# cavelandiah/BBMap

Measured on AMD Instinct MI355X. Metric: aligned_reads_per_sec, higher is better.
Workload: dtype int32

## Files before the change

bbmap_amd/_lib.py:

```python
import ctypes as C
import os

HERE = os.path.dirname(os.path.abspath(__file__))
SO_PATH = os.path.join(HERE, "libbbmap_amd.so")

EXPORTS = [
    "bbmap_last_error", "bbmap_abi_version",
    "bbmsa_create", "bbmsa_destroy", "bbmsa_align_batch_device", "bbmsa_align_batch",
    "bbmsa_fill_packed", "bbmsa_fill_submit", "bbmsa_fill_collect", "bbmsa_legacy_stats", "bbmsa_last_kernel_ms", "bbmsa_last_kernel_ms3", "bbmsa_last_counts", "bbmsa_align_gapped_batch_device", "bbmsa_align_gapped_batch", "bbmsa_align_batch_device_indirect",
    "bbmsa_align_gapped_batch_device_indirect", "bbmsa_last_route", "bbmsa_last_unlimited", "bbmsa_geometry", "bbmsa_debug_sorted_lists",
    "bbband_create", "bbband_destroy", "bbband_align_batch_device", "bbband_align_batch",
    "bbband_align_quadruple_batch", "bbband_align_quadruple_progressive_batch", "bbband_align_double_batch",
    "bbidx_create", "bbidx_destroy", "bbidx_find_batch_device", "bbidx_find_batch", "bbidx_find_batch_device_rc", "bbidx_last_stats", "bbidx_last_launch", "bbidx_set_kernel", "bbidx_set_max_read_len", "bbidx_build", "bbidx_get_params", "bbidx_export_block",
    "bbmap_default_config", "bbmap_create", "bbmap_destroy", "bbmap_map_batch_device", "bbmap_map_batch", "bbmap_get_output", "bbmap_get_overflow_output", "bbmap_last_stats", "bbmap_pack_sites_device",
    "bbmap_copy_to_host", "bbidx_get_chrom_table",
    "bbpipe_revcomp_device", "bbpipe_quick_rescue_device",
    "bbidx_build_profile", "bbkeys_default_config", "bbkeys_make", "bbkeys_make_batch", "bbmap_default_config_profile",
    "bbmap_get_final", "bbmap_set_average_pair_dist", "bbmap_final_batch_device", "bbmap_untrim_batch_device",
    "bbidx_set_scaffolds", "bbmap_get_scaffold_records",
    "bbmap_get_sam_records", "bbmap_get_sam",
    "bbkeys_device_workspace_bytes", "bbkeys_make_batch_device",
    "bbpipe_run_stats_device", "bbmap_add_run_stats", "bbmap_get_run_stats", "bbmap_reset_run_stats", "bbmap_set_adaptive", "bbmap_set_truth",
    "bbmap_get_adaptive_state",
    "bbpipe_coverage_layout", "bbpipe_coverage_workspace_bytes", "bbpipe_coverage_add_device", "bbpipe_coverage_finalize_device",
    "bbmap_cov_enable", "bbmap_add_coverage", "bbmap_cov_finalize", "bbmap_get_coverage", "bbmap_reset_coverage",
    "bbpipe_read_hist_bytes", "bbpipe_read_hist_view", "bbpipe_read_hist_add_device",
    "bbmap_hist_enable", "bbmap_add_read_hist", "bbmap_get_read_hist_view", "bbmap_get_read_hist", "bbmap_reset_read_hist",
    "bbpipe_refsplit_state_bytes", "bbpipe_refsplit_add_device", "bbpipe_refsplit_lists_workspace_bytes", "bbpipe_refsplit_lists_device",
    "bbmap_split_enable", "bbmap_add_split", "bbmap_get_split_records", "bbmap_get_split_lists_device", "bbmap_get_split_lists",
    "bbmap_get_split_stats", "bbmap_reset_split",
]
TRIM_EXPORTS = ["bbtrim_default_config", "bbtrim_batch", "bbtrim_batch_device"]


class bbmsa_job(C.Structure):
    _fields_ = [("read_off", C.c_int64), ("ref_off", C.c_int64),
                ("read_len", C.c_int32), ("ref_len", C.c_int32),
                ("refStartLoc", C.c_int32), ("refEndLoc", C.c_int32),
                ("minScore", C.c_int32), ("flags", C.c_int32)]


class bbmsa_result(C.Structure):
    _fields_ = [("result", C.c_int32 * 5), ("status", C.c_int32), ("iterations", C.c_int64),
                ("score", C.c_int32 * 8), ("score_len", C.c_int32), ("match_len", C.c_int32),
                ("fill_kind", C.c_int32), ("columns", C.c_int32)]


class bbmsa_config(C.Structure):
    _fields_ = [("device", C.c_int32), ("maxRows", C.c_int32), ("maxColumns", C.c_int32),
                ("bandwidth", C.c_int32), ("bandwidthRatio", C.c_float), ("reserved", C.c_int32 * 3)]


class bbband_job(C.Structure):
    _fields_ = [("query_off", C.c_int64), ("ref_off", C.c_int64), ("query_len", C.c_int32), ("ref_len", C.c_int32),
                ("qstart", C.c_int32), ("rstart", C.c_int32), ("maxEdits", C.c_int32), ("flags", C.c_int32)]


class bbband_result(C.Structure):
    _fields_ = [("edits", C.c_int32), ("lastQueryLoc", C.c_int32), ("lastRefLoc", C.c_int32), ("lastRow", C.c_int32),
                ("lastEdits", C.c_int32), ("lastOffset", C.c_int32), ("status", C.c_int32), ("reserved", C.c_int32)]


class bbband_config(C.Structure):
# ... 10 lines not shown
    pass


def load():
    global _lib
    if _lib is not None:
        return _lib
    so_path = os.environ.get("BBMAP_AMD_SO") or SO_PATH
    if not os.path.exists(so_path):
        raise BBMapAmdError(
            "libbbmap_amd.so is missing (%s). Build it with `python -m bbmap_amd.build`; "
            "there is no CPU fallback." % so_path)
    L = C.CDLL(so_path)
    L.bbmap_last_error.restype = C.c_char_p
    L.bbmap_abi_version.restype = C.c_int
    L.bbmsa_create.argtypes = [C.POINTER(bbmsa_config), C.POINTER(C.c_void_p)]
    L.bbmsa_create.restype = C.c_int
    L.bbmsa_destroy.argtypes = [C.c_void_p]
    L.bbmsa_destroy.restype = None
    L.bbmsa_align_batch_device.argtypes = [C.c_void_p, C.c_void_p, C.c_int64, C.c_void_p, C.c_void_p,
                                           C.c_void_p, C.c_void_p, C.c_void_p, C.c_int32]
    L.bbmsa_align_batch_device.restype = C.c_int
    L.bbmsa_align_batch.argtypes = [C.c_void_p, C.c_int64, C.c_void_p, C.c_void_p, C.c_int64,
                                    C.c_void_p, C.c_int64, C.c_void_p, C.c_void_p, C.c_int32]
    L.bbmsa_align_batch.restype = C.c_int
    L.bbmsa_align_gapped_batch_device.argtypes = [C.c_void_p, C.c_void_p, C.c_int64, C.c_void_p, C.c_void_p, C.c_void_p,
                                                  C.c_void_p, C.c_void_p, C.c_void_p, C.c_int32]
    L.bbmsa_align_gapped_batch_device.restype = C.c_int
    L.bbmsa_align_batch_device_indirect.argtypes = [C.c_void_p, C.c_void_p, C.c_void_p, C.c_int64, C.c_void_p, C.c_void_p,
                                                    C.c_void_p, C.c_void_p, C.c_void_p, C.c_int32]
    L.bbmsa_align_batch_device_indirect.restype = C.c_int
    L.bbmsa_align_gapped_batch_device_indirect.argtypes = [C.c_void_p, C.c_void_p, C.c_void_p, C.c_int64, C.c_void_p, C.c_void_p,
                                                           C.c_void_p, C.c_void_p, C.c_void_p, C.c_void_p, C.c_int32]
    L.bbmsa_align_gapped_batch_device_indirect.restype = C.c_int
    L.bbmsa_align_gapped_batch.argtypes = [C.c_void_p, C.c_int64, C.c_void_p, C.c_void_p, C.c_void_p, C.c_int64,
                                           C.c_void_p, C.c_int64, C.c_void_p, C.c_void_p, C.c_int32]
    L.bbmsa_align_gapped_batch.restype = C.c_int
    L.bbmsa_fill_packed.argtypes = [C.c_void_p, C.c_void_p, C.c_int32, C.c_void_p, C.c_int32, C.c_int32, C.c_int32, C.c_int32,
                                    C.c_int32, C.c_void_p, C.POINTER(C.c_int64), C.c_void_p]
    L.bbmsa_fill_packed.restype = C.c_int
    L.bbmsa_fill_submit.argtypes = [C.c_void_p, C.c_void_p, C.c_int32, C.c_void_p, C.c_int32, C.c_int32, C.c_int32, C.c_int32,
                                    C.c_int32, C.c_void_p, C.POINTER(C.c_int64), C.c_void_p]
    L.bbmsa_fill_submit.restype = C.c_int
    L.bbmsa_fill_collect.argtypes = [C.c_void_p, C.c_void_p, C.c_void_p, C.c_void_p, C.c_void_p]
    L.bbmsa_fill_collect.restype = C.c_int
    L.bbmsa_legacy_stats.argtypes = [C.c_void_p, C.POINTER(C.c_int64)]
    L.bbmsa_legacy_stats.restype = C.c_int
    L.bbmsa_last_kernel_ms3.argtypes = [C.c_void_p, C.POINTER(C.c_float)]
    L.bbmsa_last_kernel_ms3.restype = C.c_int
    L.bbmsa_last_counts.argtypes = [C.c_void_p, C.POINTER(C.c_int64)]
    L.bbmsa_last_counts.restype = C.c_int
    L.bbmsa_debug_sorted_lists.argtypes = [C.c_void_p, C.c_int64, C.c_void_p, C.POINTER(C.c_int64)]
    L.bbmsa_debug_sorted_lists.restype = C.c_int
    L.bbmsa_last_route.argtypes = [C.c_void_p, C.POINTER(C.c_int64)]
    L.bbmsa_last_route.restype = C.c_int
    L.bbmsa_last_unlimited.argtypes = [C.c_void_p, C.POINTER(C.c_int64)]
    L.bbmsa_last_unlimited.restype = C.c_int
    L.bbmsa_geometry.argtypes = [C.c_void_p, C.POINTER(C.c_int32)]
    L.bbmsa_geometry.restype = C.c_int
    L.bbmsa_last_kernel_ms.argtypes = [C.c_void_p, C.POINTER(C.c_float), C.POINTER(C.c_float)]
    L.bbmsa_last_kernel_ms.restype = C.c_int
    L.bbband_create.argtypes = [C.POINTER(bbband_config), C.POINTER(C.c_void_p)]
    L.bbband_create.restype = C.c_int
    L.bbband_destroy.argtypes = [C.c_void_p]
    L.bbband_destroy.restype = None
    L.bbband_align_batch_device.argtypes = [C.c_void_p, C.c_void_p, C.c_int64, C.c_void_p, C.c_void_p, C.c_void_p]
    L.bbband_align_batch_device.restype = C.c_int
    L.bbband_align_batch.argtypes = [C.c_void_p, C.c_int64, C.c_void_p, C.c_void_p, C.c_int64, C.c_void_p]
    L.bbband_align_batch.restype = C.c_int
    L.bbpipe_revcomp_device.argtypes = [C.c_void_p, C.c_int64, C.c_void_p, C.c_void_p, C.c_void_p]
    L.bbpipe_revcomp_device.restype = C.c_int
    L.bbpipe_quick_rescue_device.argtypes = [C.c_void_p, C.c_int64, C.c_void_p, C.c_void_p, C.c_void_p, C.c_void_p, C.c_void_p,
                                             C.c_void_p, C.c_void_p, C.c_int32, C.c_int32, C.c_int32, C.c_int32]
    L.bbpipe_quick_rescue_device.restype = C.c_int
    _lib = L
    return L


def check(rc, what):
    if rc != 0:
        raise BBMapAmdError("%s failed (%d): %s" % (what, rc, load().bbmap_last_error().decode()))
```

bbmap_amd/csrc/mapper_ctx.h:

```cpp
#pragma once
#include <hip/hip_runtime.h>

#include <cstdio>
#include <thread>
#include <vector>

#include "bbmap_amd.h"
#include "host_common.h"
#include "index_ctx.h"
#include "mapper_dev.h"
#include "msa_ctx.h"

enum { HIO_READS, HIO_BASES, HIO_SCORES, HIO_KEYINFO, HIO_COUNTS, HIO_OFFSETS, HIO_PACKED, BUF_PACK_TMP, BUF_SAM_TMP, BUF_SAM_TEXT, BUF_COUNT };

enum { ACC_STATS, ACC_COV, ACC_HIST, ACC_SPLIT, ACC_COUNT };
struct Accum { bool counted = false; hipStream_t stream = nullptr; };

struct bbmap_ctx {
    bbmap_config cfg;
    bbidx_ctx *index;
    hipStream_t hostStream = nullptr;
    bbidx_launch probeLs;
    bbmsa_ctx *msa, *msaGapped;
    bbmapper::Settings S;
    std::vector<void *> allocs;
    bbidx_site *d_psites; int *d_pnsites;
    bbmap_msite *d_ms; int *d_mcount, *d_near;
    bbmapper::SlowState *d_slow;
    int *d_active[2];
    unsigned *d_counters;
    bbmsa_job *d_jobs; bbmap_jobinfo *d_jinfo; bbmsa_result *d_results; uint8_t *d_match;
    bbmsa_job *d_gjobs; bbmsa_gaps *d_ggaps; bbmap_jobinfo *d_ginfo; bbmsa_result *d_gresults; uint8_t *d_gmatch;
    bbresc_job *d_rjobs; bbmapper::RescInfo *d_rinfo; bbresc_result *d_rres; bbmapper::PairResc *d_pres; bbmap_msite *d_rsite;
    const uint8_t *const *d_chromArr; const int *d_chromArrLen; const uint8_t *refsBase;
    int *d_chromMin;
    long long *d_chromOff;
    long long jobCap, gjobCap, rescCap;
    bbmapper::FinalRead *d_fin; bbmap_final *d_final; uint8_t *d_pool; long long poolUnits, poolUsed, finalFills;
    int matchStride, gmatchStride, maxRows, plainColumns;
    unsigned *h_counters;
    hipEvent_t ev[bbmapper::EV_COUNT];
    bbmap_stats stats;
    long long nJobs, nGapped;
    bool ran;
    bbmap_ctx *tier;
    bool ownsMsa;
    long long narrowMinJobs;
    bool sortWide;
    bool sortPlain;
    int *d_tierUnits; bbidx_read *d_tierReads; int *d_tierReadIds;
    long long tierReads;
    hipStream_t tierStream;
    hipStream_t dpStream; hipEvent_t evFork, evJoin;
    std::thread tierThread;
    bool tierStarted;
    int tierRc; char tierErr[320];
    long long overAfterBegin;
    struct BatchArgs { int64_t n_reads; const bbidx_read *reads; uint8_t *bases; int64_t minus_delta; const int8_t *baseScores; const int32_t *keyinfo; } batch;
    DevBuf buf[BUF_COUNT];
    bbmap_scafrec *d_scafRec = nullptr;
    int *d_scafTier = nullptr;
    bbmap_samrec *d_samRec = nullptr;
    int *d_samCounts = nullptr;
    long long *d_samOffsets = nullptr;
    float *d_mapqMax = nullptr;
    long long samTextBytes = 0;
    unsigned long long *d_runStats = nullptr, *d_insertHist = nullptr;
    int adaptive = 0;
    long long numMatedSeen = 0;
    const bbmap_truth *truthNext = nullptr;
    struct CovState *cov = nullptr;
    unsigned long long *d_readHist = nullptr;
    int rhFlags = 0;
    uint8_t *d_pool2 = nullptr; long long pool2Units = 0;
    int *d_untrimCounts = nullptr;
    long long *d_untrimOffsets = nullptr;
    DevBuf untrimTmp;
    bool untrimmed = false;
    struct SplitState *split = nullptr;
    Accum accum[ACC_COUNT];
    void new_batch() { for (Accum &a : accum) a.counted = false; untrimmed = false; }
};

struct SplitState {
    bbmap_split_config cfg = {};
    int nscaf = 0;
    long long gen = 0, added = -1, total = 0;
    DevBuf sets, keys, state, recs, ws, setoff, units;
    SplitState() = default;
    SplitState(const SplitState &) = delete;
    ~SplitState() { for (DevBuf *b : {&sets, &keys, &state, &recs, &ws, &setoff, &units}) b->release(); }
};

struct CovState {
    int flags = 0, nscaf = 0, binsize = -1;
    long long slots = 0, nbins = 0, gen = 0;
    DevBuf covoff, len, diff[2], depth[2], recs, hist[2], totals, ws, refgc, binoff, bins[2];
    std::vector<int> hostLen;
    CovState() = default;
    CovState(const CovState &) = delete;
    ~CovState() {
// ... 15 lines not shown
```

bbmap_amd/csrc/mapper_host.hip:

```cpp
#include <hip/hip_runtime.h>

#include <algorithm>
#include <cstdlib>
#include <cstring>
#include <new>
#include <thread>
#include <vector>

#include "mapper_ctx.h"

using namespace bbmapper;

extern "C" int bbmap_default_config_profile(int32_t profile, bbmap_config *c) {
    if (!c || (profile != BBIDX_PROFILE_BBMAP && profile != BBIDX_PROFILE_PACBIO)) return bbfail(BBMAP_E_ARG, "bbmap_default_config: bad argument");
    memset(c, 0, sizeof *c);
    c->paired = 0; c->max_reads = 0; c->max_sites = 32;
    c->extraPadding = 10; c->maxPairDist = 32000; c->averagePairDist = 100; c->maxRescueDist = 1200; c->maxRescueMismatches = 32;
    c->maxTrimSitesToRetain = 800; c->trimList = 1; c->doRescue = 1; c->clearzone3 = 800; c->fastCols = 0; c->jobsPerRead = 0;
    c->finalStage = profile == BBIDX_PROFILE_BBMAP ? 1 : 0;
    if (profile == BBIDX_PROFILE_PACBIO) {
        c->max_read_len = 6016; c->minRatio = 0.46f; c->slowAlignPadding = 8; c->slowRescuePadding = 16; c->tipSearchDist = 15;
        c->alignColumns = 7600; c->msaMaxColumns = 7600;
    } else {
        c->max_read_len = 150; c->minRatio = 0.56f; c->slowAlignPadding = 4; c->slowRescuePadding = 8; c->tipSearchDist = 100;
// ... 62 lines not shown
    S.clearzone1e = 2 * S.ptsMatch2 - S.ptsMatch - S.ptsSub + 1;
    S.msaMaxColumns = cfg->msaMaxColumns;
    if (pacbio) { S.ptsSubR = -157; S.ptsIns = -205; S.ptsIns2 = -42; S.ptsIns3 = -23; S.ptsIns4 = -8; S.ptsDel = -292; S.ptsDel2 = -37; S.ptsDel3 = -17; S.ptsDel4 = -2; }
    else { S.ptsSubR = -147; S.ptsIns = -395; S.ptsIns2 = -39; S.ptsIns3 = -23; S.ptsIns4 = -8; S.ptsDel = -472; S.ptsDel2 = -33; S.ptsDel3 = -9; S.ptsDel4 = -1; }
    S.ptsDel5 = -1; S.ptsGap = -2;
    if (pacbio && (cfg->finalStage < 0 || cfg->finalStage > 2)) return bail(bbfail(BBMAP_E_ARG, "bbmap_create: finalStage must be 0, 1 or 2"));
    S.finalStage = cfg->finalStage ? 1 : 0;
    S.finalPolicy = (pacbio && cfg->finalStage == 1) ? 1 : 0;
    {
        const float rP = S.finalPolicy ? 1.5f : 1.6f, r1 = S.finalPolicy ? 2.2f : 2.0f, r1b = S.finalPolicy ? 2.8f : 2.6f, r1c = S.finalPolicy ? 4.8f : 4.6f;
        const float m2 = (float)S.ptsMatch2;
        S.czP = (int)(rP * m2); S.cz1 = (int)(r1 * m2); S.cz1b = (int)(r1b * m2); S.cz1c = (int)(r1c * m2);
        S.czLimit1e = 40;
    }
    index->dev.p.quitAfterTwoPerfects = cfg->paired ? 0 : 1;
    S.expLimit = (cfg->alignColumns * 17) / 20 - (2 * (cfg->slowAlignPadding + 10));
    const int maxRows = ((cfg->max_read_len + 31) / 32) * 32;
    c->maxRows = maxRows;
    bbmsa_config mc; memset(&mc, 0, sizeof mc);
    mc.device = cfg->device; mc.maxRows = maxRows;
    bbmsa_config gc;
    if (pacbio) {
        mc.maxRows = cfg->max_read_len + 4 > 6100 ? 6100 : cfg->max_read_len + 4;
        c->maxRows = mc.maxRows;
        mc.maxColumns = cfg->msaMaxColumns;
        mc.reserved[2] = BBMSA_SCHEME_9PACBIO;
        gc = mc;
        c->plainColumns = mc.maxColumns;
        if (parent) { c->msa = parent->msa; c->msaGapped = parent->msaGapped; c->ownsMsa = false; }
        else {
            c->ownsMsa = true;
            if ((rc = bbmsa_create(&mc, &c->msa)) != BBMAP_OK) return bail(rc);
            c->msaGapped = c->msa;
        }
    } else {
        mc.maxColumns = cfg->fastCols > 0 ? cfg->fastCols : 256;
        if (mc.maxColumns > cfg->msaMaxColumns) mc.maxColumns = cfg->msaMaxColumns;
        c->plainColumns = mc.maxColumns;
        gc = mc;
        gc.maxColumns = cfg->msaMaxColumns;
        gc.reserved[0] = 32; gc.reserved[1] = 640 < gc.maxColumns ? 640 : gc.maxColumns;
        if (const char *e = getenv("BBMAP_G2_LANES")) { if (*e) gc.reserved[0] = atoi(e); }
        if (const char *e = getenv("BBMAP_G2_COLS")) { if (*e) gc.reserved[1] = atoi(e) < gc.maxColumns ? atoi(e) : gc.maxColumns; }
        (void)parent;
        c->ownsMsa = true;
        if ((rc = bbmsa_create(&mc, &c->msa)) != BBMAP_OK) return bail(rc);
        if ((rc = bbmsa_create(&gc, &c->msaGapped)) != BBMAP_OK) return bail(rc);
    }
    const long long n = cfg->max_reads;
    const int cap = cfg->max_sites;
    c->narrowMinJobs = getenv("BBMAP_NARROW_MIN_JOBS") ? atoll(getenv("BBMAP_NARROW_MIN_JOBS")) : 32768;
    c->sortWide = !(getenv("BBMAP_SORT_WIDE") && atoi(getenv("BBMAP_SORT_WIDE")) == 0);
    c->sortPlain = !(getenv("BBMAP_SORT_PLAIN") && atoi(getenv("BBMAP_SORT_PLAIN")) == 0);
    if (!pacbio) {
        const bool wideUnl = !(getenv("BBMAP_WIDE_UNLIMITED") && atoi(getenv("BBMAP_WIDE_UNLIMITED")) == 0);
        bbmsa_set_wide_unlimited(c->msa, wideUnl);
        if (c->msaGapped != c->msa) bbmsa_set_wide_unlimited(c->msaGapped, wideUnl);
    }
    if (!pacbio) {
        const long long lat = getenv("BBMAP_LATENCY_JOBS") ? atoll(getenv("BBMAP_LATENCY_JOBS")) : 4096;
        if ((rc = bbmsa_set_latency_jobs(c->msa, lat)) != BBMAP_OK) return bail(rc);
        if (c->msaGapped != c->msa && (rc = bbmsa_set_latency_jobs(c->msaGapped, lat)) != BBMAP_OK) return bail(rc);
    }
    const int jpr = cfg->jobsPerRead > 0 ? cfg->jobsPerRead : 3;
    c->jobCap = n * jpr + 1024;
    c->gjobCap = parent ? n * 16 + 4096 : (n * jpr) / 24 + 4096;
    if (cfg->jobsPerRead < 0) c->jobCap = c->gjobCap = -(long long)cfg->jobsPerRead;
    c->rescCap = parent ? n * 64 + 1024 : n * 2 + 1024;
    c->matchStride = ((maxRows + c->plainColumns + 15) / 16) * 16;
    c->gmatchStride = ((maxRows + gc.maxColumns + 2 + 128 * 8 + 15) / 16) * 16;
#define DA(ptr, count) if ((rc = dalloc(c, &(ptr), (size_t)(count))) != BBMAP_OK) return bail(rc)
    DA(c->d_psites, n * cap); DA(c->d_pnsites, n);
    DA(c->d_ms, n * cap); DA(c->d_mcount, n); DA(c->d_near, n);
    DA(c->d_slow, n);
    DA(c->d_active[0], n); DA(c->d_active[1], n);
    DA(c->d_counters, CNT_WORDS);
    DA(c->d_jobs, c->jobCap); DA(c->d_jinfo, c->jobCap); DA(c->d_results, c->jobCap); DA(c->d_match, c->jobCap * c->matchStride);
    DA(c->d_gjobs, c->gjobCap); DA(c->d_ggaps, c->gjobCap); DA(c->d_ginfo, c->gjobCap); DA(c->d_gresults, c->gjobCap); DA(c->d_gmatch, c->gjobCap * c->gmatchStride);
    DA(c->d_rjobs, c->rescCap); DA(c->d_rinfo, c->rescCap); DA(c->d_rres, c->rescCap); DA(c->d_rsite, c->rescCap);
    DA(c->d_pres, n / 2 + 1);
    if (S.finalStage) {
        c->poolUnits = (n * (long long)(3 * (cfg->max_read_len + 16)) + 65536) / 4;
        if (const char *e = getenv("BBMAP_FINAL_POOL_UNITS")) { if (*e && atoll(e) >= 64) c->poolUnits = atoll(e); }
        DA(c->d_fin, n); DA(c->d_final, n); DA(c->d_pool, c->poolUnits * 4);
    }
    const int nch = index->dev.nchroms;
    DA(c->d_chromMin, nch + 1); DA(c->d_chromOff, nch + 1);
#undef DA
    c->d_chromArr = index->dev.chromArr; c->d_chromArrLen = index->dev.chromArrLen;
    {
        std::vector<const uint8_t *> hc((size_t)nch + 1);
        if (hipMemcpy(hc.data(), index->dev.chromArr, sizeof(void *) * hc.size(), hipMemcpyDeviceToHost) != hipSuccess) return bail(bbfail(BBMAP_E_HIP, "bbmap_create: reading the chromosome table failed"));
        c->refsBase = hc[1];
        std::vector<long long> off((size_t)nch + 1, 0);
        for (int i = 1; i <= nch; i++) off[(size_t)i] = (long long)(hc[(size_t)i] - hc[1]);
        if (hipMemcpy(c->d_chromOff, off.data(), 8 * off.size(), hipMemcpyHostToDevice) != hipSuccess) return bail(bbfail(BBMAP_E_HIP, "bbmap_create: upload failed"));
        if (hipMemset(c->d_chromMin, 0, 4 * ((size_t)nch + 1)) != hipSuccess) return bail(bbfail(BBMAP_E_HIP, "bbmap_create: memset failed"));
    }
    if (hipHostMalloc((void **)&c->h_counters, CNT_WORDS * 4) != hipSuccess) return bail(bbfail(BBMAP_E_NOMEM, "bbmap_create: pinned allocation failed"));
    for (hipEvent_t &e : c->ev) if (hipEventCreate(&e) != hipSuccess) return bail(bbfail(BBMAP_E_HIP, "bbmap_create: hipEventCreate failed"));
    if (!getenv("BBMAP_SERIAL_DP") && !pacbio) {
        if (hipStreamCreateWithFlags(&c->dpStream, hipStreamNonBlocking) != hipSuccess || hipEventCreateWithFlags(&c->evFork, hipEventDisableTiming) != hipSuccess ||
            hipEventCreateWithFlags(&c->evJoin, hipEventDisableTiming) != hipSuccess) return bail(bbfail(BBMAP_E_HIP, "bbmap_create: stream / event creation failed"));
    }
    *out = c;
    return BBMAP_OK;
// ... 28 lines not shown
    BBHIP(hipMemcpyAsync(c->h_counters, c->d_counters, CNT_WORDS * 4, hipMemcpyDeviceToHost, stream));
    BBHIP(hipStreamSynchronize(stream));
    return BBMAP_OK;
}

template <class T> static int regrow(bbmap_ctx *c, hipStream_t stream, T **p, size_t oldCount, size_t newCount, std::vector<void *> &dead) {
    void *d = nullptr;
    if (hipMalloc(&d, (newCount ? newCount : 1) * sizeof(T)) != hipSuccess) return bbfail(BBMAP_E_NOMEM, "bbmap_map_batch_device: growing a fill log failed (device memory)");
    if (oldCount) BBHIP(hipMemcpyAsync(d, *p, oldCount * sizeof(T), hipMemcpyDeviceToDevice, stream));
    for (void *&q : c->allocs) if (q == (void *)*p) q = d;
    dead.push_back((void *)*p);
    *p = (T *)d;
    return BBMAP_OK;
}
struct DeadArrays {
    hipStream_t stream; std::vector<void *> v;
    explicit DeadArrays(hipStream_t s) : stream(s) {}
    ~DeadArrays() { if (!v.empty()) { (void)hipStreamSynchronize(stream); for (void *q : v) (void)hipFree(q); } }
};
static int grow_logs(bbmap_ctx *c, hipStream_t stream, Dev &D, long long needJobs, long long needGapped, long long usedJobs, long long usedGapped) {
    DeadArrays guard(stream);
    std::vector<void *> &dead = guard.v;
    if (needJobs > c->jobCap) {
        long long nc = c->jobCap * 2; if (nc < needJobs) nc = needJobs + needJobs / 4 + 1024;
        BBTRY(regrow(c, stream, &c->d_jobs, (size_t)usedJobs, (size_t)nc, dead));
        BBTRY(regrow(c, stream, &c->d_jinfo, (size_t)usedJobs, (size_t)nc, dead));
        BBTRY(regrow(c, stream, &c->d_results, (size_t)usedJobs, (size_t)nc, dead));
        BBTRY(regrow(c, stream, &c->d_match, (size_t)usedJobs * c->matchStride, (size_t)nc * c->matchStride, dead));
        c->jobCap = nc;
    }
    if (needGapped > c->gjobCap) {
        long long nc = c->gjobCap * 2; if (nc < needGapped) nc = needGapped + needGapped / 4 + 1024;
        BBTRY(regrow(c, stream, &c->d_gjobs, (size_t)usedGapped, (size_t)nc, dead));
        BBTRY(regrow(c, stream, &c->d_ggaps, (size_t)usedGapped, (size_t)nc, dead));
        BBTRY(regrow(c, stream, &c->d_ginfo, (size_t)usedGapped, (size_t)nc, dead));
        BBTRY(regrow(c, stream, &c->d_gresults, (size_t)usedGapped, (size_t)nc, dead));
        BBTRY(regrow(c, stream, &c->d_gmatch, (size_t)usedGapped * c->gmatchStride, (size_t)nc * c->gmatchStride, dead));
        c->gjobCap = nc;
    }
    c->h_counters[CNT_STAGE_FILLS] = (unsigned)usedJobs; c->h_counters[CNT_STAGE_GAPPED] = (unsigned)usedGapped;
    BBHIP(hipMemcpyAsync(c->d_counters + CNT_FILLS, c->h_counters + CNT_STAGE_FILLS, 8, hipMemcpyHostToDevice, stream));
    BBHIP(hipStreamSynchronize(stream));
    D.jobs = c->d_jobs; D.jinfo = c->d_jinfo; D.results = c->d_results; D.match = c->d_match; D.jobCap = c->jobCap;
    D.gjobs = c->d_gjobs; D.ggaps = c->d_ggaps; D.ginfo = c->d_ginfo; D.gresults = c->d_gresults; D.gmatch = c->d_gmatch; D.gjobCap = c->gjobCap;
    c->stats.log_growths += 1.0f;
    return BBMAP_OK;
}

static int run_fills(bbmap_ctx *c, hipStream_t stream, const uint8_t *bases, long long jobBase, long long nNew, long long gBase, long long gNew,
                     bool finalStage = false) {
    bbmsa_use_narrow(c->msa, nNew >= c->narrowMinJobs);
    bbmsa_sort_by_width(c->msa, c->sortPlain && nNew >= c->narrowMinJobs);
    bbmsa_sort_with_band(c->msa, c->sortPlain);
    if (c->msaGapped != c->msa) { bbmsa_use_narrow(c->msaGapped, false); bbmsa_sort_by_width(c->msaGapped, c->sortWide); }
    hipStream_t gs = (c->dpStream && nNew > 0) ? c->dpStream : stream;
    if (gNew > 0) {
        if (gs != stream) { BBHIP(hipEventRecord(c->evFork, stream)); BBHIP(hipStreamWaitEvent(gs, c->evFork, 0)); }
        BBTRY(bbmsa_align_gapped_batch_device(c->msaGapped, gs, gNew, c->d_gjobs + gBase, c->d_ggaps + gBase, bases, c->refsBase,
                                             c->d_gresults + gBase, c->d_gmatch + gBase * c->gmatchStride, c->gmatchStride));
        if (gs != stream) { BBHIP(hipEventRecord(c->evJoin, gs)); if (nNew > 0) BBTRY(bbmsa_wait_first_pass(c->msaGapped, stream)); }
    }
    if (nNew > 0)
        BBTRY(bbmsa_align_batch_device(c->msa, stream, nNew, c->d_jobs + jobBase, bases, c->refsBase, c->d_results + jobBase,
                                      c->d_match + jobBase * c->matchStride, c->matchStride));
    const int r1 = nNew > 0 ? bbmsa_last_route_flags(c->msa) : 0;
    const int r2 = gNew > 0 ? bbmsa_last_route_flags(c->msaGapped) : 0;
    c->stats.dp_narrow_launches += (r1 & 1) + (r2 & 1);
    c->stats.dp_sorted_launches += ((r1 >> 1) & 1) + ((r2 >> 1) & 1);
    if (gNew > 0 && gs != stream) BBHIP(hipStreamWaitEvent(stream, c->evJoin, 0));
    return BBMAP_OK;
}

static void add_dp_ms(bbmap_ctx *c, bool plain, bool gapped) {
    float k3[3];
    if (plain && bbmsa_last_kernel_ms3(c->msa, k3) == BBMAP_OK) { c->stats.ms_dp_narrow += k3[0]; c->stats.ms_dp_wave += k3[1]; c->stats.ms_dp_generic += k3[2];
                                                                 if (k3[1] > c->stats.ms_dp_wave_max) c->stats.ms_dp_wave_max = k3[1]; }
    if (gapped && c->msaGapped != c->msa && bbmsa_last_kernel_ms3(c->msaGapped, k3) == BBMAP_OK) c->stats.ms_dp_gapped += k3[0] + k3[1] + k3[2];
    static const bool show = getenv("BBMAP_DP_COUNTS") != nullptr;
    if (show) {
        int64_t n4[4], u4[4];
        if (plain && bbmsa_last_counts(c->msa, n4) == BBMAP_OK && bbmsa_last_unlimited(c->msa, u4) == BBMAP_OK)
            fprintf(stderr, "dp counts plain : narrow finished %lld, narrow handed on %lld, wavefront list %lld, to the wide/generic pass %lld, "
                    "unlimited in their own build %lld, in the general build %lld, wavefront steps unlimited %lld of %lld\n",
                    (long long)n4[0], (long long)n4[1], (long long)n4[2], (long long)n4[3], (long long)u4[0], (long long)u4[1], (long long)u4[2], (long long)u4[3]);
        if (gapped && bbmsa_last_counts(c->msaGapped, n4) == BBMAP_OK && bbmsa_last_unlimited(c->msaGapped, u4) == BBMAP_OK)
            fprintf(stderr, "dp counts second: narrow finished %lld, narrow handed on %lld, wavefront list %lld, to the wide/generic pass %lld, "
                    "unlimited in their own build %lld, in the general build %lld, wavefront steps unlimited %lld of %lld\n",
                    (long long)n4[0], (long long)n4[1], (long long)n4[2], (long long)n4[3], (long long)u4[0], (long long)u4[1], (long long)u4[2], (long long)u4[3]);
    }
}

static void tier_start_async(bbmap_ctx *c, long long found);

struct Rounds {
    bool finalStage;
    long long jobBase, gBase;
    long long nActive;
    int cur = 0;
    bool first = true, ranPlain = false, ranGapped = false;
};
template <class K> static int round_begin(bbmap_ctx *c, hipStream_t stream, Dev &D, Rounds &R, K kernel) {
    BBHIP(hipMemsetAsync(c->d_counters + CNT_NEXT_ACTIVE, 0, 4, stream));
    if (R.finalStage) {
        BBHIP(hipMemsetAsync(c->d_counters + CNT_POOL_AT_FAILURE, 0xff, 4, stream));
        BBHIP(hipMemsetAsync(c->d_counters + CNT_POOL_FAILED, 0, 4, stream));
    }
    D.activeIn = R.first ? nullptr : c->d_active[R.cur]; D.nActiveIn = (int)R.nActive; D.activeOut = c->d_active[1 - R.cur];
    BBTRY(launch<128>(kernel, R.nActive, stream, D));
    return read_counters(c, stream);
}
static int round_end(bbmap_ctx *c, hipStream_t stream, Dev &D, Rounds &R, const uint8_t *bases) {
    add_dp_ms(c, R.ranPlain, R.ranGapped);
    const long long asked = c->h_counters[CNT_FILLS], gasked = c->h_counters[CNT_GAPPED_FILLS];
    const long long total = asked < c->jobCap ? asked : c->jobCap, gtotal = gasked < c->gjobCap ? gasked : c->gjobCap;
    BBTRY(run_fills(c, stream, bases, R.jobBase, total - R.jobBase, R.gBase, gtotal - R.gBase, R.finalStage));
    R.ranPlain = total > R.jobBase; R.ranGapped = gtotal > R.gBase;
    R.jobBase = total; R.gBase = gtotal;
    if (asked > c->jobCap || gasked > c->gjobCap) BBTRY(grow_logs(c, stream, D, asked, gasked, total, gtotal));
    R.nActive = c->h_counters[CNT_NEXT_ACTIVE];
    R.cur = 1 - R.cur; R.first = false;
    return BBMAP_OK;
}

static int grow_pool(bbmap_ctx *c, hipStream_t stream, Dev &D, long long used, long long units, bool setCounter) {
    if (units > 0x7ffffff0LL) return bbfail(BBMAP_E_NOMEM, "bbmap_map_batch_device: the final stage's match strings exceed 8 GB; map smaller batches");
    DeadArrays guard(stream);
    BBTRY(regrow(c, stream, &c->d_pool, (size_t)used * 4, (size_t)units * 4, guard.v));
    if (setCounter) {
        c->h_counters[CNT_STAGE_POOL] = (unsigned)used;
        BBHIP(hipMemcpyAsync(c->d_counters + CNT_POOL_UNITS, c->h_counters + CNT_STAGE_POOL, 4, hipMemcpyHostToDevice, stream));
    }
    BBHIP(hipStreamSynchronize(stream));
    c->poolUnits = units; D.pool = c->d_pool; D.poolUnits = units;
    return BBMAP_OK;
}

static int run_final_stage(bbmap_ctx *c, hipStream_t stream, Dev &D, int64_t n_reads, const uint8_t *bases, long long jobBase, long long gBase,
                           long long &finalRounds, long long &finalLocal) {
// ... 141 lines not shown
    c->finalFills = 0; c->poolUsed = 0;
    long long finalRounds = 0, finalLocal = 0;
    if (c->S.finalStage) BBTRY(run_final_stage(c, stream, D, n_reads, bases, jobBase, gBase, finalRounds, finalLocal));
    BBTRY(finish_stats(c, stream, true, jobBase + gBase, finalRounds, finalLocal));
    c->ran = true;
    return BBMAP_OK;
}

static int tier_pass(bbmap_ctx *c, hipStream_t s, long long found) {
    bbmap_ctx *t = c->tier;
    const bbmap_ctx::BatchArgs &B = c->batch;
    const int paired = c->cfg.paired;
    c->tierReads = 0; t->ran = false;
    std::vector<int> ids((size_t)found);
    BBHIP(hipMemcpyAsync(ids.data(), c->d_tierUnits, 4 * (size_t)found, hipMemcpyDeviceToHost, s));
    BBHIP(hipStreamSynchronize(s));
    std::sort(ids.begin(), ids.end());
    const long long room = paired ? t->cfg.max_reads / 2 : t->cfg.max_reads;
    const long long take = found < room ? found : room;
    BBHIP(hipMemcpyAsync(c->d_tierUnits, ids.data(), 4 * (size_t)take, hipMemcpyHostToDevice, s));
    BBTRY(launch<128>(gather_reads_kernel, take, s, B.reads, c->d_tierUnits, (int)take, paired, c->d_tierReads, c->d_tierReadIds));
    BBHIP(hipStreamSynchronize(s));
    const long long tn = paired ? 2 * take : take;
    BBTRY(map_records(t, s, tn, c->d_tierReads, B.bases, B.minus_delta, B.baseScores, B.keyinfo, false));
    c->tierReads = tn;
    return BBMAP_OK;
}

static void tier_start_async(bbmap_ctx *c, long long found) {
    c->tierStarted = true; c->tierRc = BBMAP_OK; c->tierErr[0] = 0;
    c->tierThread = std::thread([c, found]() {
        int rc = hipSetDevice(c->cfg.device) == hipSuccess ? BBMAP_OK : BBMAP_E_HIP;
        if (rc == BBMAP_OK) rc = tier_pass(c, c->tierStream, found);
        if (rc != BBMAP_OK) { snprintf(c->tierErr, sizeof c->tierErr, "overflow tier: %s", bbmap_last_error()); }
        c->tierRc = rc;
    });
}

static int tier_finish(bbmap_ctx *c, hipStream_t stream) {
    bbmap_ctx *t = c->tier;
    const long long tn = c->tierReads;
    if (tn == 0) return BBMAP_OK;
    BBHIP(hipMemsetAsync(c->d_counters + CNT_TIER_RESOLVED, 0, 4, stream));
    BBTRY(launch<128>(mark_tier_kernel, tn, stream, c->d_mcount, t->d_mcount, c->d_tierReadIds, (int)tn, c->d_counters + CNT_TIER_RESOLVED));
    BBTRY(read_counters(c, stream));
    bbmap_stats &st = c->stats; const bbmap_stats &ts = t->stats;
    st.reads_reprobed = tn;
    st.reads_overflowed -= (long long)c->h_counters[CNT_TIER_RESOLVED];
    st.reads_without_site += ts.reads_without_site;
    st.fills += ts.fills; st.gapped_fills += ts.gapped_fills; st.refills += ts.refills; st.rescue_scans += ts.rescue_scans;
    st.rescue_fills += ts.rescue_fills; st.fills_dropped += ts.fills_dropped;
    st.final_fills += ts.final_fills; st.final_local += ts.final_local;
    st.dp_narrow_launches += ts.dp_narrow_launches; st.dp_sorted_launches += ts.dp_sorted_launches;
    st.sites_cross_scaffold += ts.sites_cross_scaffold;
    if (getenv("BBMAP_TIER_DEBUG"))
        fprintf(stderr, "[bbmap tier] reads %lld: probe %.2f begin %.2f score %.2f slow %.2f (rounds %lld) finish %.2f rescue %.2f total %.2f\n",
                tn, ts.ms_probe, ts.ms_begin, ts.ms_score, ts.ms_slow, (long long)ts.rounds, ts.ms_finish, ts.ms_rescue, ts.ms_total);
    return BBMAP_OK;
}

static int rescue_skip_rule(bbmap_ctx *c, bool *skip) {
    *skip = false;
    if (!c->d_runStats) return BBMAP_OK;
    bbmap_runstats rs;
    BBHIP(hipStreamSynchronize(c->accum[ACC_STATS].stream));
    BBHIP(hipMemcpy(&rs, c->d_runStats, sizeof rs, hipMemcpyDeviceToHost));
    *skip = rs.mappedRetained2 > 1000 && rs.numMated * 20LL < rs.mappedRetained2;
    return BBMAP_OK;
}

static int adapt_after_batch(bbmap_ctx *c, hipStream_t stream) {
    if (!(c->adaptive & BBMAP_ADAPT_INSERT_LENGTH)) return BBMAP_OK;
    bbmap_runstats rs;
    BBHIP(hipMemcpyAsync(&rs, c->d_runStats, sizeof rs, hipMemcpyDeviceToHost, stream));
    BBHIP(hipStreamSynchronize(stream));
    const bool heldPaired = rs.numMated > c->numMatedSeen;
    c->numMatedSeen = rs.numMated;
    if (rs.numMated > 1000 && heldPaired) {
        volatile float sum = (float)rs.innerLengthSum, cnt = (float)rs.numMated;
        const float q = sum * 1.0f / cnt;
        const int v = (int)q;
        if (v >= 0) BBTRY(bbmap_set_average_pair_dist(c, v));
    }
    return BBMAP_OK;
}

extern "C" int bbmap_get_adaptive_state(bbmap_ctx *c, int32_t *averagePairDist, int32_t *rescueSkipped) {
    if (!c) return bbfail(BBMAP_E_ARG, "bbmap_get_adaptive_state: null context");
    if (averagePairDist) *averagePairDist = c->cfg.averagePairDist;
    if (rescueSkipped) {
        bool skip = false;
        if (c->adaptive & BBMAP_ADAPT_RESCUE_SKIP) { BBHIP(hipSetDevice(c->cfg.device)); BBTRY(rescue_skip_rule(c, &skip)); }
        *rescueSkipped = skip ? 1 : 0;
    }
    return BBMAP_OK;
}

static int map_batch_device(bbmap_ctx *c, hipStream_t stream, int64_t n_reads, const bbidx_read *reads, uint8_t *bases,
                            int64_t minus_delta, const int8_t *baseScores, const int32_t *keyinfo) {
    c->batch = {n_reads, reads, bases, minus_delta, baseScores, keyinfo};
    c->tierStarted = false; c->tierReads = 0;
    if (c->tier) c->tier->ran = false;
    const int rc = map_records(c, stream, n_reads, reads, bases, minus_delta, baseScores, keyinfo, true);
    hipEvent_t e0 = c->ev[EV_TIER_BEGIN], e1 = c->ev[EV_TIER_END];
    if (c->tierStarted) {
        c->tierThread.join();
// ... 72 lines not shown
```

bbmap_amd/csrc/msa_common.h:

```cpp
#pragma once
#include <hip/hip_runtime.h>
#include <stdint.h>
#include "bbmap_amd.h"

namespace bbmsa {

constexpr int kScoreOffset = 11;
constexpr int kTimeMask = 0x7FF;
constexpr int kScoreMask = (int)0xFFFFF800;
constexpr int kMaxTime = 2047;

#define BBMSA_PT(x) ((x) * 2048)
constexpr int P_MATCH = BBMSA_PT(70), P_MATCH2 = BBMSA_PT(100);
constexpr int P_SUB = BBMSA_PT(-127), P_SUBR = BBMSA_PT(-147), P_SUB2 = BBMSA_PT(-51), P_SUB3 = BBMSA_PT(-25);
constexpr int P_INS = BBMSA_PT(-395), P_INS2 = BBMSA_PT(-39), P_INS3 = BBMSA_PT(-23), P_INS4 = BBMSA_PT(-8);
constexpr int P_DEL = BBMSA_PT(-472), P_DEL2 = BBMSA_PT(-33), P_DEL3 = BBMSA_PT(-9), P_DEL4 = BBMSA_PT(-1),
              P_DEL5 = BBMSA_PT(-1);
constexpr int P_DEL_REF_N = BBMSA_PT(-10), P_GAP = BBMSA_PT(-2);
constexpr int kBadOff = (-(((1 << 20) - 1) - 2000) - 1) * 2048;
constexpr int kMinOffScore = (-(((1 << 20) - 1) - 2000)) * 2048;
constexpr int kNegInf = -(1 << 30);
constexpr int kGapLen = 128;

constexpr int kTableLen = 3072;
// ... 49 lines not shown
    static constexpr int BADOFF = (-(((1 << 22) - 1) - 2000) - 1) * 512;
#undef BBMSA_PB
    __host__ __device__ static inline int del_off(int len) {
        if (len <= 0) return 0;
        int s = DEL;
        if (len > 80) { s += ((len - 80 + 3) / 4) * DEL5; len = 80; }
        if (len > 20) { s += (len - 20) * DEL4; len = 20; }
        if (len > 5) { s += (len - 5) * DEL3; len = 5; }
        if (len > 1) s += (len - 1) * DEL2;
        return s;
    }
    __host__ __device__ static inline int ins_cum_off(int len) {
        if (len <= 0) return 0;
        int s = INS;
        if (len > 20) { s += (len - 20) * INS4; len = 20; }
        if (len > 5) { s += (len - 5) * INS3; len = 5; }
        if (len > 1) s += (len - 1) * INS2;
        return s;
    }
    __host__ __device__ static inline int col0(int row) {
        if (row <= 0) return 0;
        int s = INS;
        if (row >= 20) { s += (row - 19) * INS4; row = 19; }
        if (row >= 5) { s += (row - 4) * INS3; row = 4; }
        if (row >= 2) s += (row - 1) * INS2;
        return s;
    }
};

__host__ __device__ inline int fill_halfband(int rows, int columns, int bandwidth, float bandwidthRatio) {
    if (bandwidth < 1 && bandwidthRatio <= 0.0f) return 0;
    const int bwA = bandwidth < 1 ? 9999999 : bandwidth;
    const int bwB = bandwidthRatio <= 0.0f ? 9999999 : 8 + (int)((float)rows * bandwidthRatio);
    return max(min(bwA, bwB), columns - rows + 8) / 2;
}
__host__ __device__ inline bool fill_is_limited(int flags, int minScore, int rows, int columns, int halfband) {
    const int mode = flags & BBMSA_MODE_MASK;
    if (mode == BBMSA_FILL_UNLIMITED_RAW) return false;
    if (mode == BBMSA_FILL_LIMITED_RAW) return true;
    return !(minScore < 1 || (columns + rows < 90) ||
             ((halfband < 1 || halfband * 3 > columns) && (columns > rows + min(170, rows + 20))));
}

__host__ __device__ inline bool band_is_candidate(int flags, int minScore, int rows, int columns, int maxRows, int maxColumns, int bandRows, int maxSlack) {
    const int mode = flags & BBMSA_MODE_MASK;
    if (!(rows >= 16 && columns >= rows && rows <= maxRows && rows <= bandRows && columns <= maxColumns && mode != BBMSA_FILL_UNLIMITED_RAW)) return false;
    int tmin = minScore;
    if (mode == BBMSA_FILL_LIMITED) {
        if (tmin < 1 || (columns + rows < 90) || (columns > rows + min(170, rows + 20))) return false;
        tmin -= 120;
    }
    return (70 + 100 * (rows - 1)) - tmin <= maxSlack;
}

__device__ inline long long job_count(long long njobs, const unsigned int *njobs_dev) {
    if (!njobs_dev) return njobs;
    const long long n = (long long)__hip_atomic_load(njobs_dev, __ATOMIC_RELAXED, __HIP_MEMORY_SCOPE_AGENT);
    return n < njobs ? n : njobs;
}

constexpr int kCounterWords = 32, kCounterBytes = kCounterWords * 4;
enum CounterSlot {
    CNT_FAST_QUEUE = 0,
    CNT_SLOW_COUNT = 1,
    CNT_GENERIC_QUEUE = 2,
    CNT_BAND_QUEUE = 3,
    CNT_LIST_COUNT = 4,
    CNT_BAND_DONE = 5,
    CNT_BAND_HANDED = 6,
    CNT_WIDE_SLOW_COUNT = 7,
    CNT_WIDE_QUEUE = 8,
    CNT_UNL_RAN_UNL = 9,
    CNT_UNL_RAN_GENERAL = 10,
    CNT_UNL_LIST_COUNT = 11,
    CNT_UNL_QUEUE = 12,
    CNT_UNL_STEPS = 13,
    CNT_ALL_STEPS = 14,
    CNT_CAND_COUNT = 15,
    CNT_SORTED_COUNT = 16,
    CNT_WAVE_STEPS = 17,
};
constexpr int CNT_BAND_STATS = 5, CNT_UNL_STATS = 9;
enum BandStat { BAND_STAT_DONE = 0, BAND_STAT_HANDED = 1 };
enum UnlStat { UNL_STAT_RAN_UNL = 0, UNL_STAT_RAN_GENERAL = 1, UNL_STAT_STEPS = 4, UNL_STAT_ALL_STEPS = 5, UNL_STAT_WAVE_STEPS = 8 };
static_assert(CNT_BAND_DONE == CNT_BAND_STATS + BAND_STAT_DONE && CNT_BAND_HANDED == CNT_BAND_STATS + BAND_STAT_HANDED, "band kernel's counters");
static_assert(CNT_UNL_RAN_UNL == CNT_UNL_STATS + UNL_STAT_RAN_UNL && CNT_UNL_RAN_GENERAL == CNT_UNL_STATS + UNL_STAT_RAN_GENERAL &&
              CNT_UNL_STEPS == CNT_UNL_STATS + UNL_STAT_STEPS && CNT_ALL_STEPS == CNT_UNL_STATS + UNL_STAT_ALL_STEPS &&
              CNT_WAVE_STEPS == CNT_UNL_STATS + UNL_STAT_WAVE_STEPS, "wavefront kernel's counters");
constexpr bool counter_slots_distinct() {
    constexpr int all[] = {CNT_FAST_QUEUE, CNT_SLOW_COUNT, CNT_GENERIC_QUEUE, CNT_BAND_QUEUE, CNT_LIST_COUNT, CNT_BAND_DONE, CNT_BAND_HANDED,
                           CNT_WIDE_SLOW_COUNT, CNT_WIDE_QUEUE, CNT_UNL_RAN_UNL, CNT_UNL_RAN_GENERAL, CNT_UNL_LIST_COUNT, CNT_UNL_QUEUE,
                           CNT_UNL_STEPS, CNT_ALL_STEPS, CNT_CAND_COUNT, CNT_SORTED_COUNT, CNT_WAVE_STEPS};
    unsigned seen = 0;
    for (int s : all) { if (s < 0 || s >= kCounterWords || ((seen >> s) & 1u)) return false; seen |= 1u << s; }
    return true;
}
static_assert(counter_slots_distinct(), "two counter names share a word, or one lies outside d_counters");

struct FillParams {
    const bbmsa_job *jobs;
    const uint8_t *reads;
    const uint8_t *refs;
    bbmsa_result *results;
    uint8_t *match;
    long long njobs;
    const unsigned int *njobs_dev;
    unsigned int *queue;
    unsigned int *dirbuf;
    long long dir_slot_dwords;
    const int *list;
    const unsigned int *list_count;
    int priority;
    int *slow_list;
    unsigned int *slow_count;
    int match_stride;
    int lanesPerJob;
    int fastCols;
    int tmpBytes;
    int tableLen;
    int maxRows, maxColumns;
    int bandwidth;
    float bandwidthRatio;
    unsigned int *unl_stats;
    int *planes;
    const long long *plane_off;
    int *limits;
    const long long *limits_off;
};

struct NarrowParams {
    const bbmsa_job *jobs;
    const uint8_t *reads;
    const uint8_t *refs;
    bbmsa_result *results;
    uint8_t *match;
    long long njobs;
    const unsigned int *njobs_dev;
    unsigned int *queue;
    int *fast_list;
    unsigned int *fast_count;
    unsigned int *stats;
    int match_stride;
    int maxRows, maxColumns;
    int bandwidth;
    float bandwidthRatio;
    int maxSlack;
    unsigned int *dirbuf32;
    int tableLen;
    int bandRows;
    const int *list;
    const unsigned int *list_count;
};

struct GenericParams {
    const bbmsa_job *jobs;
    const uint8_t *reads;
    const uint8_t *refs;
    bbmsa_result *results;
    uint8_t *match;
    const int *list;
    const unsigned int *list_count;
    long long njobs;
    const unsigned int *njobs_dev;
    int *matrix;
    int *limits;
    unsigned int *queue;
    int match_stride;
    int maxRows, maxColumns;
    int bandwidth;
    float bandwidthRatio;
};

}
```

bbmap_amd/csrc/msa_ctx.h:

```cpp
#pragma once
#include <hip/hip_runtime.h>

#include "bbmap_amd.h"
#include "host_common.h"
#include "msa_route.h"

struct bbmsa_ctx {
    bbmsa_config cfg = {};
    int device = 0;
    int numCUs = 0;
    RouteSwitches sw;
    Route last;
    int G = 0, R = 0, fastCols = 0, tmpBytes = 0, blocks = 0, ldsBytes = 0, tableLen = 0, wideTableLen = 0;
    long long dirSlotDwords = 0;
    unsigned int *d_dir = nullptr;
    unsigned int *d_counters = nullptr;
    DevBuf slowList;
    int genThreads = 0;
    int *d_matrix = nullptr;
    int *d_limits = nullptr;
    int wideR = 0, wideCols = 0, wideTmpBytes = 0, wideBlocks = 0, wideLdsBytes = 0;
    long long wideDirSlotDwords = 0;
    unsigned int *d_wideDir = nullptr;
    DevBuf slowList2;
    int narrowBlocks = 0, narrowSlack = 0;
    bool unlimitedStats = false;
    unsigned int *d_widthHist = nullptr;
    int bandRows = 0, bandLds = 0;
    unsigned int *d_bandDir = nullptr;
    DevBuf fastList;
    DevBuf gref, gaux, gjobs;
    hipEvent_t ev[4] = {};
    bool timed = false;
    bool legacyOnly = false;
    struct bbmsa_legacy *legacy = nullptr;
    int stripBlocks = 0, stripLds = 0;
    long long stripDwords = 0, stripSlotDwords = 0;
    int *d_stripBoundary = nullptr;
    uint8_t *d_stripTmp = nullptr;
    int pipeK = 0, pipeSlots = 0;
    int *d_pipeBoundary = nullptr, *d_pipeSync = nullptr;
};

struct JobBatch {
    int64_t n_jobs; const uint32_t *n_jobs_dev; const bbmsa_job *jobs; const uint8_t *reads, *refs; bbmsa_result *results; uint8_t *match;
    int32_t match_stride;
};
template <class P> void set_batch(P &p, const bbmsa_ctx *c, const JobBatch &B) {
    p.jobs = B.jobs; p.reads = B.reads; p.refs = B.refs; p.results = B.results; p.match = B.match;
    p.njobs = B.n_jobs; p.njobs_dev = B.n_jobs_dev; p.match_stride = B.match_stride;
    p.maxRows = c->cfg.maxRows; p.maxColumns = c->cfg.maxColumns; p.bandwidth = c->cfg.bandwidth; p.bandwidthRatio = c->cfg.bandwidthRatio;
}

int bbmsa_width_sort(bbmsa_ctx *c, hipStream_t stream, const bbmsa_job *jobs, int64_t n_jobs, bool band);

int bbmsa_align_impl(bbmsa_ctx *c, void *stream_, int64_t n_jobs, const uint32_t *n_jobs_dev, const bbmsa_job *jobs,
                     const uint8_t *reads, const uint8_t *refs, bbmsa_result *results, uint8_t *match, int32_t match_stride);

void bbmsa_use_narrow(bbmsa_ctx *c, bool on);
int bbmsa_wait_first_pass(bbmsa_ctx *c, void *waiter);
void bbmsa_sort_by_width(bbmsa_ctx *c, bool on);
void bbmsa_sort_with_band(bbmsa_ctx *c, bool on);
void bbmsa_set_wide_unlimited(bbmsa_ctx *c, bool on);
int bbmsa_set_latency_jobs(bbmsa_ctx *c, int64_t n);
enum { BBMSA_ROUTE_NARROW = 1, BBMSA_ROUTE_SORTED = 2, BBMSA_ROUTE_LATENCY = 4 };
int bbmsa_last_route_flags(const bbmsa_ctx *c);

int bbmsa_legacy_create(bbmsa_ctx *c);
void bbmsa_legacy_destroy(bbmsa_ctx *c);
void bbmsa_legacy_rows_per_lane(bbmsa_ctx *c, int *last, int *mask);
```

bbmap_amd/csrc/msa_fill_band.hip:

```cpp
#include "msa_common.h"
#include "msa_cell.h"

namespace bbmsa {

namespace {

__device__ __forceinline__ int from_left(int x, int fill) { return __builtin_amdgcn_update_dpp(fill, x, 0x138, 0xf, 0xf, false); }
__device__ __forceinline__ int from_right(int x, int fill) { return __builtin_amdgcn_update_dpp(fill, x, 0x130, 0xf, 0xf, false); }

__device__ __forceinline__ unsigned ld_coherent(const unsigned *p) { return __hip_atomic_load(p, __ATOMIC_RELAXED, __HIP_MEMORY_SCOPE_AGENT); }
__device__ __forceinline__ unsigned ld_coherent(const uint8_t *p) { return __hip_atomic_load(p, __ATOMIC_RELAXED, __HIP_MEMORY_SCOPE_AGENT); }

struct BandSet {
    int M[4], D[4], I[4];
    int rows, columns;
    int c0off;
    int minScoreOff, vs;
    unsigned w;
    int gprev;
    int gmask, mprev;
    int gpass;
    int bail;
    int rdOff, rfOff;
    int slot;
};

}

#ifndef BBMSA_BAND_OCC
#define BBMSA_BAND_OCC 4
#endif

template <int Q>
__global__ __launch_bounds__(256, BBMSA_BAND_OCC) void msa_fill_band_kernel(const NarrowParams p) {
    constexpr int B = 4 * Q;
    constexpr int GROUPS = 64 / Q;
    constexpr int JOBS = 2 * GROUPS;
    static_assert(Q == 4 || Q == 8 || Q == 16, "a group is a power of two of lanes, its good bits fit 64");
    extern __shared__ int lds[];
    const int TL = p.tableLen;
    int *delC = lds, *insC = lds + TL, *delExt = lds + 2 * TL, *insExt = delExt + 128;
    int4 *mTab = reinterpret_cast<int4 *>(delExt + 192);
    LdsPen pen; pen.delC = delC; pen.insC = insC; pen.delExt = delExt; pen.insExt = insExt; pen.mTab = mTab;
    for (int i = threadIdx.x; i < TL; i += blockDim.x) { delC[i] = calc_del_off(i); insC[i] = calc_ins_cum_off(i); }
    for (int i = threadIdx.x; i < 128; i += blockDim.x) delExt[i] = SpelledPen<Scheme11ts>().del_ext(i);
    if (threadIdx.x < 32) insExt[threadIdx.x] = SpelledPen<Scheme11ts>().ins_ext(threadIdx.x);
    if (threadIdx.x < 32) {
        const int st = threadIdx.x & 7, mt = (threadIdx.x >> 3) & 1, pv = threadIdx.x >> 4;
        const MEntry e = SpelledPen<Scheme11ts>().m_entry(min(st, 5), 0, 0, pv != 0, mt != 0);
        int4 v; v.x = e.addA; v.y = e.bonus; v.z = e.t3sub; v.w = 0;
        mTab[threadIdx.x] = v;
    }
    __syncthreads();

    const int lane = threadIdx.x & 63, wave = threadIdx.x >> 6;
    const int q = lane & (Q - 1), grp = lane / Q, groupBase = grp * Q;
    const int RB = (p.bandRows + 4 + 3) & ~3, FB = (p.bandRows + B + 4 + 3) & ~3;
    uint8_t *jobLds = reinterpret_cast<uint8_t *>(lds + lds_table_ints(TL)) + (long long)wave * JOBS * (RB + FB);
    unsigned *dir = p.dirbuf32 + ((long long)blockIdx.x * 4 + wave) * (long long)(p.bandRows + 1) * 128;
    const long long NJ = p.list ? (long long)ld_coherent(p.list_count) : job_count(p.njobs, p.njobs_dev);
    unsigned nDone = 0, nLeft = 0;

    for (;;) {
        long long myJ = -1;
        if (lane < JOBS) {
            for (;;) {
                const long long e_ = (long long)atomicAdd(p.queue, 1u);
                if (e_ >= NJ || e_ >= p.njobs) break;
                const long long t_ = p.list ? (long long)p.list[e_] : e_;
                const bbmsa_job t = p.jobs[t_];
                int ta = t.refStartLoc, tb = t.refEndLoc;
                if (t.flags & BBMSA_CLAMP_WINDOW) {
                    ta = max(0, ta); tb = min(t.ref_len - 1, tb);
                    if (tb - ta >= p.maxColumns) tb = min(t.ref_len - 1, ta + p.maxColumns - 1);
                }
                if (band_is_candidate(t.flags, t.minScore, t.read_len, tb - ta + 1, p.maxRows, p.maxColumns, p.bandRows, p.maxSlack)) { myJ = t_; break; }
                const unsigned k = atomicAdd(p.fast_count, 1u);
                p.fast_list[k] = (int)t_;
            }
        }
        if (!__any(myJ >= 0)) break;

        BandSet S[2];
        long long jobJ[2]; bool jobOk[2];
#pragma unroll
        for (int s = 0; s < 2; s++) {
            const long long j = __shfl(myJ, grp * 2 + s, 64);
            jobJ[s] = j;
            bbmsa_job jb;
            jb.read_off = 0; jb.ref_off = 0; jb.read_len = 0; jb.ref_len = 0; jb.refStartLoc = 0; jb.refEndLoc = -1; jb.minScore = 0; jb.flags = 0;
            if (j >= 0) jb = p.jobs[j];
            int a = jb.refStartLoc, b = jb.refEndLoc;
            if (jb.flags & BBMSA_CLAMP_WINDOW) {
                a = max(0, a); b = min(jb.ref_len - 1, b);
                if (b - a >= p.maxColumns) b = min(jb.ref_len - 1, a + p.maxColumns - 1);
            }
            const int rows = jb.read_len, columns = b - a + 1;
            int minScore = jb.minScore;
            if ((jb.flags & BBMSA_MODE_MASK) == BBMSA_FILL_LIMITED) minScore -= 120;
            const int D0 = (columns - rows) / 2 - B / 2;
            const uint8_t *rd = p.reads + jb.read_off, *rf = p.refs + jb.ref_off + a;
            const int rdOff = (grp * 2 + s) * (RB + FB), rfOff = rdOff + RB;
            int cost = 0; bool allDef = true;
#pragma unroll 4
            for (int i = q; i < rows; i += Q) {
                const int cb = rd[i];
                jobLds[rdOff + i] = (uint8_t)cb;
                if (fully_defined(cb)) cost += (i + 1 < rows && fully_defined(rd[i + 1])) ? P_MATCH2 : P_MATCH;
            }
            if (j >= 0)
#pragma unroll 4
            for (int k = q; k < rows + B + 1; k += Q) {
                const int col = k + D0;
                int v = 0;
                if (col == 0) v = '!';
                else if (col >= 1 && col <= columns) { v = rf[col - 1]; allDef = allDef && fully_defined(v); }
                jobLds[rfOff + k] = (uint8_t)v;
            }
            for (int c = 1 + q; c <= columns; c += Q) if (c < 1 + D0 || c > D0 + B) allDef = allDef && fully_defined(rf[c - 1]);
            int nd = allDef ? 0 : 1;
            for (int d = 1; d < Q; d <<= 1) { cost += __shfl_xor(cost, d, 64); nd |= __shfl_xor(nd, d, 64); }
            bool ok = j >= 0 && nd == 0;

            const int minScoreOff = minScore * 2048;
            const int floorv = minScoreOff - ((rows - 1) * P_MATCH2 + P_MATCH);
            const int subfloor = floorv - 5 * P_MATCH2;
            if (ok) {
                const int cl1 = rd[0];
                const int c0cost = fully_defined(cl1) ? ((rows > 1 && fully_defined(rd[1])) ? P_MATCH2 : P_MATCH) : 0;
// ... 66 lines not shown
                    const int c0 = row + T.c0off;
                    const int insRow = insC[row], insPrev = insC[row - 1];
                    const int delForce = (row < 3 || row > rows - 3) ? INT_MAX : INT_MIN;
                    const unsigned g5 = (unsigned)T.gmask | (((unsigned)uG & 1u) << 4);
                    const bool rowOne = row == 1;
                    unsigned goods = 0, mbits = 0, word = 0;
                    int leftM = lM, leftD = lD;
#pragma unroll
                    for (int i = 0; i < 4; i++) {
                        const int c = c0 + i;
                        const int ref1 = (int)((T.w >> (8 * i)) & 255u);
                        const bool inRange = (c >= 1) & (c <= columns);
                        const bool started = (T.gprev != 0) | ((g5 & ((4u << i) - 1u)) != 0u);
                        const bool first = c == 1;
                        const int hs = c <= columns - 1 ? P_MATCH + (columns - 1 - c) * P_MATCH2 : 0;
                        CellIn ci;
                        ci.row = row; ci.c = c; ci.rows = rows; ci.insNeededBase = (columns - c) + 1;
                        ci.cl1 = cl1; ci.ref1 = ref1; ci.refN = false; ci.gap = false; ci.match = cl1 == ref1; ci.act = inRange & started;
                        ci.refPen = 0; ci.limitP = max(vlimP, max(T.minScoreOff - hs, floorv) + 2048); ci.floorP = floorP; ci.subfloor = subfloor;
                        ci.dgM = first ? insPrev : T.M[i]; ci.dgD = first ? insPrev : T.D[i]; ci.dgI = first ? insPrev : T.I[i];
                        ci.lM = first ? insRow : leftM; ci.lD = first ? insRow : leftD;
                        ci.upM = i < 3 ? T.M[i + 1] : uM; ci.upI = i < 3 ? T.I[i + 1] : uI;
                        ci.delForce = delForce;
                        ci.insForce = ((rowOne & (c > 1)) | ((row > rows - 2) & (c < columns - 1))) ? INT_MAX : INT_MIN;
                        ci.pm8 = ((T.mprev >> i) & 1) ? 8 : 0;
                        const CellOut co = cell_update<Scheme11ts, false>(pen, ci);
                        const bool good = co.goodM | co.goodD | co.goodI;
                        goods |= good ? (1u << i) : 0u;
                        mbits |= ci.match ? (1u << i) : 0u;
                        word |= co.nib << (4 * i);
                        T.M[i] = co.nM; T.D[i] = co.nD; T.I[i] = co.nI;
                        leftM = co.nM; leftD = co.nD;
                    }
                    if (q == 0 && (goods & 1u) && c0 >= 1) T.bail = 1;
                    if (q == Q - 1 && (goods & 8u) && c0 + 3 < columns) T.bail = 1;
                    T.gprev = gIn; T.gmask = (int)goods; T.mprev = (int)mbits; T.gpass = (gIn | (goods ? 1 : 0));
                    dir[((long long)row * 2 + T.slot) * 64 + lane] = word | (goods << 16);
                }
            }
        }
        asm volatile("s_waitcnt vmcnt(0)" ::: "memory");
        __builtin_amdgcn_wave_barrier();

#pragma unroll
        for (int s = 0; s < 2; s++) {
            const long long j = jobJ[s];
            const int set = (q & 1) ^ s;
            int lastM[4], lastD[4], lastI[4];
#pragma unroll
            for (int i = 0; i < 4; i++) { lastM[i] = set ? S[1].M[i] : S[0].M[i]; lastD[i] = set ? S[1].D[i] : S[0].D[i]; lastI[i] = set ? S[1].I[i] : S[0].I[i]; }
            int bail = set ? S[1].bail : S[0].bail;
            for (int d = 1; d < Q; d <<= 1) bail |= __shfl_xor(bail, d, 64);
            const bool live = jobOk[s];
            if (live && bail) { if (q == 0) { const unsigned k = atomicAdd(p.fast_count, 1u); p.fast_list[k] = (int)j; nLeft++; } }
            if (!(live && !bail)) continue;

            const bbmsa_job jb = p.jobs[j];
            int a = jb.refStartLoc, b = jb.refEndLoc;
            if (jb.flags & BBMSA_CLAMP_WINDOW) {
                a = max(0, a); b = min(jb.ref_len - 1, b);
                if (b - a >= p.maxColumns) b = min(jb.ref_len - 1, a + p.maxColumns - 1);
            }
            const int rows = jb.read_len, columns = b - a + 1, mode = jb.flags & BBMSA_MODE_MASK;
            const int minScoreOff = (mode == BBMSA_FILL_LIMITED ? jb.minScore - 120 : jb.minScore) * 2048;
            const int subfloor = minScoreOff - ((rows - 1) * P_MATCH2 + P_MATCH) - 5 * P_MATCH2;
            const int D0 = (columns - rows) / 2 - B / 2;
            const uint8_t *rdL = jobLds + (grp * 2 + s) * (RB + FB), *rfL = rdL + RB;
            const unsigned *jdir = dir + s * 64 + groupBase;

            const int per = (rows + Q - 1) / Q;
            const int rFirst = q * per + 1, rLast = min(rows, (q + 1) * per);
            int iters = 0, lastColStart = 1, lastHasGood = 0, lastEntered = 0;
            {
                unsigned long long pg = 0;
                if (rFirst > 1 && rFirst <= rLast) for (int l = 0; l < Q; l++) pg |= (unsigned long long)((ld_coherent(jdir + (long long)(rFirst - 1) * 128 + l) >> 16) & 15u) << (4 * l);
                for (int r = rFirst; r <= rLast; r++) {
                    unsigned long long g = 0;
                    for (int l = 0; l < Q; l++) g |= (unsigned long long)((ld_coherent(jdir + (long long)r * 128 + l) >> 16) & 15u) << (4 * l);
                    const bool entered = r == 1 || pg != 0;
                    const int colStart = r == 1 ? 1 : (r - 1) + D0 + __builtin_ctzll(pg | (1ull << 63));
                    const int colStop = r == 1 ? columns : (r - 1) + D0 + (63 - __builtin_clzll(pg | 1ull));
                    const int maxG = g ? r + D0 + (63 - __builtin_clzll(g)) : -2;
                    const int endc = min(columns, max(colStop, maxG) + 1);
                    if (entered) iters += endc - colStart + 1;
                    if (r == rows) { lastColStart = colStart; lastHasGood = g != 0; lastEntered = entered; }
                    pg = g;
                }
            }
            for (int d = 1; d < Q; d <<= 1) iters += __shfl_xor(iters, d, 64);
            {
                const int owner = groupBase + (rows - 1) / per;
                lastColStart = __shfl(lastColStart, owner, 64); lastHasGood = __shfl(lastHasGood, owner, 64); lastEntered = __shfl(lastEntered, owner, 64);
            }
            int bScore = INT_MIN, bKey = INT_MAX, bPacked = 0;
#pragma unroll
            for (int i = 0; i < 4; i++) {
                const int c = rows + D0 + 4 * q + i;
                if (c >= 1 && c <= columns) {
                    const int v[3] = {lastM[i], lastD[i], lastI[i]};
#pragma unroll
                    for (int st = 0; st < 3; st++) {
                        const int sc = v[st] & kScoreMask, key = st * 65536 + c;
                        if (sc > bScore || (sc == bScore && key < bKey)) { bScore = sc; bKey = key; bPacked = v[st]; }
                    }
                }
            }
            for (int d = 1; d < Q; d <<= 1) {
// ... 53 lines not shown
                }
                int colS = col;
                if (row > colS) colS -= row;
                const int bestRefStart = a + colS, bestRefStop = a + res1 - 1;
                int padLeft = 0, padRight = 0;
                if (bestRefStart < a) padLeft = max(0, a - bestRefStart);
                else if (bestRefStart == a && state == 2) padLeft = stateTime;
                const int bW = (jb.flags & BBMSA_INTERNAL_GAPPED) ? jb.ref_len : b;
                if (bestRefStop > bW) padRight = max(0, bestRefStop - bW);
                else if (bestRefStop == bW && res2 == 2) padRight = bPacked & kTimeMask;
                if (wantScore) {
                    sc[0] = bScore >> kScoreOffset; sc[1] = bestRefStart; sc[2] = bestRefStop; sc[3] = rows; sc[4] = res1; sc[5] = res2;
                    scoreLen = (padLeft > 0 || padRight > 0) ? 8 : 6;
                    if (scoreLen == 8) { sc[6] = padLeft; sc[7] = padRight; }
                }
                if (wantTrace) {
                    const int xs = (col != row) ? row : 0;
                    for (int i = q; i < xs; i += Q) if (n + i < p.match_stride) out[n + i] = 'X';
                    n += xs;
                    if (n > p.match_stride) matchLen = -1;
                    else {
                        asm volatile("s_waitcnt vmcnt(0)" ::: "memory");
                        __builtin_amdgcn_wave_barrier();
                        for (int i = q; i < n / 2; i += Q) {
                            const uint8_t lo = (uint8_t)ld_coherent(out + i), hi = (uint8_t)ld_coherent(out + n - 1 - i);
                            out[i] = hi; out[n - 1 - i] = lo;
                        }
                        matchLen = n;
                    }
                }
            }
            if (q == 0) {
                bbmsa_result r;
                r.result[0] = rows; r.result[1] = res1; r.result[2] = res2; r.result[3] = res3; r.result[4] = res4;
                r.status = (fillNull && mode == BBMSA_FILL_LIMITED) ? BBMSA_ST_NULL : BBMSA_ST_OK;
                r.iterations = iters;
#pragma unroll
                for (int i = 0; i < 8; i++) r.score[i] = sc[i];
                r.score_len = scoreLen; r.match_len = matchLen; r.fill_kind = 0; r.columns = columns;
                p.results[j] = r;
                nDone++;
            }
        }
        __builtin_amdgcn_fence(__ATOMIC_ACQ_REL, "wavefront");
        __builtin_amdgcn_wave_barrier();
    }
    if (p.stats) {
        for (int d = 32; d >= 1; d >>= 1) { nDone += __shfl_xor(nDone, d, 64); nLeft += __shfl_xor(nLeft, d, 64); }
        if (lane == 0) { if (nDone) atomicAdd(&p.stats[BAND_STAT_DONE], nDone); if (nLeft) atomicAdd(&p.stats[BAND_STAT_HANDED], nLeft); }
    }
}

template __global__ void msa_fill_band_kernel<8>(const NarrowParams);

const void *band_kernel() { return (const void *)msa_fill_band_kernel<8>; }
int band_lds_bytes(int tableLen, int bandRows) {
    constexpr int Q = 8, B = 4 * Q, JOBS = 2 * (64 / Q);
    const int RB = (bandRows + 4 + 3) & ~3, FB = (bandRows + B + 4 + 3) & ~3;
    return lds_table_ints(tableLen) * 4 + 4 * JOBS * (RB + FB);
}

}
```

bbmap_amd/csrc/msa_fill_fast.hip:

```cpp
#include "msa_common.h"
#include "msa_cell.h"

namespace bbmsa {

__device__ __forceinline__ int lane_up(int x, int fill) {
    return __builtin_amdgcn_update_dpp(fill, x, 0x138, 0xf, 0xf, false);
}

__device__ __forceinline__ int clamp_time(int t) { return t > kMaxTime ? kMaxTime - 3 : t; }

__device__ __forceinline__ int del_extend(int streak) {
    int c = (streak & 3) == 0 ? P_DEL5 : 0;
    c = streak < 80 ? P_DEL4 : c;
    c = streak < 20 ? P_DEL3 : c;
    c = streak < 5 ? P_DEL2 : c;
    c = streak == 0 ? P_DEL : c;
    return c;
}
__device__ __forceinline__ int ins_extend(int streak) {
    int c = P_INS4;
    c = streak < 20 ? P_INS3 : c;
    c = streak < 5 ? P_INS2 : c;
    c = streak == 0 ? P_INS : c;
    return c;
}
__device__ __forceinline__ int sub_extend(int streak) {
    int c = P_SUB3;
    c = streak < 5 ? P_SUB2 : c;
    c = streak == 0 ? P_SUB : c;
    return c;
}

__device__ __forceinline__ unsigned load_coherent(const unsigned *p) {
    return __hip_atomic_load(p, __ATOMIC_RELAXED, __HIP_MEMORY_SCOPE_AGENT);
}

#ifndef BBMSA_MIN_WAVES
#define BBMSA_MIN_WAVES(R) ((R) <= 5 ? 4 : ((R) <= 7 ? 2 : 1))
#endif

template <int R, bool BANDED, bool MAT = false, int UNL = 0>
__global__ __launch_bounds__(256, (UNL == 2 && BBMSA_MIN_WAVES(R) > 2) ? 2 : BBMSA_MIN_WAVES(R)) void msa_fill_fast_kernel(const FillParams p) {
    extern __shared__ int lds[];
    int *delC = lds;
    const int TL = p.tableLen;
    int *insC = lds + TL;
    int *delExt = lds + 2 * TL;
    int *insExt = delExt + 128;
    int4 *mTab = reinterpret_cast<int4 *>(delExt + 192);
    LdsPen pen; pen.delC = delC; pen.insC = insC; pen.delExt = delExt; pen.insExt = insExt; pen.mTab = mTab;
    for (int i = threadIdx.x; i < TL; i += blockDim.x) {
        delC[i] = calc_del_off(i);
        insC[i] = calc_ins_cum_off(i);
    }
    for (int i = threadIdx.x; i < 128; i += blockDim.x) delExt[i] = del_extend(i);
    if (threadIdx.x < 32) insExt[threadIdx.x] = ins_extend(threadIdx.x);
    if (threadIdx.x < 32) {
        const int st = threadIdx.x & 7, mt = (threadIdx.x >> 3) & 1, pv = threadIdx.x >> 4;
        int4 e;
        if (mt) { e.x = pv ? P_MATCH2 : P_MATCH; e.y = P_MATCH; e.z = P_MATCH2; }
        else { e.x = pv ? (st <= 1 ? P_SUBR : P_SUB) : sub_extend(min(st, 5)); e.y = P_SUB; e.z = P_SUB3; }
        e.w = 0;
        mTab[threadIdx.x] = e;
    }
    __syncthreads();

    if (p.priority == 3) __builtin_amdgcn_s_setprio(3);
    else if (p.priority == 2) __builtin_amdgcn_s_setprio(2);
    else if (p.priority == 1) __builtin_amdgcn_s_setprio(1);
    const int lane = threadIdx.x & 63;
    const int wave = threadIdx.x >> 6;
    const int G = p.lanesPerJob;
    const int gl = lane & (G - 1);
    const int sub = lane / G;
    const int jobsPerWave = 64 / G;
    const int groupBase = sub * G;

    const int perJobLds = lds_job_ints(p.fastCols, p.tmpBytes);
    int *myLds = lds + lds_table_ints(TL) + (wave * jobsPerWave + sub) * perJobLds;
    int *colHl = myLds;
    uint8_t *colRef = reinterpret_cast<uint8_t *>(myLds + (p.fastCols + 2));
    uint8_t *tmp = reinterpret_cast<uint8_t *>(myLds + (p.fastCols + 2) + ((p.fastCols + 2 + 3) >> 2));

    const long long slot = ((long long)blockIdx.x * (blockDim.x >> 6) + wave) * jobsPerWave + sub;
    unsigned *dir = p.dirbuf + slot * p.dir_slot_dwords;

    const long long total = p.list ? (long long)load_coherent(p.list_count) : job_count(p.njobs, p.njobs_dev);
    for (;;) {
        unsigned base = 0;
        if (lane == 0) base = atomicAdd(p.queue, (unsigned)jobsPerWave);
        base = __builtin_amdgcn_readfirstlane(base);
        if ((long long)base >= total) break;
        const long long q = (long long)base + sub;
        const bool valid = q < total;
        const long long j = (p.list && valid) ? (long long)p.list[q] : q;

        bbmsa_job jb;
        if (valid) jb = p.jobs[j];
        else { jb.read_off = 0; jb.ref_off = 0; jb.read_len = 0; jb.ref_len = 0; jb.refStartLoc = 0; jb.refEndLoc = -1; jb.minScore = 0; jb.flags = 0; }
        const int rows = jb.read_len;
        int a = jb.refStartLoc, b = jb.refEndLoc;
        const int mode = jb.flags & BBMSA_MODE_MASK;
        if (jb.flags & BBMSA_CLAMP_WINDOW) {
            a = max(0, a);
            b = min(jb.ref_len - 1, b);
            if (b - a >= p.maxColumns) b = min(jb.ref_len - 1, a + p.maxColumns - 1);
        }
        const int columns = b - a + 1;
        const bool shapeOK = valid && rows >= 1 && columns >= 1 && rows <= p.maxRows && columns <= p.maxColumns;

        const int halfband = fill_halfband(rows, columns, p.bandwidth, p.bandwidthRatio);
        const bool limited = fill_is_limited(jb.flags, jb.minScore, rows, columns, halfband);
        const int minScore = (limited && mode != BBMSA_FILL_LIMITED_RAW) ? jb.minScore - 120 : jb.minScore;
        const bool fits = rows <= G * R && columns <= p.fastCols && columns >= rows - 2;
        const bool needGeneric = shapeOK && (!fits || (UNL == 1 && limited));
        const bool run = shapeOK && !needGeneric;
        const bool banded = limited && halfband > 0;
        int bandViolation = 0;

        if (gl == 0 && valid) {
            if (!shapeOK) {
                bbmsa_result r;
                for (int i = 0; i < 5; i++) r.result[i] = 0;
                r.status = BBMSA_ST_BAD_SHAPE; r.iterations = 0;
                for (int i = 0; i < 8; i++) r.score[i] = 0;
                r.score_len = 0; r.match_len = 0; r.fill_kind = 0; r.columns = columns;
                p.results[j] = r;
            } else if (needGeneric) {
                const unsigned k = atomicAdd(p.slow_count, 1u);
                p.slow_list[k] = (int)j;
            }
        }

        const uint8_t *rd = p.reads + jb.read_off;
        const uint8_t *rf = p.refs + jb.ref_off + a;
        int *planeM = nullptr; long long planeInts = 0; int planeW = 0;
        if (MAT && valid) { planeW = columns; planeInts = (long long)rows * planeW; planeM = p.planes + p.plane_off[j]; }

        const int maxGain = (rows - 1) * P_MATCH2 + P_MATCH;
        const int minScoreOff = minScore * 2048;
// ... 505 lines not shown
```

bbmap_amd/csrc/msa_host.hip:

```cpp
#include <hip/hip_runtime.h>

#include <cstdio>
#include <cstdlib>
#include <new>

#include "host_common.h"
#include "msa_common.h"
#include "msa_ctx.h"

namespace bbmsa {
struct StripParams {
    const bbmsa_job *jobs; const uint8_t *reads; const uint8_t *refs; bbmsa_result *results; uint8_t *match;
    long long njobs; const unsigned int *njobs_dev; unsigned int *queue; unsigned int *dirbuf;
    long long dir_slot_dwords, dir_strip_dwords; int *boundary; uint8_t *tmpbuf; int *slow_list; unsigned int *slow_count;
    int match_stride; int maxRows, maxColumns; int bandwidth; float bandwidthRatio;
    int pipeK, pipeSlots; int *pipeBoundary; int *pipeSync; int pipeSpinLimit;
};
int strip_rows_per_lane();
const void *strip_kernel_pacbio();
const void *strip_kernel_pacbio_pipelined();
int strip_pipe_sync_ints(int K);
const void *fast_kernel_for(int R, bool banded);
const void *fast_kernel_unl_for(int R);
const void *fast_kernel_both_for(int R);
template <class S> __global__ void msa_fill_generic_kernel(const GenericParams p);
const void *band_kernel();
int band_lds_bytes(int tableLen, int bandRows);
}

static int clamp_occupancy(int per, int most) { return per < 1 ? 1 : (per > most ? most : per); }

static int setup_wide_pass(bbmsa_ctx *c) {
    if (c->wideBlocks > 0) return BBMAP_OK;
    c->wideR = (c->cfg.maxRows + 63) / 64;
    c->wideCols = c->cfg.maxColumns;
    c->wideTmpBytes = ((64 * c->wideR + c->wideCols + 8) + 3) & ~3;
    const int perJob = bbmsa::lds_job_ints(c->wideCols, c->wideTmpBytes);
    c->wideLdsBytes = (bbmsa::lds_table_ints(c->wideTableLen) + perJob) * 4;
    const void *wfn = bbmsa::fast_kernel_for(c->wideR, c->sw.banded);
    if (wfn && c->wideLdsBytes <= 160 * 1024) {
        if (c->wideLdsBytes > 64 * 1024) BBHIP(hipFuncSetAttribute(wfn, hipFuncAttributeMaxDynamicSharedMemorySize, c->wideLdsBytes));
        const void *bfn = c->sw.banded ? nullptr : bbmsa::fast_kernel_both_for(c->wideR);
        if (bfn && c->wideLdsBytes > 64 * 1024) BBHIP(hipFuncSetAttribute(bfn, hipFuncAttributeMaxDynamicSharedMemorySize, c->wideLdsBytes));
        int per = 0;
        BBHIP(hipOccupancyMaxActiveBlocksPerMultiprocessor(&per, wfn, 64, c->wideLdsBytes));
        per = clamp_occupancy(per, 8);
        const long long slotDwords = (long long)(((c->wideCols + 64 - 1) >> 3) + 1) * c->wideR * 64;
        BBHIP(hipMalloc(&c->d_wideDir, (size_t)((long long)c->numCUs * per * slotDwords * 4)));
        c->wideDirSlotDwords = slotDwords;
        c->wideBlocks = c->numCUs * per;
        c->sw.widePresent = true;
    }
    return BBMAP_OK;
}

static int generic_threads(const bbmsa_config &cfg, int defaultMB, long long mostThreads, int *out) {
    const long long perThread = 3LL * (cfg.maxRows + 1) * (cfg.maxColumns + 2) * 4;
    long long threads = ((long long)env_int("BBMSA_GENERIC_SCRATCH_MB", defaultMB) << 20) / perThread;
    if (threads > mostThreads) threads = mostThreads;
    threads = (threads / 64) * 64;
    if (threads < 64) return bbfail(BBMAP_E_NOMEM, "bbmsa_create: BBMSA_GENERIC_SCRATCH_MB cannot hold one wavefront of scratch matrices for this maxRows x maxColumns");
    *out = (int)threads;
    return BBMAP_OK;
}
static int alloc_generic_scratch(bbmsa_ctx *c, int threads) {
    c->genThreads = threads;
    BBHIP(hipMalloc(&c->d_matrix, (size_t)threads * 3 * (size_t)(c->cfg.maxRows + 1) * (size_t)(c->cfg.maxColumns + 2) * 4));
    BBHIP(hipMalloc(&c->d_limits, (size_t)threads * (size_t)(c->cfg.maxRows + c->cfg.maxColumns + 4) * 4));
    return BBMAP_OK;
}

static int create_legacy_only(bbmsa_ctx *c) {
    BBTRY(alloc_generic_scratch(c, 1));
    return bbmsa_legacy_create(c);
}

static int create_pacbio(bbmsa_ctx *c) {
    const bbmsa_config *cfg = &c->cfg;
    int threads = 0;
    BBTRY(generic_threads(*cfg, 40960, 4096, &threads));
// ... 36 lines not shown
    if (G != 16 && G != 32 && G != 64) {
        G = env_int("BBMSA_LANES_PER_JOB", 0);
        if (G != 16 && G != 32 && G != 64) G = (cfg->maxRows <= 320) ? 32 : 64;
    }
    while (G < 64 && (cfg->maxRows + G - 1) / G > 10) G *= 2;
    c->G = G;
    c->R = (cfg->maxRows + G - 1) / G;
    int fastCols = cfg->reserved[1] > 0 ? cfg->reserved[1] : env_int("BBMSA_FAST_COLS", 0);
    if (fastCols <= 0) fastCols = cfg->maxColumns < 640 ? cfg->maxColumns : 640;
    if (fastCols > cfg->maxColumns) fastCols = cfg->maxColumns;
    c->fastCols = fastCols;
    c->tmpBytes = ((G * c->R + fastCols + 8) + 3) & ~3;
    const int jobsPerWave = 64 / G;
    const int perJobInts = bbmsa::lds_job_ints(fastCols, c->tmpBytes);
    {
        const int side = (cfg->maxColumns > cfg->maxRows ? cfg->maxColumns : cfg->maxRows) + 2;
        c->wideTableLen = (side < 2048 ? side : 2048) + cfg->maxRows + 8;
        const int sideF = (fastCols > cfg->maxRows ? fastCols : cfg->maxRows) + 2;
        c->tableLen = (sideF < 2048 ? sideF : 2048) + cfg->maxRows + 8;
    }
    if (c->tableLen > bbmsa::kTableLen) c->tableLen = bbmsa::kTableLen;
    if (c->wideTableLen > bbmsa::kTableLen) c->wideTableLen = bbmsa::kTableLen;
    c->tableLen = (c->tableLen + 3) & ~3; c->wideTableLen = (c->wideTableLen + 3) & ~3;
    c->ldsBytes = (bbmsa::lds_table_ints(c->tableLen) + 4 * jobsPerWave * perJobInts) * 4;
    if (c->ldsBytes > 160 * 1024) return bbfail(BBMAP_E_ARG, "bbmsa_create: fast-path LDS budget exceeded; lower reserved[1] (fastCols)");

    c->sw.banded = !(cfg->bandwidth < 1 && cfg->bandwidthRatio <= 0.0f);
    const void *kfn = bbmsa::fast_kernel_for(c->R, c->sw.banded);
    if (!kfn) return bbfail(BBMAP_E_ARG, "bbmsa_create: no kernel for this rows-per-lane");
    if (c->ldsBytes > 64 * 1024) {
        BBHIP(hipFuncSetAttribute(kfn, hipFuncAttributeMaxDynamicSharedMemorySize, c->ldsBytes));
        BBHIP(hipFuncSetAttribute(bbmsa::fast_kernel_unl_for(c->R), hipFuncAttributeMaxDynamicSharedMemorySize, c->ldsBytes));
    }
    int blocksPerCU = 0;
    BBHIP(hipOccupancyMaxActiveBlocksPerMultiprocessor(&blocksPerCU, kfn, 256, c->ldsBytes));
    if (blocksPerCU < 1) blocksPerCU = 1;
    const int capBlocks = env_int("BBMSA_BLOCKS_PER_CU", 0);
    if (capBlocks > 0 && capBlocks < blocksPerCU) blocksPerCU = capBlocks;
    c->blocks = c->numCUs * blocksPerCU;

    const int maxSteps = fastCols + G - 1;
    c->dirSlotDwords = (long long)((maxSteps >> 3) + 1) * c->R * G;
    const long long slots = (long long)c->blocks * 4 * jobsPerWave;
    BBHIP(hipMalloc(&c->d_dir, (size_t)(slots * c->dirSlotDwords * 4)));

    int threads = 0;
    BBTRY(generic_threads(*cfg, 2048, 16384, &threads));
    BBTRY(alloc_generic_scratch(c, threads));
    if (cfg->maxColumns > fastCols) BBTRY(setup_wide_pass(c));
    c->narrowSlack = env_int("BBMSA_NARROW_SLACK", 2000);
    if (!c->sw.banded && env_int("BBMSA_NARROW", 1) != 0) {
        int perCU = 0;
        c->bandRows = cfg->maxRows < 256 ? cfg->maxRows : 256;
        c->bandLds = bbmsa::band_lds_bytes(c->tableLen, c->bandRows);
        if (c->bandLds > 64 * 1024) BBHIP(hipFuncSetAttribute(bbmsa::band_kernel(), hipFuncAttributeMaxDynamicSharedMemorySize, c->bandLds));
        BBHIP(hipOccupancyMaxActiveBlocksPerMultiprocessor(&perCU, bbmsa::band_kernel(), 256, c->bandLds));
        c->narrowBlocks = c->numCUs * clamp_occupancy(perCU, 4);
        c->sw.bandPresent = true;
        BBHIP(hipMalloc(&c->d_bandDir, (size_t)c->narrowBlocks * 4 * (size_t)(c->bandRows + 1) * 128 * 4));
    }
    c->sw.sortByWidth = env_int("BBMSA_SORT_BY_WIDTH", 0) != 0;
    c->sw.sortWithBand = env_int("BBMSA_SORT_WITH_BAND", 0) != 0;
    c->sw.wideUnlimited = env_int("BBMSA_WIDE_UNLIMITED", 0) != 0;
    c->sw.unlimitedLoop = env_int("BBMSA_UNLIMITED_LOOP", 1) != 0;
    c->unlimitedStats = env_int("BBMSA_UNLIMITED_STATS", 0) != 0 || getenv("BBMAP_DP_COUNTS") != nullptr;
    { const int lat = env_int("BBMSA_LATENCY_JOBS", 0); if (lat > 0) BBTRY(bbmsa_set_latency_jobs(c, lat)); }
    return BBMAP_OK;
}

extern "C" int bbmsa_create(const bbmsa_config *cfg, bbmsa_ctx **out) {
    if (!cfg || !out) return bbfail(BBMAP_E_ARG, "bbmsa_create: null argument");
    *out = nullptr;
    const int scheme = cfg->reserved[2] & 0xFF;
    const bool legacyOnly = (cfg->reserved[2] & BBMSA_LEGACY_ONLY) != 0;
    if (scheme != BBMSA_SCHEME_11TS && scheme != BBMSA_SCHEME_9PACBIO) return bbfail(BBMAP_E_ARG, "bbmsa_create: unknown scoring scheme");
    if (scheme == BBMSA_SCHEME_11TS && (cfg->maxRows < 1 || cfg->maxRows > 640 || cfg->maxColumns < 1 || cfg->maxColumns > 4096))
        return bbfail(BBMAP_E_ARG, "bbmsa_create: maxRows must be 1..640 and maxColumns 1..4096");
    if (scheme == BBMSA_SCHEME_9PACBIO && (cfg->maxRows < 1 || cfg->maxRows > 6100 || cfg->maxColumns < 1 || cfg->maxColumns > 8192))
        return bbfail(BBMAP_E_ARG, "bbmsa_create: the PacBio scheme takes maxRows 1..6100 and maxColumns 1..8192");
    hipDeviceProp_t prop;
    BBTRY(bb_use_gfx950("bbmsa_create", cfg->device, &prop));

    bbmsa_ctx *c = new (std::nothrow) bbmsa_ctx();
    if (!c) return bbfail(BBMAP_E_NOMEM, "bbmsa_create: out of host memory");
    c->cfg = *cfg;
    c->device = cfg->device;
    c->numCUs = prop.multiProcessorCount;
    c->sw.scheme = scheme;
    c->legacyOnly = legacyOnly;
    struct Guard { bbmsa_ctx *c; ~Guard() { if (c) bbmsa_destroy(c); } } guard{c};
    BBTRY(legacyOnly ? create_legacy_only(c) : scheme != BBMSA_SCHEME_11TS ? create_pacbio(c) : create_11ts(c));
    BBHIP(hipMalloc(&c->d_counters, bbmsa::kCounterBytes));
    BBHIP(hipMemset(c->d_counters, 0, bbmsa::kCounterBytes));
    for (int i = 0; i < 4; i++) BBHIP(hipEventCreate(&c->ev[i]));
    guard.c = nullptr;
    *out = c;
    return BBMAP_OK;
}

extern "C" void bbmsa_destroy(bbmsa_ctx *c) {
    if (!c) return;
    (void)hipSetDevice(c->device);
    bbmsa_legacy_destroy(c);
    if (c->d_dir) (void)hipFree(c->d_dir);
    if (c->d_counters) (void)hipFree(c->d_counters);
    if (c->d_widthHist) (void)hipFree(c->d_widthHist);
    for (DevBuf *b : {&c->slowList, &c->slowList2, &c->fastList, &c->gref, &c->gaux, &c->gjobs}) b->release();
    if (c->d_matrix) (void)hipFree(c->d_matrix);
    if (c->d_limits) (void)hipFree(c->d_limits);
    if (c->d_wideDir) (void)hipFree(c->d_wideDir);
    if (c->d_bandDir) (void)hipFree(c->d_bandDir);
    if (c->d_stripBoundary) (void)hipFree(c->d_stripBoundary);
// ... 3 lines not shown
    for (int i = 0; i < 4; i++) if (c->ev[i]) (void)hipEventDestroy(c->ev[i]);
    delete c;
}

extern "C" int bbmsa_align_batch_device(bbmsa_ctx *c, void *stream_, int64_t n_jobs,
                                        const bbmsa_job *jobs, const uint8_t *reads, const uint8_t *refs,
                                        bbmsa_result *results, uint8_t *match, int32_t match_stride) {
    return bbmsa_align_impl(c, stream_, n_jobs, nullptr, jobs, reads, refs, results, match, match_stride);
}

extern "C" int bbmsa_align_batch_device_indirect(bbmsa_ctx *c, void *stream_, const uint32_t *n_jobs_dev, int64_t max_jobs,
                                                 const bbmsa_job *jobs, const uint8_t *reads, const uint8_t *refs,
                                                 bbmsa_result *results, uint8_t *match, int32_t match_stride) {
    if (!n_jobs_dev) return bbfail(BBMAP_E_ARG, "bbmsa_align_batch_device_indirect: null counter");
    return bbmsa_align_impl(c, stream_, max_jobs, n_jobs_dev, jobs, reads, refs, results, match, match_stride);
}

namespace {
using namespace bbmsa;

template <class S> int launch_generic(bbmsa_ctx *c, const JobBatch &B, hipStream_t stream, const int *list, const unsigned int *count) {
    bbmsa::GenericParams gp;
    set_batch(gp, c, B);
    gp.list = list; gp.list_count = count;
    gp.matrix = c->d_matrix; gp.limits = c->d_limits; gp.queue = c->d_counters + CNT_GENERIC_QUEUE;
    hipLaunchKernelGGL(bbmsa::msa_fill_generic_kernel<S>, dim3(c->genThreads / 64), dim3(64), 0, stream, gp);
    BBHIP(hipGetLastError());
    BBHIP(hipEventRecord(c->ev[2], stream));
    c->timed = true;
    return BBMAP_OK;
}

int launch_strip(bbmsa_ctx *c, const JobBatch &B, const Route &r, hipStream_t stream) {
    bbmsa::StripParams sp;
    set_batch(sp, c, B);
    sp.queue = c->d_counters + CNT_FAST_QUEUE; sp.dirbuf = c->d_dir; sp.dir_slot_dwords = c->stripSlotDwords; sp.dir_strip_dwords = c->stripDwords;
    sp.boundary = c->d_stripBoundary; sp.tmpbuf = c->d_stripTmp; sp.slow_list = c->slowList.as<int>(); sp.slow_count = c->d_counters + CNT_SLOW_COUNT;
    sp.pipeK = 0; sp.pipeSlots = 0; sp.pipeBoundary = nullptr; sp.pipeSync = nullptr;
    sp.pipeSpinLimit = env_int("BBMSA_PIPE_SPIN_LIMIT", 1 << 21);
    if (sp.pipeSpinLimit < 1) sp.pipeSpinLimit = 1;
    void *sargs[] = {&sp};
    if (r.pipelined) {
        const long long slots = r.jobs < c->pipeSlots ? r.jobs : c->pipeSlots;
        sp.pipeK = c->pipeK; sp.pipeSlots = (int)slots; sp.pipeBoundary = c->d_pipeBoundary; sp.pipeSync = c->d_pipeSync;
        BBHIP(hipMemsetAsync(c->d_pipeSync, 0, (size_t)(slots * bbmsa::strip_pipe_sync_ints(c->pipeK) * 4), stream));
        BBHIP(hipLaunchKernel(bbmsa::strip_kernel_pacbio_pipelined(), dim3((unsigned)(slots * c->pipeK)), dim3(64), sargs, (size_t)c->stripLds, stream));
        return BBMAP_OK;
    }
    const long long sblocks = r.jobs < c->stripBlocks ? r.jobs : c->stripBlocks;
    BBHIP(hipLaunchKernel(bbmsa::strip_kernel_pacbio(), dim3((unsigned)sblocks), dim3(64), sargs, (size_t)c->stripLds, stream));
    return BBMAP_OK;
}

int launch_band(bbmsa_ctx *c, const JobBatch &B, const Route &r, hipStream_t stream) {
    int *const fastList = c->fastList.as<int>();
    bbmsa::NarrowParams np;
    set_batch(np, c, B);
    np.queue = c->d_counters + CNT_BAND_QUEUE; np.fast_list = fastList; np.fast_count = c->d_counters + CNT_LIST_COUNT;
    np.stats = c->d_counters + CNT_BAND_STATS; np.maxSlack = c->narrowSlack;
    np.dirbuf32 = c->d_bandDir; np.tableLen = c->tableLen; np.bandRows = c->bandRows;
    np.list = r.sorted ? fastList + 2 * r.jobs : nullptr; np.list_count = r.sorted ? c->d_counters + CNT_CAND_COUNT : nullptr;
    long long nb = (r.jobs + 63) / 64;
    if (nb > c->narrowBlocks) nb = c->narrowBlocks;
    void *nargs[] = {&np};
    BBHIP(hipLaunchKernel(bbmsa::band_kernel(), dim3((unsigned)nb), dim3(256), nargs, (size_t)c->bandLds, stream));
    return BBMAP_OK;
}

bbmsa::FillParams first_pass_params(const bbmsa_ctx *c, const JobBatch &B, const Route &r) {
    bbmsa::FillParams fp = {};
    set_batch(fp, c, B);
    fp.queue = c->d_counters + CNT_FAST_QUEUE; fp.dirbuf = c->d_dir; fp.dir_slot_dwords = c->dirSlotDwords;
    fp.list = (r.band || r.sorted) ? c->fastList.as<int>() : nullptr; fp.list_count = c->d_counters + CNT_LIST_COUNT; fp.priority = 0;
    fp.slow_list = c->slowList.as<int>(); fp.slow_count = c->d_counters + CNT_SLOW_COUNT;
    fp.lanesPerJob = c->G; fp.fastCols = c->fastCols; fp.tmpBytes = c->tmpBytes; fp.tableLen = c->tableLen;
    fp.unl_stats = c->unlimitedStats ? c->d_counters + CNT_UNL_STATS : nullptr;
    return fp;
}

int launch_unlimited(bbmsa_ctx *c, const bbmsa::FillParams &fp, const Route &r, long long blocks, hipStream_t stream) {
    bbmsa::FillParams up = fp;
    up.queue = c->d_counters + CNT_UNL_QUEUE; up.list = c->fastList.as<int>() + r.jobs; up.list_count = c->d_counters + CNT_UNL_LIST_COUNT;
    void *uargs[] = {&up};
    BBHIP(hipLaunchKernel(bbmsa::fast_kernel_unl_for(c->R), dim3((unsigned)blocks), dim3(256), uargs, (size_t)c->ldsBytes, stream));
    return BBMAP_OK;
}

int launch_wide(bbmsa_ctx *c, const bbmsa::FillParams &fp, const Route &r, hipStream_t stream) {
    bbmsa::FillParams wp = fp;
    wp.queue = c->d_counters + CNT_WIDE_QUEUE; wp.dirbuf = c->d_wideDir; wp.dir_slot_dwords = c->wideDirSlotDwords;
    wp.list = r.latency ? nullptr : fp.slow_list; wp.list_count = r.latency ? nullptr : fp.slow_count;
    wp.slow_list = c->slowList2.as<int>(); wp.slow_count = c->d_counters + CNT_WIDE_SLOW_COUNT;
    wp.lanesPerJob = 64; wp.fastCols = c->wideCols; wp.tmpBytes = c->wideTmpBytes; wp.tableLen = c->wideTableLen;
    static const int widePrio = env_int("BBMSA_WIDE_PRIORITY", 2);
    wp.priority = widePrio;
    void *wargs[] = {&wp};
    const long long wblocks = r.latency && r.jobs < c->wideBlocks ? r.jobs : c->wideBlocks;
    const void *bothFn = r.wideBoth ? bbmsa::fast_kernel_both_for(c->wideR) : nullptr;
    BBHIP(hipLaunchKernel(bothFn ? bothFn : bbmsa::fast_kernel_for(c->wideR, c->sw.banded), dim3((unsigned)wblocks), dim3(64), wargs, (size_t)c->wideLdsBytes, stream));
    return BBMAP_OK;
}
}

int bbmsa_align_impl(bbmsa_ctx *c, void *stream_, int64_t n_jobs, const uint32_t *n_jobs_dev,
                     const bbmsa_job *jobs, const uint8_t *reads, const uint8_t *refs,
                     bbmsa_result *results, uint8_t *match, int32_t match_stride) {
    if (!c) return bbfail(BBMAP_E_ARG, "bbmsa_align_batch_device: null context");
    if (n_jobs < 0 || n_jobs > 0x7fffffffLL) return bbfail(BBMAP_E_ARG, "bbmsa_align_batch_device: n_jobs out of range");
    if (n_jobs == 0) return BBMAP_OK;
    if (!jobs || !reads || !refs || !results) return bbfail(BBMAP_E_ARG, "bbmsa_align_batch_device: null buffer");
    if (match && match_stride < 1) return bbfail(BBMAP_E_ARG, "bbmsa_align_batch_device: match_stride must be positive");
    hipStream_t stream = (hipStream_t)stream_;
    BBHIP(hipSetDevice(c->device));
    if (c->legacyOnly) return bbfail(BBMAP_E_ARG, "bbmsa_align_batch_device: this context was created for bbmsa_fill_packed only (BBMSA_LEGACY_ONLY)");
    const JobBatch B = {n_jobs, n_jobs_dev, jobs, reads, refs, results, match, match_stride};
    const Route r = plan_route(c->sw, n_jobs, n_jobs_dev != nullptr);
    const size_t listBytes = (size_t)n_jobs * 4;
    BBHIP(c->slowList.grow(listBytes, 0, &stream));
    if (r.wide) BBHIP(c->slowList2.grow(listBytes, 0, &stream));
    if (c->sw.bandPresent || r.sorted) BBHIP(c->fastList.grow(r.sorted ? 3 * listBytes : listBytes, 0, &stream));
    BBHIP(hipMemsetAsync(c->d_counters, 0, bbmsa::kCounterBytes, stream));
    c->last = r;
    BBHIP(hipEventRecord(c->ev[0], stream));
    if (c->sw.scheme != BBMSA_SCHEME_11TS) {
        BBHIP(hipEventRecord(c->ev[3], stream));
        BBTRY(launch_strip(c, B, r, stream));
        BBHIP(hipEventRecord(c->ev[1], stream));
        return launch_generic<bbmsa::Scheme9PacBio>(c, B, stream, c->slowList.as<int>(), c->d_counters + CNT_SLOW_COUNT);
    }
    if (r.sorted) BBTRY(bbmsa_width_sort(c, stream, jobs, n_jobs, r.band));
    if (r.band) BBTRY(launch_band(c, B, r, stream));
    BBHIP(hipEventRecord(c->ev[3], stream));
    bbmsa::FillParams fp = first_pass_params(c, B, r);
    const int jobsPerBlock = 4 * (64 / c->G);
    long long blocks = (n_jobs + jobsPerBlock - 1) / jobsPerBlock;
    if (blocks > c->blocks) blocks = c->blocks;
    if (r.unlList) BBTRY(launch_unlimited(c, fp, r, blocks, stream));
    void *args[] = {&fp};
    if (!r.latency)
        BBHIP(hipLaunchKernel(bbmsa::fast_kernel_for(c->R, c->sw.banded), dim3((unsigned)blocks), dim3(256), args, (size_t)c->ldsBytes, stream));
    if (r.wide) BBTRY(launch_wide(c, fp, r, stream));
    BBHIP(hipEventRecord(c->ev[1], stream));
    return launch_generic<bbmsa::Scheme11ts>(c, B, stream, r.wide ? c->slowList2.as<int>() : fp.slow_list,
                                             c->d_counters + (r.wide ? CNT_WIDE_SLOW_COUNT : CNT_SLOW_COUNT));
}

void bbmsa_use_narrow(bbmsa_ctx *c, bool on) { if (c) c->sw.bandOff = !on; }
void bbmsa_sort_by_width(bbmsa_ctx *c, bool on) { if (c) c->sw.sortByWidth = on; }
void bbmsa_sort_with_band(bbmsa_ctx *c, bool on) { if (c) c->sw.sortWithBand = on; }
void bbmsa_set_wide_unlimited(bbmsa_ctx *c, bool on) { if (c) c->sw.wideUnlimited = on; }
int bbmsa_set_latency_jobs(bbmsa_ctx *c, int64_t n) {
    if (!c || c->sw.scheme != BBMSA_SCHEME_11TS || c->legacyOnly) return BBMAP_OK;
    BBHIP(hipSetDevice(c->device));
    if (n > 0) BBTRY(setup_wide_pass(c));
    if (n > 0 && !c->slowList2.p) BBHIP(c->slowList2.grow(c->slowList.cap));
    c->sw.latencyJobs = c->sw.widePresent ? n : 0;
    return BBMAP_OK;
}
int bbmsa_wait_first_pass(bbmsa_ctx *c, void *waiter) {
    if (!c || !c->timed) return BBMAP_OK;
    BBHIP(hipStreamWaitEvent((hipStream_t)waiter, c->ev[3], 0));
    return BBMAP_OK;
}

extern "C" int bbmsa_last_kernel_ms(bbmsa_ctx *c, float *ms_fast, float *ms_slow) {
    if (!c || !c->timed) return bbfail(BBMAP_E_ARG, "bbmsa_last_kernel_ms: nothing launched yet");
    BBHIP(hipSetDevice(c->device));
    BBHIP(hipEventSynchronize(c->ev[2]));
    float a = 0, b = 0;
    BBHIP(hipEventElapsedTime(&a, c->ev[0], c->ev[1]));
    BBHIP(hipEventElapsedTime(&b, c->ev[1], c->ev[2]));
    if (ms_fast) *ms_fast = a;
    if (ms_slow) *ms_slow = b;
    return BBMAP_OK;
}

extern "C" int bbmsa_last_kernel_ms3(bbmsa_ctx *c, float *ms3) {
    if (!c || !c->timed || !ms3) return bbfail(BBMAP_E_ARG, "bbmsa_last_kernel_ms3: nothing launched yet");
    BBHIP(hipSetDevice(c->device));
    BBHIP(hipEventSynchronize(c->ev[2]));
    BBHIP(hipEventElapsedTime(&ms3[0], c->ev[0], c->ev[3]));
    BBHIP(hipEventElapsedTime(&ms3[1], c->ev[3], c->ev[1]));
    BBHIP(hipEventElapsedTime(&ms3[2], c->ev[1], c->ev[2]));
    return BBMAP_OK;
}

static int read_counters(bbmsa_ctx *c, unsigned (&h)[bbmsa::kCounterWords]) {
    BBHIP(hipSetDevice(c->device));
    BBHIP(hipEventSynchronize(c->ev[2]));
    BBHIP(hipMemcpy(h, c->d_counters, sizeof h, hipMemcpyDeviceToHost));
    return BBMAP_OK;
}

extern "C" int bbmsa_last_counts(bbmsa_ctx *c, int64_t *counts4) {
    if (!c || !c->timed || !counts4) return bbfail(BBMAP_E_ARG, "bbmsa_last_counts: nothing launched yet");
    unsigned h[bbmsa::kCounterWords];
    BBTRY(read_counters(c, h));
    const Route &r = c->last;
    counts4[0] = h[CNT_BAND_DONE]; counts4[1] = h[CNT_BAND_HANDED];
    counts4[2] = r.band ? (r.sorted ? h[CNT_SORTED_COUNT] + h[CNT_UNL_LIST_COUNT] : h[CNT_LIST_COUNT]) : 0;
    counts4[3] = r.wide ? h[CNT_WIDE_SLOW_COUNT] : h[CNT_SLOW_COUNT];
    if (getenv("BBMAP_DP_COUNTS")) {
        if (r.wide) fprintf(stderr, "   (first pass handed %u jobs to the wide pass)\n", h[CNT_SLOW_COUNT]);
        if (r.sorted) fprintf(stderr, "   (sorted: %u general, %u unlimited, %u band candidates)\n", h[CNT_SORTED_COUNT], h[CNT_UNL_LIST_COUNT], h[CNT_CAND_COUNT]);
        fprintf(stderr, "   (the wavefronts ran %u steps)\n", h[CNT_WAVE_STEPS]);
    }
    return BBMAP_OK;
}

extern "C" int bbmsa_debug_sorted_lists(bbmsa_ctx *c, int64_t n_jobs, int32_t *lists3, int64_t *lens3) {
    if (!c || !c->timed || !lists3 || !lens3) return bbfail(BBMAP_E_ARG, "bbmsa_debug_sorted_lists: nothing launched yet");
    if (!c->last.sorted || n_jobs != c->last.jobs) return bbfail(BBMAP_E_ARG, "bbmsa_debug_sorted_lists: the last launch was not a sorted launch of n_jobs jobs");
    unsigned h[bbmsa::kCounterWords];
    BBTRY(read_counters(c, h));
    const unsigned len[3] = {h[CNT_SORTED_COUNT], h[CNT_UNL_LIST_COUNT], h[CNT_CAND_COUNT]};
    for (int k = 0; k < 3; k++) {
        if ((int64_t)len[k] > n_jobs) return bbfail(BBMAP_E_HIP, "bbmsa_debug_sorted_lists: a list is longer than the launch");
        lens3[k] = len[k];
        if (len[k]) BBHIP(hipMemcpy(lists3 + (size_t)k * (size_t)n_jobs, c->fastList.as<int>() + (size_t)k * (size_t)n_jobs, (size_t)len[k] * 4, hipMemcpyDeviceToHost));
    }
    return BBMAP_OK;
}

extern "C" int bbmsa_last_unlimited(bbmsa_ctx *c, int64_t *counts4) {
    if (!c || !c->timed || !counts4) return bbfail(BBMAP_E_ARG, "bbmsa_last_unlimited: nothing launched yet");
    const bool wave = c->sw.scheme == BBMSA_SCHEME_11TS && !c->legacyOnly;
    if (wave && !c->unlimitedStats) return bbfail(BBMAP_E_ARG, "bbmsa_last_unlimited: the context does not count (create it with BBMSA_UNLIMITED_STATS=1 in the environment)");
    unsigned h[bbmsa::kCounterWords];
    BBTRY(read_counters(c, h));
    counts4[0] = wave ? h[CNT_UNL_RAN_UNL] : 0; counts4[1] = wave ? h[CNT_UNL_RAN_GENERAL] : 0;
    counts4[2] = wave ? h[CNT_UNL_STEPS] : 0; counts4[3] = wave ? h[CNT_ALL_STEPS] : 0;
    return BBMAP_OK;
}

int bbmsa_last_route_flags(const bbmsa_ctx *c) {
    if (!c || !c->timed) return 0;
    return (c->last.band ? BBMSA_ROUTE_NARROW : 0) | (c->last.sorted ? BBMSA_ROUTE_SORTED : 0) | (c->last.latency ? BBMSA_ROUTE_LATENCY : 0);
}

extern "C" int bbmsa_last_route(bbmsa_ctx *c, int64_t *route8) {
    if (!c || !c->timed || !route8) return bbfail(BBMAP_E_ARG, "bbmsa_last_route: nothing launched yet");
    unsigned h[bbmsa::kCounterWords];
    BBTRY(read_counters(c, h));
    const Route &r = c->last;
    route8[0] = r.band; route8[1] = r.sorted; route8[2] = r.latency; route8[3] = r.wide; route8[4] = r.indirect;
    route8[5] = h[CNT_SLOW_COUNT]; route8[6] = r.wide ? h[CNT_WIDE_SLOW_COUNT] : 0; route8[7] = r.band ? h[CNT_BAND_DONE] : 0;
    return BBMAP_OK;
}

extern "C" int bbmsa_geometry(bbmsa_ctx *c, int32_t *geo4) {
    if (!c || !geo4) return bbfail(BBMAP_E_ARG, "bbmsa_geometry: null argument");
    geo4[0] = geo4[1] = geo4[2] = geo4[3] = 0;
    if (c->legacy) {
        int last = 0, mask = 0;
        bbmsa_legacy_rows_per_lane(c, &last, &mask);
        geo4[0] = 64; geo4[1] = last; geo4[2] = c->cfg.maxColumns; geo4[3] = mask;
    } else if (c->sw.scheme == BBMSA_SCHEME_11TS) {
        geo4[0] = c->G; geo4[1] = c->R; geo4[2] = c->fastCols; geo4[3] = c->wideBlocks > 0 ? c->wideR : 0;
    }
    return BBMAP_OK;
}

extern "C" int bbmsa_align_batch(bbmsa_ctx *c, int64_t n_jobs, const bbmsa_job *jobs,
                                 const uint8_t *reads, int64_t reads_bytes,
                                 const uint8_t *refs, int64_t refs_bytes,
                                 bbmsa_result *results, uint8_t *match, int32_t match_stride) {
    if (!c) return bbfail(BBMAP_E_ARG, "bbmsa_align_batch: null context");
    if (n_jobs == 0) return BBMAP_OK;
    if (n_jobs < 0 || !jobs || !reads || !refs || !results || reads_bytes < 0 || refs_bytes < 0)
        return bbfail(BBMAP_E_ARG, "bbmsa_align_batch: bad argument");
    BBHIP(hipSetDevice(c->device));
    for (int64_t i = 0; i < n_jobs; i++) {
        const bbmsa_job &j = jobs[i];
        if (j.read_len < 0 || j.read_off < 0 || j.read_off + j.read_len > reads_bytes)
            return bbfail(BBMAP_E_ARG, "bbmsa_align_batch: a read lies outside the reads buffer");
        if (j.ref_len < 0 || j.ref_off < 0 || j.ref_off + j.ref_len > refs_bytes)
            return bbfail(BBMAP_E_ARG, "bbmsa_align_batch: a reference array lies outside the refs buffer");
        if (!(j.flags & BBMSA_CLAMP_WINDOW) && (j.refStartLoc < 0 || j.refEndLoc >= j.ref_len))
            return bbfail(BBMAP_E_ARG, "bbmsa_align_batch: window outside its reference array (set BBMSA_CLAMP_WINDOW to clamp)");
    }
    DevTmp<bbmsa_job> d_jobs; DevTmp<uint8_t> d_reads, d_refs, d_match; DevTmp<bbmsa_result> d_res;
    BBTRY(d_jobs.upload(jobs, (size_t)n_jobs));
    BBTRY(d_reads.upload(reads, (size_t)reads_bytes));
    BBTRY(d_refs.upload(refs, (size_t)refs_bytes));
    BBTRY(d_res.alloc((size_t)n_jobs));
    if (match) BBTRY(d_match.alloc((size_t)n_jobs * (size_t)match_stride));
    BBHIP(hipMemset(d_res, 0xff, (size_t)n_jobs * sizeof(bbmsa_result)));
    BBTRY(bbmsa_align_batch_device(c, nullptr, n_jobs, d_jobs, d_reads, d_refs, d_res, d_match, match_stride));
    BBHIP(hipStreamSynchronize(nullptr));
    BBHIP(hipMemcpy(results, d_res, (size_t)n_jobs * sizeof(bbmsa_result), hipMemcpyDeviceToHost));
// ... 4 lines not shown
```

bbmap_amd/csrc/msa_route.h:

```cpp
#pragma once
#include "bbmap_amd.h"

struct RouteSwitches {
    int scheme = 0;
    bool banded = false;
    bool bandPresent = false;
    bool bandOff = false;
    bool sortByWidth = false;
    bool sortWithBand = false;
    bool unlimitedLoop = true;
    bool wideUnlimited = false;
    bool widePresent = false;
    long long latencyJobs = 0;
    int pipeJobsMax = 0;
};

struct Route {
    bool band = false;
    bool sorted = false;
    bool latency = false;
    bool indirect = false;
    bool wide = false;
    bool unlList = false;
    bool wideBoth = false;
    bool pipelined = false;
    long long jobs = 0;
};

inline Route plan_route(const RouteSwitches &s, long long n_jobs, bool indirect) {
    Route r;
    r.indirect = indirect; r.jobs = n_jobs;
    if (s.scheme != BBMSA_SCHEME_11TS) {
        r.pipelined = !indirect && s.pipeJobsMax > 0 && n_jobs <= s.pipeJobsMax;
        return r;
    }
    r.band = s.bandPresent && !s.bandOff;
    r.wide = s.widePresent;
    r.sorted = s.sortByWidth && !indirect && n_jobs >= 256 && n_jobs > s.latencyJobs && (!r.band || s.sortWithBand);
    r.latency = r.wide && !indirect && !r.band && n_jobs <= s.latencyJobs;
    r.unlList = r.sorted && s.unlimitedLoop;
    r.wideBoth = s.wideUnlimited && !s.banded;
    return r;
}
```

bbmap_amd/csrc/msa_sort.hip:

```cpp
#include <hip/hip_runtime.h>

#include "host_common.h"
#include "msa_common.h"
#include "msa_ctx.h"

namespace bbmsa {
constexpr int WIDTH_PER_CLASS = 512;
constexpr int WIDTH_CLASSES = 3;
constexpr int WIDTH_BUCKETS = WIDTH_CLASSES * WIDTH_PER_CLASS;
enum { CLASS_UNLIMITED = 0, CLASS_CANDIDATE = 1, CLASS_GENERAL = 2 };
constexpr int SORT_THREADS = 256, SORT_JOBS_PER_THREAD = 4;
struct SortKey { int maxRows, maxColumns, bandwidth; float bandwidthRatio; int byKind, band, bandRows, maxSlack; };
__device__ inline int job_width_bucket(const bbmsa_job &t, const SortKey k) {
    int a = t.refStartLoc, b = t.refEndLoc;
    if (t.flags & BBMSA_CLAMP_WINDOW) { a = max(0, a); b = min(t.ref_len - 1, b); if (b - a >= k.maxColumns) b = min(t.ref_len - 1, a + k.maxColumns - 1); }
    const int cols = max(0, b - a + 1);
    int cls = CLASS_GENERAL;
    if (k.band && band_is_candidate(t.flags, t.minScore, t.read_len, b - a + 1, k.maxRows, k.maxColumns, k.bandRows, k.maxSlack)) cls = CLASS_CANDIDATE;
    else if (k.byKind && !fill_is_limited(t.flags, t.minScore, t.read_len, b - a + 1, fill_halfband(t.read_len, b - a + 1, k.bandwidth, k.bandwidthRatio))) cls = CLASS_UNLIMITED;
    constexpr int W = WIDTH_PER_CLASS;
    return cls * W + W - 1 - min(W - 1, cols >> 3);
}
__global__ __launch_bounds__(SORT_THREADS) void width_hist_kernel(const bbmsa_job *jobs, long long n, SortKey key, unsigned *hist) {
    __shared__ unsigned s[WIDTH_BUCKETS];
    for (int i = threadIdx.x; i < WIDTH_BUCKETS; i += SORT_THREADS) s[i] = 0;
    __syncthreads();
    const long long base = (long long)blockIdx.x * (SORT_THREADS * SORT_JOBS_PER_THREAD) + threadIdx.x;
#pragma unroll
    for (int k = 0; k < SORT_JOBS_PER_THREAD; k++) {
        const long long i = base + (long long)k * SORT_THREADS;
        if (i < n) atomicAdd(&s[job_width_bucket(jobs[i], key)], 1u);
    }
    __syncthreads();
    for (int i = threadIdx.x; i < WIDTH_BUCKETS; i += SORT_THREADS) { const unsigned v = s[i]; if (v) atomicAdd(&hist[i], v); }
}
__global__ void width_scan_kernel(unsigned *hist, unsigned *listCount, unsigned *sortedCount, unsigned *unlCount, unsigned *candCount) {
    __shared__ unsigned s[WIDTH_PER_CLASS];
    const int t = threadIdx.x;
    for (int cls = 0; cls < WIDTH_CLASSES; cls++) {
        const unsigned own = hist[cls * WIDTH_PER_CLASS + t];
        s[t] = own;
        __syncthreads();
        for (int d = 1; d < WIDTH_PER_CLASS; d <<= 1) { const unsigned v = t >= d ? s[t - d] : 0u; __syncthreads(); s[t] += v; __syncthreads(); }
        hist[cls * WIDTH_PER_CLASS + t] = s[t] - own;
        if (t == WIDTH_PER_CLASS - 1) {
            if (cls == CLASS_UNLIMITED) *unlCount = s[t];
            else if (cls == CLASS_CANDIDATE) *candCount = s[t];
            else { *listCount = s[t]; *sortedCount = s[t]; }
        }
        __syncthreads();
    }
}
__global__ __launch_bounds__(SORT_THREADS) void width_scatter_kernel(const bbmsa_job *jobs, long long n, SortKey key, unsigned *cursor, int *list, int *unlList, int *candList) {
    __shared__ unsigned s[WIDTH_BUCKETS];
    for (int i = threadIdx.x; i < WIDTH_BUCKETS; i += SORT_THREADS) s[i] = 0;
    __syncthreads();
    const long long base = (long long)blockIdx.x * (SORT_THREADS * SORT_JOBS_PER_THREAD) + threadIdx.x;
    int bucket[SORT_JOBS_PER_THREAD]; unsigned rank[SORT_JOBS_PER_THREAD];
#pragma unroll
    for (int k = 0; k < SORT_JOBS_PER_THREAD; k++) {
        const long long i = base + (long long)k * SORT_THREADS;
        bucket[k] = -1; rank[k] = 0;
        if (i < n) { bucket[k] = job_width_bucket(jobs[i], key); rank[k] = atomicAdd(&s[bucket[k]], 1u); }
    }
    __syncthreads();
    for (int i = threadIdx.x; i < WIDTH_BUCKETS; i += SORT_THREADS) { const unsigned v = s[i]; if (v) s[i] = atomicAdd(&cursor[i], v); }
    __syncthreads();
#pragma unroll
    for (int k = 0; k < SORT_JOBS_PER_THREAD; k++) {
        if (bucket[k] < 0) continue;
        const long long i = base + (long long)k * SORT_THREADS;
        const unsigned pos = s[bucket[k]] + rank[k];
        if ((long long)pos >= n) continue;
        const int cls = bucket[k] / WIDTH_PER_CLASS;
        (cls == CLASS_UNLIMITED ? unlList : (cls == CLASS_CANDIDATE ? candList : list))[pos] = (int)i;
    }
}
}

int bbmsa_width_sort(bbmsa_ctx *c, hipStream_t stream, const bbmsa_job *jobs, int64_t n_jobs, bool band) {
    using namespace bbmsa;
    if (!c->d_widthHist) BBHIP(hipMalloc(&c->d_widthHist, WIDTH_BUCKETS * 4));
    BBHIP(hipMemsetAsync(c->d_widthHist, 0, WIDTH_BUCKETS * 4, stream));
    const int perBlock = SORT_THREADS * SORT_JOBS_PER_THREAD;
    const unsigned sb = (unsigned)((n_jobs + perBlock - 1) / perBlock);
    const SortKey key = {c->cfg.maxRows, c->cfg.maxColumns, c->cfg.bandwidth, c->cfg.bandwidthRatio, c->sw.unlimitedLoop ? 1 : 0,
                         band ? 1 : 0, c->bandRows, c->narrowSlack};
    int *const list = c->fastList.as<int>();
    unsigned *const cnt = c->d_counters;
    hipLaunchKernelGGL(width_hist_kernel, dim3(sb), dim3(SORT_THREADS), 0, stream, jobs, (long long)n_jobs, key, c->d_widthHist);
    hipLaunchKernelGGL(width_scan_kernel, dim3(1), dim3(WIDTH_PER_CLASS), 0, stream, c->d_widthHist, cnt + CNT_LIST_COUNT, cnt + CNT_SORTED_COUNT,
                       cnt + CNT_UNL_LIST_COUNT, cnt + CNT_CAND_COUNT);
    hipLaunchKernelGGL(width_scatter_kernel, dim3(sb), dim3(SORT_THREADS), 0, stream, jobs, (long long)n_jobs, key, c->d_widthHist,
                       list, list + n_jobs, list + 2 * n_jobs);
    BBHIP(hipGetLastError());
    return BBMAP_OK;
}
```

bbmap_amd/mapper.py:

```python
import ctypes as C

import numpy as np
import torch

from . import _lib
from . import msa as M
from .index import READ_DTYPE

MSITE_DTYPE = np.dtype([("chrom", "<i4"), ("strand", "<i4"), ("start", "<i4"), ("stop", "<i4"), ("hits", "<i4"),
                        ("quickScore", "<i4"), ("score", "<i4"), ("slowScore", "<i4"), ("pairedScore", "<i4"),
                        ("perfect", "<i4"), ("semiperfect", "<i4"), ("rescued", "<i4"), ("ngaps", "<i4"),
                        ("gaps", "<i4", (16,)), ("match_job", "<i4"), ("reserved", "<i4", (2,))])
JOBINFO_DTYPE = np.dtype([("read", "<i4"), ("seq", "<i4"), ("kind", "<i4"), ("site", "<i4")])
FINAL_DTYPE = np.dtype([("mapped", "<i4"), ("chrom", "<i4"), ("strand", "<i4"), ("start", "<i4"), ("stop", "<i4"), ("mapScore", "<i4"),
                        ("paired", "<i4"), ("ambiguous", "<i4"), ("perfect", "<i4"), ("rescued", "<i4"), ("match_len", "<i4"),
                        ("nsites", "<i4"), ("match_off", "<i8"), ("reserved", "<i4", (2,))])
SCAFREC_DTYPE = np.dtype([("scaffold", "<i4"), ("start", "<i4"), ("stop", "<i4"), ("pos", "<i4"), ("end", "<i4"), ("scaflen", "<i4"),
                          ("flags", "<i4"), ("reserved", "<i4")])
SCAF_MAPPED, SCAF_PAIRED, SCAF_INBOUNDS, SCAF_SAME_SCAFFOLD = 1, 2, 4, 8
SAMREC_DTYPE = np.dtype([("flag", "<i4"), ("mapq", "<i4"), ("rname", "<i4"), ("rnext", "<i4"), ("pos", "<i4"), ("pnext", "<i4"),
                         ("tlen", "<i4"), ("nm", "<i4"), ("am", "<i4"), ("tags", "<i4"), ("cigar_off", "<i8"), ("cigar_len", "<i4"),
                         ("md_len", "<i4"), ("md_off", "<i8")])
SAM_CIGAR13, SAM_MD = 1, 2
SAM_TAG_XT = 1
assert MSITE_DTYPE.itemsize == 128 and FINAL_DTYPE.itemsize == 64 and SCAFREC_DTYPE.itemsize == 32 and SAMREC_DTYPE.itemsize == 64
GAPPED_BIT = 1 << 30


class bbmap_config(C.Structure):
    _fields_ = [("device", C.c_int32), ("paired", C.c_int32), ("max_reads", C.c_int32), ("max_read_len", C.c_int32),
                ("max_sites", C.c_int32), ("minRatio", C.c_float)] + [(n, C.c_int32) for n in (
                    "slowAlignPadding", "slowRescuePadding", "extraPadding", "tipSearchDist", "maxPairDist", "averagePairDist",
                    "maxRescueDist", "maxRescueMismatches", "maxTrimSitesToRetain", "trimList", "doRescue", "alignColumns",
                    "clearzone3", "msaMaxColumns", "fastCols", "jobsPerRead", "finalStage")] + [("reserved", C.c_int32 * 4)]


class bbmap_output(C.Structure):
    _fields_ = [("sites", C.c_void_p), ("nsites", C.c_void_p), ("cap", C.c_int32), ("match_stride", C.c_int32),
                ("gmatch_stride", C.c_int32), ("reserved", C.c_int32), ("n_jobs", C.c_int64), ("n_gapped_jobs", C.c_int64),
                ("jobs", C.c_void_p), ("results", C.c_void_p), ("jobinfo", C.c_void_p), ("match", C.c_void_p),
                ("gjobs", C.c_void_p), ("gresults", C.c_void_p), ("gjobinfo", C.c_void_p), ("gmatch", C.c_void_p),
                ("ggaps", C.c_void_p), ("final", C.c_void_p), ("final_match", C.c_void_p), ("final_match_bytes", C.c_int64),
                ("n_final_fills", C.c_int64)]


class bbmap_stats(C.Structure):
    _fields_ = [(n, C.c_int64) for n in ("reads", "reads_overflowed", "reads_without_site", "fills", "gapped_fills", "refills",
                                         "rescue_scans", "rescue_fills", "rounds", "fills_dropped")] + \
               [(n, C.c_float) for n in ("ms_probe", "ms_begin", "ms_score", "ms_slow", "ms_finish", "ms_rescue", "ms_total",
                                         "ms_dp_narrow", "ms_dp_wave", "ms_dp_generic", "ms_dp_gapped", "ms_quick_rescue")] + \
               [("probe_stats", C.c_int64 * 5), ("reads_reprobed", C.c_int64), ("ms_overflow", C.c_float), ("log_growths", C.c_float),
                ("ms_dp_wave_max", C.c_float), ("ms_final", C.c_float), ("final_fills", C.c_int64), ("final_rounds", C.c_int64),
                ("final_local", C.c_int64), ("dp_narrow_launches", C.c_int64), ("dp_sorted_launches", C.c_int64),
                ("sites_cross_scaffold", C.c_int64)]


class bbmap_overflow_output(C.Structure):
    _fields_ = [("n_reads", C.c_int64), ("read_ids", C.c_void_p), ("out", bbmap_output)]


NSITES_OVERFLOW, NSITES_MATE_OVERFLOW, NSITES_IN_TIER = -1, -2, -3


def _bind(L):
    L.bbmap_default_config.argtypes = [C.POINTER(bbmap_config)]
    L.bbmap_default_config_profile.argtypes = [C.c_int32, C.POINTER(bbmap_config)]
    L.bbmap_default_config_profile.restype = C.c_int
    L.bbmap_create.argtypes = [C.c_void_p, C.POINTER(bbmap_config), C.POINTER(C.c_void_p)]
    L.bbmap_destroy.argtypes = [C.c_void_p]
    L.bbmap_destroy.restype = None
    L.bbmap_map_batch_device.argtypes = [C.c_void_p, C.c_void_p, C.c_int64, C.c_void_p, C.c_void_p, C.c_int64, C.c_void_p, C.c_void_p]
    L.bbmap_get_output.argtypes = [C.c_void_p, C.POINTER(bbmap_output)]
    L.bbmap_last_stats.argtypes = [C.c_void_p, C.POINTER(bbmap_stats)]
    L.bbmap_get_overflow_output.argtypes = [C.c_void_p, C.POINTER(bbmap_overflow_output)]
    L.bbmap_pack_sites_device.argtypes = [C.c_void_p, C.c_void_p, C.c_int64, C.c_void_p, C.c_void_p, C.c_void_p, C.c_int64]
    L.bbmap_pack_sites_device.restype = C.c_int
    L.bbmap_map_batch.argtypes = [C.c_void_p, C.c_int64, C.c_void_p, C.c_void_p, C.c_int64, C.c_void_p, C.c_void_p, C.c_int64, C.c_void_p,
                                  C.c_void_p, C.c_void_p, C.c_int64, C.POINTER(C.c_int64)]
    L.bbmap_map_batch.restype = C.c_int
    L.bbmap_get_final.argtypes = [C.c_void_p, C.c_int64, C.c_void_p, C.c_void_p, C.c_int64, C.POINTER(C.c_int64)]
    L.bbmap_get_final.restype = C.c_int
    L.bbmap_set_average_pair_dist.argtypes = [C.c_void_p, C.c_int32]
    L.bbmap_set_average_pair_dist.restype = C.c_int
    L.bbmap_get_scaffold_records.argtypes = [C.c_void_p, C.c_void_p, C.POINTER(C.c_void_p)]
    L.bbmap_get_scaffold_records.restype = C.c_int
    L.bbmap_get_sam_records.argtypes = [C.c_void_p, C.c_void_p, C.c_int32, C.POINTER(C.c_void_p), C.POINTER(C.c_void_p), C.POINTER(C.c_int64)]
    L.bbmap_get_sam_records.restype = C.c_int
    L.bbmap_get_sam.argtypes = [C.c_void_p, C.c_int64, C.c_int32, C.c_void_p, C.c_void_p, C.c_int64, C.POINTER(C.c_int64)]
    L.bbmap_get_sam.restype = C.c_int
    L.bbmap_add_run_stats.argtypes = [C.c_void_p, C.c_void_p, C.c_void_p]
    L.bbmap_get_run_stats.argtypes = [C.c_void_p, C.c_void_p, C.c_void_p]
    L.bbmap_reset_run_stats.argtypes = [C.c_void_p]
    L.bbmap_set_adaptive.argtypes = [C.c_void_p, C.c_int32]
    L.bbmap_set_truth.argtypes = [C.c_void_p, C.c_void_p]
    L.bbmap_get_adaptive_state.argtypes = [C.c_void_p, C.POINTER(C.c_int32), C.POINTER(C.c_int32)]
    for f in ("bbmap_add_run_stats", "bbmap_get_run_stats", "bbmap_reset_run_stats", "bbmap_set_adaptive", "bbmap_set_truth",
              "bbmap_get_adaptive_state"):
        getattr(L, f).restype = C.c_int
    for f in ("bbmap_default_config", "bbmap_create", "bbmap_map_batch_device", "bbmap_get_output", "bbmap_last_stats",
              "bbmap_get_overflow_output"):
        getattr(L, f).restype = C.c_int


def _copy(ptr, nbytes, dev=None):
    out = np.empty(max(nbytes, 0), np.uint8)
    if nbytes > 0:
        L = _lib.load()
# ... 445 lines not shown
```

bbmap_amd/msa.py:

```python
import ctypes as C

import numpy as np

from . import _lib
from ._lib import bbmsa_config, bbmsa_job, bbmsa_result

FILL_LIMITED_RAW = 0
FILL_UNLIMITED_RAW = 1
FILL_LIMITED = 2
CLAMP_WINDOW = 1 << 3
DO_SCORE = 1 << 4
DO_TRACEBACK = 1 << 5
NO_ITERATIONS = 1 << 6
FILL_AND_SCORE_LIMITED = FILL_LIMITED | CLAMP_WINDOW | DO_SCORE

ST_OK, ST_NULL, ST_BAD_SHAPE = 0, 1, 2

JOB_DTYPE = np.dtype([("read_off", "<i8"), ("ref_off", "<i8"), ("read_len", "<i4"), ("ref_len", "<i4"),
                      ("refStartLoc", "<i4"), ("refEndLoc", "<i4"), ("minScore", "<i4"), ("flags", "<i4")])
RESULT_DTYPE = np.dtype([("result", "<i4", (5,)), ("status", "<i4"), ("iterations", "<i8"),
                         ("score", "<i4", (8,)), ("score_len", "<i4"), ("match_len", "<i4"),
                         ("fill_kind", "<i4"), ("columns", "<i4")])
GAPS_DTYPE = np.dtype([("ngaps", "<i4"), ("gaps", "<i4", (16,))])
assert JOB_DTYPE.itemsize == C.sizeof(bbmsa_job) and RESULT_DTYPE.itemsize == C.sizeof(bbmsa_result)
# ... 85 lines not shown
    def align_batch_device(self, n_jobs, jobs_ptr, reads_ptr, refs_ptr, results_ptr, match_ptr=0,
                           match_stride=0, stream=0):
        rc = self.L.bbmsa_align_batch_device(self.h, C.c_void_p(stream), n_jobs, C.c_void_p(jobs_ptr),
                                             C.c_void_p(reads_ptr), C.c_void_p(refs_ptr),
                                             C.c_void_p(results_ptr),
                                             C.c_void_p(match_ptr) if match_ptr else None, match_stride)
        _lib.check(rc, "bbmsa_align_batch_device")

    def align_batch_device_indirect(self, n_jobs_ptr, max_jobs, jobs_ptr, reads_ptr, refs_ptr, results_ptr, match_ptr=0,
                                    match_stride=0, stream=0):
        rc = self.L.bbmsa_align_batch_device_indirect(self.h, C.c_void_p(stream), C.c_void_p(n_jobs_ptr), max_jobs,
                                                      C.c_void_p(jobs_ptr), C.c_void_p(reads_ptr), C.c_void_p(refs_ptr),
                                                      C.c_void_p(results_ptr),
                                                      C.c_void_p(match_ptr) if match_ptr else None, match_stride)
        _lib.check(rc, "bbmsa_align_batch_device_indirect")

    def align_gapped_batch_device(self, n_jobs, jobs_ptr, gaps_ptr, reads_ptr, refs_ptr, results_ptr, match_ptr=0,
                                  match_stride=0, stream=0):
        rc = self.L.bbmsa_align_gapped_batch_device(self.h, C.c_void_p(stream), n_jobs, C.c_void_p(jobs_ptr), C.c_void_p(gaps_ptr),
                                                    C.c_void_p(reads_ptr), C.c_void_p(refs_ptr), C.c_void_p(results_ptr),
                                                    C.c_void_p(match_ptr) if match_ptr else None, match_stride)
        _lib.check(rc, "bbmsa_align_gapped_batch_device")

    def align_gapped_batch_device_indirect(self, n_jobs_ptr, max_jobs, jobs_ptr, gaps_ptr, reads_ptr, refs_ptr, results_ptr,
                                           match_ptr=0, match_stride=0, stream=0):
        rc = self.L.bbmsa_align_gapped_batch_device_indirect(self.h, C.c_void_p(stream), C.c_void_p(n_jobs_ptr), max_jobs,
                                                             C.c_void_p(jobs_ptr), C.c_void_p(gaps_ptr), C.c_void_p(reads_ptr),
                                                             C.c_void_p(refs_ptr), C.c_void_p(results_ptr),
                                                             C.c_void_p(match_ptr) if match_ptr else None, match_stride)
        _lib.check(rc, "bbmsa_align_gapped_batch_device_indirect")

    def last_route(self):
        r = (C.c_int64 * 8)()
        _lib.check(self.L.bbmsa_last_route(self.h, r), "bbmsa_last_route")
        return {"narrow": bool(r[0]), "sorted": bool(r[1]), "latency": bool(r[2]), "wide_pass": bool(r[3]), "indirect": bool(r[4]),
                "first_handed_on": r[5], "wide_handed_on": r[6], "narrow_finished": r[7]}

    def last_unlimited(self):
        c = (C.c_int64 * 4)()
        _lib.check(self.L.bbmsa_last_unlimited(self.h, c), "bbmsa_last_unlimited")
        return {"stripped": c[0], "general": c[1], "unlimited_steps": c[2], "steps": c[3]}

    def geometry(self):
        g = (C.c_int32 * 4)()
        _lib.check(self.L.bbmsa_geometry(self.h, g), "bbmsa_geometry")
        if self.legacy:
            return {"lanes": g[0], "rows_per_lane": g[1], "columns": g[2], "launched": {r for r in range(1, 32) if g[3] >> r & 1}}
        return {"lanes": g[0], "rows_per_lane": g[1], "fast_cols": g[2], "wide_rows_per_lane": g[3]}

    def last_counts(self):
        c = (C.c_int64 * 4)()
        _lib.check(self.L.bbmsa_last_counts(self.h, c), "bbmsa_last_counts")
        return {"narrow": c[0], "narrow_left": c[1], "wave": c[2], "generic": c[3]}

    def debug_sorted_lists(self, n_jobs):
        lists = np.full((3, n_jobs), -1, np.int32)
        lens = (C.c_int64 * 3)()
        _lib.check(self.L.bbmsa_debug_sorted_lists(self.h, n_jobs, lists.ctypes.data, lens), "bbmsa_debug_sorted_lists")
        return {"general": lists[0, :lens[0]].copy(), "unlimited": lists[1, :lens[1]].copy(), "candidates": lists[2, :lens[2]].copy()}

    def last_kernel_ms3(self):
        m = (C.c_float * 3)()
        _lib.check(self.L.bbmsa_last_kernel_ms3(self.h, m), "bbmsa_last_kernel_ms3")
        return m[0], m[1], m[2]

    def last_kernel_ms(self):
        a, b = C.c_float(), C.c_float()
        _lib.check(self.L.bbmsa_last_kernel_ms(self.h, C.byref(a), C.byref(b)), "bbmsa_last_kernel_ms")
        return a.value, b.value


def pack_problems(problems, flags):
    reads, refs, jobs = bytearray(), bytearray(), []
    ref_cache = {}
    for k, (read, ref, a, b, ms) in enumerate(problems):
        ro = len(reads)
        reads += bytes(read)
        key = id(ref)
        if key not in ref_cache:
            ref_cache[key] = len(refs)
            refs += bytes(ref)
        fo = ref_cache[key]
        fl = flags[k] if isinstance(flags, (list, tuple, np.ndarray)) else flags
        jobs.append((ro, fo, len(read), len(ref), a, b, ms, fl))
    jobs = np.array(jobs, dtype=JOB_DTYPE) if jobs else np.zeros(0, JOB_DTYPE)
    return jobs, np.frombuffer(bytes(reads) or b"\0", np.uint8), np.frombuffer(bytes(refs) or b"\0", np.uint8)


class MultiStateAligner11ts:

    def __init__(self, maxRows=601, maxColumns=3000, bandwidth=0, bandwidthRatio=0.0, device=0, **kw):
        self.ctx = MSAContext(maxRows, maxColumns, bandwidth, bandwidthRatio, device, **kw)
        self.maxRows, self.maxColumns = maxRows, maxColumns
        self.iterationsLimited = 0
        self.iterationsUnlimited = 0

    def _run(self, problems, flags, want_match=False):
        problems = list(problems)
        jobs, reads, refs = pack_problems(problems, flags)
        stride = 0
        if want_match and problems:
            stride = max(len(p[0]) + (p[3] - p[2] + 1) + 8 +
                         127 * bytes(p[1][max(0, p[2]):max(0, p[3] + 1)]).count(b"-") for p in problems)
            stride = (stride + 15) & ~15
        res, match = self.ctx.align_batch(jobs, reads, refs, stride)
        for r in res:
# ... 57 lines not shown
```

include/bbmap_amd.h:

```cpp
#ifndef BBMAP_AMD_H
#define BBMAP_AMD_H

#include <stdint.h>

#ifdef __cplusplus
extern "C" {
#endif

#define BBMAP_AMD_ABI_VERSION 6

enum {
    BBMAP_OK = 0,
    BBMAP_E_NODEVICE = -1,
    BBMAP_E_ARG = -2,
    BBMAP_E_NOMEM = -3,
    BBMAP_E_HIP = -4,
    BBMAP_E_SHAPE = -5
};

const char *bbmap_last_error(void);
int bbmap_abi_version(void);


enum {
// ... 48 lines not shown
    float   bandwidthRatio;
    int32_t reserved[3];
} bbmsa_config;

#define BBMSA_SCHEME_11TS 0
#define BBMSA_SCHEME_9PACBIO 1
#define BBMSA_LEGACY_ONLY 0x100

int bbmsa_create(const bbmsa_config *cfg, bbmsa_ctx **out);
void bbmsa_destroy(bbmsa_ctx *ctx);

int bbmsa_align_batch_device(bbmsa_ctx *ctx, void *stream, int64_t n_jobs,
                             const bbmsa_job *jobs, const uint8_t *reads, const uint8_t *refs,
                             bbmsa_result *results, uint8_t *match, int32_t match_stride);

int bbmsa_align_batch_device_indirect(bbmsa_ctx *ctx, void *stream, const uint32_t *n_jobs_dev, int64_t max_jobs,
                                      const bbmsa_job *jobs, const uint8_t *reads, const uint8_t *refs,
                                      bbmsa_result *results, uint8_t *match, int32_t match_stride);

int bbmsa_align_batch(bbmsa_ctx *ctx, int64_t n_jobs, const bbmsa_job *jobs,
                      const uint8_t *reads, int64_t reads_bytes,
                      const uint8_t *refs, int64_t refs_bytes,
                      bbmsa_result *results, uint8_t *match, int32_t match_stride);

typedef struct bbmsa_ticket {
    int32_t batch, slot;
    int64_t gen;
    int32_t rows, columns;
} bbmsa_ticket;
int bbmsa_fill_submit(bbmsa_ctx *ctx, const uint8_t *read, int32_t read_len, const uint8_t *ref, int32_t ref_len,
                      int32_t refStartLoc, int32_t refEndLoc, int32_t minScore, int32_t mode,
                      int32_t *result5, int64_t *iterations, bbmsa_ticket *ticket);
int bbmsa_fill_collect(bbmsa_ctx *ctx, bbmsa_ticket *ticket, int32_t *packed, int32_t *vertLimit, int32_t *horizLimit);
int bbmsa_fill_packed(bbmsa_ctx *ctx, const uint8_t *read, int32_t read_len, const uint8_t *ref, int32_t ref_len,
                      int32_t refStartLoc, int32_t refEndLoc, int32_t minScore, int32_t mode,
                      int32_t *result5, int64_t *iterations, int32_t *packed);
int bbmsa_legacy_stats(bbmsa_ctx *ctx, int64_t *stats6);

#define BBMSA_MAX_GAPS 16
typedef struct bbmsa_gaps { int32_t ngaps; int32_t gaps[BBMSA_MAX_GAPS]; } bbmsa_gaps;
int bbmsa_align_gapped_batch_device(bbmsa_ctx *ctx, void *stream, int64_t n_jobs, const bbmsa_job *jobs,
                                    const bbmsa_gaps *gaps, const uint8_t *reads, const uint8_t *refs,
                                    bbmsa_result *results, uint8_t *match, int32_t match_stride);
int bbmsa_align_gapped_batch_device_indirect(bbmsa_ctx *ctx, void *stream, const uint32_t *n_jobs_dev, int64_t max_jobs,
                                             const bbmsa_job *jobs, const bbmsa_gaps *gaps, const uint8_t *reads,
                                             const uint8_t *refs, bbmsa_result *results, uint8_t *match, int32_t match_stride);
int bbmsa_align_gapped_batch(bbmsa_ctx *ctx, int64_t n_jobs, const bbmsa_job *jobs, const bbmsa_gaps *gaps,
                             const uint8_t *reads, int64_t reads_bytes, const uint8_t *refs, int64_t refs_bytes,
                             bbmsa_result *results, uint8_t *match, int32_t match_stride);

int bbmsa_last_kernel_ms(bbmsa_ctx *ctx, float *ms_fast, float *ms_slow);
int bbmsa_last_kernel_ms3(bbmsa_ctx *ctx, float *ms3);
int bbmsa_last_counts(bbmsa_ctx *ctx, int64_t *counts4);
int bbmsa_debug_sorted_lists(bbmsa_ctx *ctx, int64_t n_jobs, int32_t *lists3, int64_t *lens3);
int bbmsa_last_route(bbmsa_ctx *ctx, int64_t *route8);
int bbmsa_last_unlimited(bbmsa_ctx *ctx, int64_t *counts4);
int bbmsa_geometry(bbmsa_ctx *ctx, int32_t *geo4);

enum {
    BBBAND_FORWARD = 0, BBBAND_FORWARD_RC = 1, BBBAND_REVERSE = 2, BBBAND_REVERSE_RC = 3,
    BBBAND_DIR_MASK = 3,
    BBBAND_EXACT = 1 << 2
};
enum {
    BBBAND_SEMANTICS_JNI_C = 0,
    BBBAND_SEMANTICS_JAVA = 1
};

typedef struct bbband_job {
    int64_t query_off;
    int64_t ref_off;
    int32_t query_len;
    int32_t ref_len;
    int32_t qstart;
    int32_t rstart;
    int32_t maxEdits;
    int32_t flags;
} bbband_job;

typedef struct bbband_result {
    int32_t edits;
    int32_t lastQueryLoc;
    int32_t lastRefLoc;
    int32_t lastRow;
    int32_t lastEdits;
    int32_t lastOffset;
    int32_t status;
    int32_t reserved;
} bbband_result;

typedef struct bbband_ctx bbband_ctx;
typedef struct bbband_config {
    int32_t device;
    int32_t width;
    int32_t semantics;
    int32_t reserved;
} bbband_config;

int bbband_create(const bbband_config *cfg, bbband_ctx **out);
void bbband_destroy(bbband_ctx *ctx);
int bbband_align_batch_device(bbband_ctx *ctx, void *stream, int64_t n_jobs, const bbband_job *jobs,
                              const uint8_t *seqs, bbband_result *results);
int bbband_align_batch(bbband_ctx *ctx, int64_t n_jobs, const bbband_job *jobs,
                       const uint8_t *seqs, int64_t seq_bytes, bbband_result *results);

typedef struct bbband_pair { int64_t query_off, ref_off; int32_t query_len, ref_len; } bbband_pair;
// ... 176 lines not shown
    int32_t trimList;
    int32_t doRescue;
    int32_t alignColumns;
    int32_t clearzone3;
    int32_t msaMaxColumns;
    int32_t fastCols;
    int32_t jobsPerRead;
    int32_t finalStage;
    int32_t reserved[4];
} bbmap_config;

typedef struct bbmap_final {
    int32_t mapped;
    int32_t chrom, strand, start, stop;
    int32_t mapScore;
    int32_t paired, ambiguous, perfect, rescued;
    int32_t match_len;
    int32_t nsites;
    int64_t match_off;
    int32_t reserved[2];
} bbmap_final;

typedef struct bbmap_output {
    const bbmap_msite *sites;
    const int32_t *nsites;
    int32_t cap;
    int32_t match_stride, gmatch_stride;
    int32_t reserved;
    int64_t n_jobs, n_gapped_jobs;
    const bbmsa_job *jobs;   const bbmsa_result *results;  const bbmap_jobinfo *jobinfo;  const uint8_t *match;
    const bbmsa_job *gjobs;  const bbmsa_result *gresults; const bbmap_jobinfo *gjobinfo; const uint8_t *gmatch;
    const bbmsa_gaps *ggaps;
    const bbmap_final *final;
    const uint8_t *final_match;
    int64_t final_match_bytes;
    int64_t n_final_fills;
} bbmap_output;

typedef struct bbmap_stats {
    int64_t reads, reads_overflowed, reads_without_site, fills, gapped_fills, refills, rescue_scans, rescue_fills, rounds;
    int64_t fills_dropped;
    float ms_probe, ms_begin, ms_score, ms_slow, ms_finish, ms_rescue, ms_total;
    float ms_dp_narrow, ms_dp_wave, ms_dp_generic, ms_dp_gapped, ms_quick_rescue;
    int64_t probe_stats[5];
    int64_t reads_reprobed;
    float ms_overflow;
    float log_growths;
    float ms_dp_wave_max;
    float ms_final;
    int64_t final_fills, final_rounds, final_local;
    int64_t dp_narrow_launches;
    int64_t dp_sorted_launches;
    int64_t sites_cross_scaffold;
} bbmap_stats;

typedef struct bbmap_ctx bbmap_ctx;
int bbmap_default_config(bbmap_config *cfg);
int bbmap_default_config_profile(int32_t profile, bbmap_config *cfg);
int bbmap_create(bbidx_ctx *index, const bbmap_config *cfg, bbmap_ctx **out);
void bbmap_destroy(bbmap_ctx *ctx);
int bbmap_set_average_pair_dist(bbmap_ctx *ctx, int32_t average_pair_dist);
int bbmap_map_batch_device(bbmap_ctx *ctx, void *stream, int64_t n_reads, const bbidx_read *reads, uint8_t *bases,
                           int64_t minus_delta, const int8_t *baseScores, const int32_t *keyinfo);
int bbmap_get_output(bbmap_ctx *ctx, bbmap_output *out);
int bbmap_final_batch_device(bbmap_ctx *ctx, void *stream, int64_t n_reads, const bbidx_read *reads, uint8_t *bases, int64_t minus_delta,
                             const bbmap_msite *sites, const int32_t *nsites);
int bbmap_map_batch(bbmap_ctx *ctx, int64_t n_reads, const bbidx_read *reads, const uint8_t *bases, int64_t bases_bytes,
                    const int8_t *baseScores, const int32_t *keyinfo, int64_t keyinfo_ints, int32_t *nsites_out,
                    int64_t *offsets_out, bbmap_msite *sites_out, int64_t sites_cap, int64_t *total_out);
typedef struct bbmap_overflow_output {
    int64_t n_reads;
    const int32_t *read_ids;
    bbmap_output out;
} bbmap_overflow_output;
int bbmap_get_overflow_output(bbmap_ctx *ctx, bbmap_overflow_output *out);
int bbmap_get_final(bbmap_ctx *ctx, int64_t n_reads, bbmap_final *out, uint8_t *match_out, int64_t match_cap, int64_t *match_bytes);
int bbmap_untrim_batch_device(bbmap_ctx *ctx, void *stream, const bbidx_read *reads_untrimmed, const bbtrim_rec *trims);
enum { BBMAP_SCAF_MAPPED = 1,
       BBMAP_SCAF_PAIRED = 2,
       BBMAP_SCAF_INBOUNDS = 4,
       BBMAP_SCAF_SAME_SCAFFOLD = 8 };
typedef struct bbmap_scafrec {
    int32_t scaffold;
    int32_t start, stop;
    int32_t pos, end;
    int32_t scaflen;
    int32_t flags;
    int32_t reserved;
} bbmap_scafrec;
int bbmap_get_scaffold_records(bbmap_ctx *ctx, void *stream, const bbmap_scafrec **out);
enum { BBMAP_SAM_CIGAR13 = 1,
       BBMAP_SAM_MD = 2 };
enum { BBMAP_SAM_TAG_XT = 1 };
typedef struct bbmap_samrec {
    int32_t flag, mapq;
    int32_t rname;
    int32_t rnext;
    int32_t pos, pnext, tlen;
    int32_t nm;
    int32_t am;
    int32_t tags;
    int64_t cigar_off;
    int32_t cigar_len;
    int32_t md_len;
    int64_t md_off;
} bbmap_samrec;
// ... 274 lines not shown
```

Measured before the change: 10.27 million.

## Add second banded DP stage with 16-lane groups for wider-slack jobs

Adds a second band-kernel stage, msa_fill_band_kernel<16>, enabled by default. It takes jobs whose slack exceeds the 8-lane band limit but stays within a new wide-slack bound, plus jobs that bail out of the 8-lane stage. The width sort gains a fourth class for these wide candidates, and both band and fast kernels now exit early when their job list is empty. The aim is to keep moderately wide alignments off the slower generic/wavefront path, at the cost of an extra kernel launch, extra queue traffic and more LDS per block.

```diff
diff --git a/bbmap_amd/_lib.py b/bbmap_amd/_lib.py
--- a/bbmap_amd/_lib.py
+++ b/bbmap_amd/_lib.py
@@ -8,7 +8,7 @@
     "bbmap_last_error", "bbmap_abi_version",
     "bbmsa_create", "bbmsa_destroy", "bbmsa_align_batch_device", "bbmsa_align_batch",
     "bbmsa_fill_packed", "bbmsa_fill_submit", "bbmsa_fill_collect", "bbmsa_legacy_stats", "bbmsa_last_kernel_ms", "bbmsa_last_kernel_ms3", "bbmsa_last_counts", "bbmsa_align_gapped_batch_device", "bbmsa_align_gapped_batch", "bbmsa_align_batch_device_indirect",
-    "bbmsa_align_gapped_batch_device_indirect", "bbmsa_last_route", "bbmsa_last_unlimited", "bbmsa_geometry", "bbmsa_debug_sorted_lists",
+    "bbmsa_align_gapped_batch_device_indirect", "bbmsa_last_route", "bbmsa_last_unlimited", "bbmsa_geometry", "bbmsa_debug_sorted_lists", "bbmsa_last_band_counts", "bbmsa_debug_wide_list",
     "bbband_create", "bbband_destroy", "bbband_align_batch_device", "bbband_align_batch",
     "bbband_align_quadruple_batch", "bbband_align_quadruple_progressive_batch", "bbband_align_double_batch",
     "bbidx_create", "bbidx_destroy", "bbidx_find_batch_device", "bbidx_find_batch", "bbidx_find_batch_device_rc", "bbidx_last_stats", "bbidx_last_launch", "bbidx_set_kernel", "bbidx_set_max_read_len", "bbidx_build", "bbidx_get_params", "bbidx_export_block",
@@ -125,6 +125,10 @@
     L.bbmsa_last_counts.restype = C.c_int
     L.bbmsa_debug_sorted_lists.argtypes = [C.c_void_p, C.c_int64, C.c_void_p, C.POINTER(C.c_int64)]
     L.bbmsa_debug_sorted_lists.restype = C.c_int
+    L.bbmsa_last_band_counts.argtypes = [C.c_void_p, C.POINTER(C.c_int64)]
+    L.bbmsa_last_band_counts.restype = C.c_int
+    L.bbmsa_debug_wide_list.argtypes = [C.c_void_p, C.c_int64, C.c_void_p, C.POINTER(C.c_int64)]
+    L.bbmsa_debug_wide_list.restype = C.c_int
     L.bbmsa_last_route.argtypes = [C.c_void_p, C.POINTER(C.c_int64)]
     L.bbmsa_last_route.restype = C.c_int
     L.bbmsa_last_unlimited.argtypes = [C.c_void_p, C.POINTER(C.c_int64)]
diff --git a/bbmap_amd/csrc/mapper_ctx.h b/bbmap_amd/csrc/mapper_ctx.h
--- a/bbmap_amd/csrc/mapper_ctx.h
+++ b/bbmap_amd/csrc/mapper_ctx.h
@@ -47,6 +47,8 @@
     bool ownsMsa;
     long long narrowMinJobs;
     bool sortWide;
+    bool dpCounts;
+    bool band16;
     bool sortPlain;
     int *d_tierUnits; bbidx_read *d_tierReads; int *d_tierReadIds;
     long long tierReads;
diff --git a/bbmap_amd/csrc/mapper_host.hip b/bbmap_amd/csrc/mapper_host.hip
--- a/bbmap_amd/csrc/mapper_host.hip
+++ b/bbmap_amd/csrc/mapper_host.hip
@@ -138,6 +138,8 @@
     c->narrowMinJobs = getenv("BBMAP_NARROW_MIN_JOBS") ? atoll(getenv("BBMAP_NARROW_MIN_JOBS")) : 32768;
     c->sortWide = !(getenv("BBMAP_SORT_WIDE") && atoi(getenv("BBMAP_SORT_WIDE")) == 0);
     c->sortPlain = !(getenv("BBMAP_SORT_PLAIN") && atoi(getenv("BBMAP_SORT_PLAIN")) == 0);
+    c->band16 = !(getenv("BBMAP_BAND16") && atoi(getenv("BBMAP_BAND16")) == 0);
+    c->dpCounts = getenv("BBMAP_DP_COUNTS") != nullptr;
     if (!pacbio) {
         const bool wideUnl = !(getenv("BBMAP_WIDE_UNLIMITED") && atoi(getenv("BBMAP_WIDE_UNLIMITED")) == 0);
         bbmsa_set_wide_unlimited(c->msa, wideUnl);
@@ -272,6 +274,7 @@
     bbmsa_use_narrow(c->msa, nNew >= c->narrowMinJobs);
     bbmsa_sort_by_width(c->msa, c->sortPlain && nNew >= c->narrowMinJobs);
     bbmsa_sort_with_band(c->msa, c->sortPlain);
+    bbmsa_use_band16(c->msa, c->band16);
     if (c->msaGapped != c->msa) { bbmsa_use_narrow(c->msaGapped, false); bbmsa_sort_by_width(c->msaGapped, c->sortWide); }
     hipStream_t gs = (c->dpStream && nNew > 0) ? c->dpStream : stream;
     if (gNew > 0) {
@@ -287,6 +290,7 @@
     const int r2 = gNew > 0 ? bbmsa_last_route_flags(c->msaGapped) : 0;
     c->stats.dp_narrow_launches += (r1 & 1) + (r2 & 1);
     c->stats.dp_sorted_launches += ((r1 >> 1) & 1) + ((r2 >> 1) & 1);
+    c->stats.dp_band16_launches += ((r1 >> 3) & 1) + ((r2 >> 3) & 1);
     if (gNew > 0 && gs != stream) BBHIP(hipStreamWaitEvent(stream, c->evJoin, 0));
     return BBMAP_OK;
 }
@@ -297,13 +301,19 @@
                                                                  if (k3[1] > c->stats.ms_dp_wave_max) c->stats.ms_dp_wave_max = k3[1]; }
     if (gapped && c->msaGapped != c->msa && bbmsa_last_kernel_ms3(c->msaGapped, k3) == BBMAP_OK) c->stats.ms_dp_gapped += k3[0] + k3[1] + k3[2];
     static const bool show = getenv("BBMAP_DP_COUNTS") != nullptr;
-    if (show) {
-        int64_t n4[4], u4[4];
-        if (plain && bbmsa_last_counts(c->msa, n4) == BBMAP_OK && bbmsa_last_unlimited(c->msa, u4) == BBMAP_OK)
+    if (show || c->dpCounts) {
+        int64_t n4[4], u4[4], b8[8];
+        if (plain && bbmsa_last_band_counts(c->msa, b8) == BBMAP_OK) {
+            c->stats.dp_band16_finished += b8[2];
+            if (show) fprintf(stderr, "dp band stages  : finished <8> %lld, finished <16> %lld, handed on by <8> %lld (%lld of them edge leavers to <16>), handed on by <16> %lld, "
+                    "on <16>'s list by its rule %lld, tried by neither %lld\n", (long long)b8[0], (long long)b8[2], (long long)b8[1], (long long)b8[5],
+                    (long long)b8[3], (long long)b8[4], (long long)b8[6]);
+        }
+        if (show && plain && bbmsa_last_counts(c->msa, n4) == BBMAP_OK && bbmsa_last_unlimited(c->msa, u4) == BBMAP_OK)
             fprintf(stderr, "dp counts plain : narrow finished %lld, narrow handed on %lld, wavefront list %lld, to the wide/generic pass %lld, "
                     "unlimited in their own build %lld, in the general build %lld, wavefront steps unlimited %lld of %lld\n",
                     (long long)n4[0], (long long)n4[1], (long long)n4[2], (long long)n4[3], (long long)u4[0], (long long)u4[1], (long long)u4[2], (long long)u4[3]);
-        if (gapped && bbmsa_last_counts(c->msaGapped, n4) == BBMAP_OK && bbmsa_last_unlimited(c->msaGapped, u4) == BBMAP_OK)
+        if (show && gapped && bbmsa_last_counts(c->msaGapped, n4) == BBMAP_OK && bbmsa_last_unlimited(c->msaGapped, u4) == BBMAP_OK)
             fprintf(stderr, "dp counts second: narrow finished %lld, narrow handed on %lld, wavefront list %lld, to the wide/generic pass %lld, "
                     "unlimited in their own build %lld, in the general build %lld, wavefront steps unlimited %lld of %lld\n",
                     (long long)n4[0], (long long)n4[1], (long long)n4[2], (long long)n4[3], (long long)u4[0], (long long)u4[1], (long long)u4[2], (long long)u4[3]);
@@ -551,6 +561,7 @@
     st.rescue_fills += ts.rescue_fills; st.fills_dropped += ts.fills_dropped;
     st.final_fills += ts.final_fills; st.final_local += ts.final_local;
     st.dp_narrow_launches += ts.dp_narrow_launches; st.dp_sorted_launches += ts.dp_sorted_launches;
+    st.dp_band16_launches += ts.dp_band16_launches; st.dp_band16_finished += ts.dp_band16_finished;
     st.sites_cross_scaffold += ts.sites_cross_scaffold;
     if (getenv("BBMAP_TIER_DEBUG"))
         fprintf(stderr, "[bbmap tier] reads %lld: probe %.2f begin %.2f score %.2f slow %.2f (rounds %lld) finish %.2f rescue %.2f total %.2f\n",
diff --git a/bbmap_amd/csrc/msa_common.h b/bbmap_amd/csrc/msa_common.h
--- a/bbmap_amd/csrc/msa_common.h
+++ b/bbmap_amd/csrc/msa_common.h
@@ -125,6 +125,21 @@
     }
     return (70 + 100 * (rows - 1)) - tmin <= maxSlack;
 }
+
+__host__ __device__ inline bool band_is_wide_candidate(int flags, int minScore, int rows, int columns, int maxRows, int maxColumns, int bandRows, int maxSlack,
+                                                       int wideSlack) {
+    const int mode = flags & BBMSA_MODE_MASK;
+    if (wideSlack <= 0) return false;
+    if (!(rows >= 16 && columns >= rows && rows <= maxRows && rows <= bandRows && columns <= maxColumns && mode != BBMSA_FILL_UNLIMITED_RAW)) return false;
+    int tmin = minScore;
+    if (mode == BBMSA_FILL_LIMITED) {
+        if (tmin < 1 || (columns + rows < 90) || (columns > rows + min(170, rows + 20))) return false;
+        tmin -= 120;
+    }
+    const int slack = (70 + 100 * (rows - 1)) - tmin;
+    return slack > maxSlack && slack + 50 * (columns - rows) <= wideSlack;
+}
+constexpr int kWideSlackDefault = 4250;
 
 __device__ inline long long job_count(long long njobs, const unsigned int *njobs_dev) {
     if (!njobs_dev) return njobs;
@@ -152,18 +167,25 @@
     CNT_CAND_COUNT = 15,
     CNT_SORTED_COUNT = 16,
     CNT_WAVE_STEPS = 17,
-};
-constexpr int CNT_BAND_STATS = 5, CNT_UNL_STATS = 9;
+    CNT_BAND16_QUEUE = 18,
+    CNT_BAND16_DONE = 19,
+    CNT_BAND16_HANDED = 20,
+    CNT_WIDE_CAND_COUNT = 21,
+    CNT_WIDE_RULE_COUNT = 22,
+};
+constexpr int CNT_BAND_STATS = 5, CNT_BAND16_STATS = 19, CNT_UNL_STATS = 9;
 enum BandStat { BAND_STAT_DONE = 0, BAND_STAT_HANDED = 1 };
 enum UnlStat { UNL_STAT_RAN_UNL = 0, UNL_STAT_RAN_GENERAL = 1, UNL_STAT_STEPS = 4, UNL_STAT_ALL_STEPS = 5, UNL_STAT_WAVE_STEPS = 8 };
 static_assert(CNT_BAND_DONE == CNT_BAND_STATS + BAND_STAT_DONE && CNT_BAND_HANDED == CNT_BAND_STATS + BAND_STAT_HANDED, "band kernel's counters");
+static_assert(CNT_BAND16_DONE == CNT_BAND16_STATS + BAND_STAT_DONE && CNT_BAND16_HANDED == CNT_BAND16_STATS + BAND_STAT_HANDED, "second band stage's counters");
 static_assert(CNT_UNL_RAN_UNL == CNT_UNL_STATS + UNL_STAT_RAN_UNL && CNT_UNL_RAN_GENERAL == CNT_UNL_STATS + UNL_STAT_RAN_GENERAL &&
               CNT_UNL_STEPS == CNT_UNL_STATS + UNL_STAT_STEPS && CNT_ALL_STEPS == CNT_UNL_STATS + UNL_STAT_ALL_STEPS &&
               CNT_WAVE_STEPS == CNT_UNL_STATS + UNL_STAT_WAVE_STEPS, "wavefront kernel's counters");
 constexpr bool counter_slots_distinct() {
     constexpr int all[] = {CNT_FAST_QUEUE, CNT_SLOW_COUNT, CNT_GENERIC_QUEUE, CNT_BAND_QUEUE, CNT_LIST_COUNT, CNT_BAND_DONE, CNT_BAND_HANDED,
                            CNT_WIDE_SLOW_COUNT, CNT_WIDE_QUEUE, CNT_UNL_RAN_UNL, CNT_UNL_RAN_GENERAL, CNT_UNL_LIST_COUNT, CNT_UNL_QUEUE,
-                           CNT_UNL_STEPS, CNT_ALL_STEPS, CNT_CAND_COUNT, CNT_SORTED_COUNT, CNT_WAVE_STEPS};
+                           CNT_UNL_STEPS, CNT_ALL_STEPS, CNT_CAND_COUNT, CNT_SORTED_COUNT, CNT_WAVE_STEPS, CNT_BAND16_QUEUE, CNT_BAND16_DONE,
+                           CNT_BAND16_HANDED, CNT_WIDE_CAND_COUNT, CNT_WIDE_RULE_COUNT};
     unsigned seen = 0;
     for (int s : all) { if (s < 0 || s >= kCounterWords || ((seen >> s) & 1u)) return false; seen |= 1u << s; }
     return true;
@@ -218,6 +240,10 @@
     int bandwidth;
     float bandwidthRatio;
     int maxSlack;
+    int wideSlack;
+    int takeWide;
+    int *edge_list;
+    unsigned int *edge_count;
     unsigned int *dirbuf32;
     int tableLen;
     int bandRows;
diff --git a/bbmap_amd/csrc/msa_ctx.h b/bbmap_amd/csrc/msa_ctx.h
--- a/bbmap_amd/csrc/msa_ctx.h
+++ b/bbmap_amd/csrc/msa_ctx.h
@@ -28,6 +28,7 @@
     unsigned int *d_widthHist = nullptr;
     int bandRows = 0, bandLds = 0;
     unsigned int *d_bandDir = nullptr;
+    int band16Lds = 0, band16Blocks = 0, wideSlack = 0;
     DevBuf fastList;
     DevBuf gref, gaux, gjobs;
     hipEvent_t ev[4] = {};
@@ -52,7 +53,7 @@
     p.maxRows = c->cfg.maxRows; p.maxColumns = c->cfg.maxColumns; p.bandwidth = c->cfg.bandwidth; p.bandwidthRatio = c->cfg.bandwidthRatio;
 }
 
-int bbmsa_width_sort(bbmsa_ctx *c, hipStream_t stream, const bbmsa_job *jobs, int64_t n_jobs, bool band);
+int bbmsa_width_sort(bbmsa_ctx *c, hipStream_t stream, const bbmsa_job *jobs, int64_t n_jobs, bool band, bool band16);
 
 int bbmsa_align_impl(bbmsa_ctx *c, void *stream_, int64_t n_jobs, const uint32_t *n_jobs_dev, const bbmsa_job *jobs,
                      const uint8_t *reads, const uint8_t *refs, bbmsa_result *results, uint8_t *match, int32_t match_stride);
@@ -61,9 +62,10 @@
 int bbmsa_wait_first_pass(bbmsa_ctx *c, void *waiter);
 void bbmsa_sort_by_width(bbmsa_ctx *c, bool on);
 void bbmsa_sort_with_band(bbmsa_ctx *c, bool on);
+void bbmsa_use_band16(bbmsa_ctx *c, bool on);
 void bbmsa_set_wide_unlimited(bbmsa_ctx *c, bool on);
 int bbmsa_set_latency_jobs(bbmsa_ctx *c, int64_t n);
-enum { BBMSA_ROUTE_NARROW = 1, BBMSA_ROUTE_SORTED = 2, BBMSA_ROUTE_LATENCY = 4 };
+enum { BBMSA_ROUTE_NARROW = 1, BBMSA_ROUTE_SORTED = 2, BBMSA_ROUTE_LATENCY = 4, BBMSA_ROUTE_BAND16 = 8 };
 int bbmsa_last_route_flags(const bbmsa_ctx *c);
 
 int bbmsa_legacy_create(bbmsa_ctx *c);
diff --git a/bbmap_amd/csrc/msa_fill_band.hip b/bbmap_amd/csrc/msa_fill_band.hip
--- a/bbmap_amd/csrc/msa_fill_band.hip
+++ b/bbmap_amd/csrc/msa_fill_band.hip
@@ -38,6 +38,8 @@
     constexpr int JOBS = 2 * GROUPS;
     static_assert(Q == 4 || Q == 8 || Q == 16, "a group is a power of two of lanes, its good bits fit 64");
     extern __shared__ int lds[];
+    const long long NJ = p.list ? (long long)ld_coherent(p.list_count) : job_count(p.njobs, p.njobs_dev);
+    if (NJ <= 0) return;
     const int TL = p.tableLen;
     int *delC = lds, *insC = lds + TL, *delExt = lds + 2 * TL, *insExt = delExt + 128;
     int4 *mTab = reinterpret_cast<int4 *>(delExt + 192);
@@ -58,7 +60,6 @@
     const int RB = (p.bandRows + 4 + 3) & ~3, FB = (p.bandRows + B + 4 + 3) & ~3;
     uint8_t *jobLds = reinterpret_cast<uint8_t *>(lds + lds_table_ints(TL)) + (long long)wave * JOBS * (RB + FB);
     unsigned *dir = p.dirbuf32 + ((long long)blockIdx.x * 4 + wave) * (long long)(p.bandRows + 1) * 128;
-    const long long NJ = p.list ? (long long)ld_coherent(p.list_count) : job_count(p.njobs, p.njobs_dev);
     unsigned nDone = 0, nLeft = 0;
 
     for (;;) {
@@ -75,6 +76,13 @@
                     if (tb - ta >= p.maxColumns) tb = min(t.ref_len - 1, ta + p.maxColumns - 1);
                 }
                 if (band_is_candidate(t.flags, t.minScore, t.read_len, tb - ta + 1, p.maxRows, p.maxColumns, p.bandRows, p.maxSlack)) { myJ = t_; break; }
+                if (band_is_wide_candidate(t.flags, t.minScore, t.read_len, tb - ta + 1, p.maxRows, p.maxColumns, p.bandRows, p.maxSlack, p.wideSlack)) {
+                    if (p.takeWide) { myJ = t_; break; }
+                    const unsigned k = atomicAdd(p.edge_count, 1u);
+                    p.edge_list[k] = (int)t_;
+                    atomicAdd(p.edge_count + 1, 1u);
+                    continue;
+                }
                 const unsigned k = atomicAdd(p.fast_count, 1u);
                 p.fast_list[k] = (int)t_;
             }
@@ -247,7 +255,7 @@
             int bail = set ? S[1].bail : S[0].bail;
             for (int d = 1; d < Q; d <<= 1) bail |= __shfl_xor(bail, d, 64);
             const bool live = jobOk[s];
-            if (live && bail) { if (q == 0) { const unsigned k = atomicAdd(p.fast_count, 1u); p.fast_list[k] = (int)j; nLeft++; } }
+            if (live && bail) { if (q == 0) { const unsigned k = atomicAdd(p.edge_count, 1u); p.edge_list[k] = (int)j; nLeft++; } }
             if (!(live && !bail)) continue;
 
             const bbmsa_job jb = p.jobs[j];
@@ -407,10 +415,11 @@
 }
 
 template __global__ void msa_fill_band_kernel<8>(const NarrowParams);
-
-const void *band_kernel() { return (const void *)msa_fill_band_kernel<8>; }
-int band_lds_bytes(int tableLen, int bandRows) {
-    constexpr int Q = 8, B = 4 * Q, JOBS = 2 * (64 / Q);
+template __global__ void msa_fill_band_kernel<16>(const NarrowParams);
+
+const void *band_kernel(int Q) { return Q == 16 ? (const void *)msa_fill_band_kernel<16> : (const void *)msa_fill_band_kernel<8>; }
+int band_lds_bytes(int tableLen, int bandRows, int Q) {
+    const int B = 4 * Q, JOBS = 2 * (64 / Q);
     const int RB = (bandRows + 4 + 3) & ~3, FB = (bandRows + B + 4 + 3) & ~3;
     return lds_table_ints(tableLen) * 4 + 4 * JOBS * (RB + FB);
 }
diff --git a/bbmap_amd/csrc/msa_fill_fast.hip b/bbmap_amd/csrc/msa_fill_fast.hip
--- a/bbmap_amd/csrc/msa_fill_fast.hip
+++ b/bbmap_amd/csrc/msa_fill_fast.hip
@@ -42,6 +42,8 @@
 template <int R, bool BANDED, bool MAT = false, int UNL = 0>
 __global__ __launch_bounds__(256, (UNL == 2 && BBMSA_MIN_WAVES(R) > 2) ? 2 : BBMSA_MIN_WAVES(R)) void msa_fill_fast_kernel(const FillParams p) {
     extern __shared__ int lds[];
+    const long long total = p.list ? (long long)load_coherent(p.list_count) : job_count(p.njobs, p.njobs_dev);
+    if (total <= 0) return;
     int *delC = lds;
     const int TL = p.tableLen;
     int *insC = lds + TL;
@@ -85,7 +87,6 @@
     const long long slot = ((long long)blockIdx.x * (blockDim.x >> 6) + wave) * jobsPerWave + sub;
     unsigned *dir = p.dirbuf + slot * p.dir_slot_dwords;
 
-    const long long total = p.list ? (long long)load_coherent(p.list_count) : job_count(p.njobs, p.njobs_dev);
     for (;;) {
         unsigned base = 0;
         if (lane == 0) base = atomicAdd(p.queue, (unsigned)jobsPerWave);
diff --git a/bbmap_amd/csrc/msa_host.hip b/bbmap_amd/csrc/msa_host.hip
--- a/bbmap_amd/csrc/msa_host.hip
+++ b/bbmap_amd/csrc/msa_host.hip
@@ -24,8 +24,8 @@
 const void *fast_kernel_unl_for(int R);
 const void *fast_kernel_both_for(int R);
 template <class S> __global__ void msa_fill_generic_kernel(const GenericParams p);
-const void *band_kernel();
-int band_lds_bytes(int tableLen, int bandRows);
+const void *band_kernel(int Q);
+int band_lds_bytes(int tableLen, int bandRows, int Q);
 }
 
 static int clamp_occupancy(int per, int most) { return per < 1 ? 1 : (per > most ? most : per); }
@@ -168,12 +168,21 @@
     if (!c->sw.banded && env_int("BBMSA_NARROW", 1) != 0) {
         int perCU = 0;
         c->bandRows = cfg->maxRows < 256 ? cfg->maxRows : 256;
-        c->bandLds = bbmsa::band_lds_bytes(c->tableLen, c->bandRows);
-        if (c->bandLds > 64 * 1024) BBHIP(hipFuncSetAttribute(bbmsa::band_kernel(), hipFuncAttributeMaxDynamicSharedMemorySize, c->bandLds));
-        BBHIP(hipOccupancyMaxActiveBlocksPerMultiprocessor(&perCU, bbmsa::band_kernel(), 256, c->bandLds));
+        c->bandLds = bbmsa::band_lds_bytes(c->tableLen, c->bandRows, 8);
+        if (c->bandLds > 64 * 1024) BBHIP(hipFuncSetAttribute(bbmsa::band_kernel(8), hipFuncAttributeMaxDynamicSharedMemorySize, c->bandLds));
+        BBHIP(hipOccupancyMaxActiveBlocksPerMultiprocessor(&perCU, bbmsa::band_kernel(8), 256, c->bandLds));
         c->narrowBlocks = c->numCUs * clamp_occupancy(perCU, 4);
         c->sw.bandPresent = true;
         BBHIP(hipMalloc(&c->d_bandDir, (size_t)c->narrowBlocks * 4 * (size_t)(c->bandRows + 1) * 128 * 4));
+        int perCU16 = 0;
+        c->band16Lds = bbmsa::band_lds_bytes(c->tableLen, c->bandRows, 16);
+        if (c->band16Lds > 64 * 1024) BBHIP(hipFuncSetAttribute(bbmsa::band_kernel(16), hipFuncAttributeMaxDynamicSharedMemorySize, c->band16Lds));
+        BBHIP(hipOccupancyMaxActiveBlocksPerMultiprocessor(&perCU16, bbmsa::band_kernel(16), 256, c->band16Lds));
+        c->band16Blocks = c->numCUs * clamp_occupancy(perCU16, 4);
+        if (c->band16Blocks > c->narrowBlocks) c->band16Blocks = c->narrowBlocks;
+        c->wideSlack = env_int("BBMSA_BAND16_SLACK", bbmsa::kWideSlackDefault);
+        c->sw.band16Present = c->wideSlack > c->narrowSlack;
+        c->sw.band16 = env_int("BBMSA_BAND16", 0) != 0;
     }
     c->sw.sortByWidth = env_int("BBMSA_SORT_BY_WIDTH", 0) != 0;
     c->sw.sortWithBand = env_int("BBMSA_SORT_WITH_BAND", 0) != 0;
@@ -283,18 +292,28 @@
     return BBMAP_OK;
 }
 
-int launch_band(bbmsa_ctx *c, const JobBatch &B, const Route &r, hipStream_t stream) {
+int *wide_list(const bbmsa_ctx *c, const Route &r) { return c->fastList.as<int>() + (r.sorted ? 3 : 1) * r.jobs; }
+
+int launch_band(bbmsa_ctx *c, const JobBatch &B, const Route &r, hipStream_t stream, int Q) {
     int *const fastList = c->fastList.as<int>();
+    unsigned *const cnt = c->d_counters;
+    const bool second = Q == 16;
     bbmsa::NarrowParams np;
     set_batch(np, c, B);
-    np.queue = c->d_counters + CNT_BAND_QUEUE; np.fast_list = fastList; np.fast_count = c->d_counters + CNT_LIST_COUNT;
-    np.stats = c->d_counters + CNT_BAND_STATS; np.maxSlack = c->narrowSlack;
+    np.queue = cnt + (second ? CNT_BAND16_QUEUE : CNT_BAND_QUEUE); np.fast_list = fastList; np.fast_count = cnt + CNT_LIST_COUNT;
+    np.stats = cnt + (second ? CNT_BAND16_STATS : CNT_BAND_STATS); np.maxSlack = c->narrowSlack;
+    np.wideSlack = r.band16 ? c->wideSlack : 0; np.takeWide = second ? 1 : 0;
+    const bool toWide = r.band16 && !second;
+    np.edge_list = toWide ? wide_list(c, r) : fastList; np.edge_count = cnt + (toWide ? CNT_WIDE_CAND_COUNT : CNT_LIST_COUNT);
     np.dirbuf32 = c->d_bandDir; np.tableLen = c->tableLen; np.bandRows = c->bandRows;
-    np.list = r.sorted ? fastList + 2 * r.jobs : nullptr; np.list_count = r.sorted ? c->d_counters + CNT_CAND_COUNT : nullptr;
-    long long nb = (r.jobs + 63) / 64;
-    if (nb > c->narrowBlocks) nb = c->narrowBlocks;
+    if (second) { np.list = wide_list(c, r); np.list_count = cnt + CNT_WIDE_CAND_COUNT; }
+    else { np.list = r.sorted ? fastList + 2 * r.jobs : nullptr; np.list_count = r.sorted ? cnt + CNT_CAND_COUNT : nullptr; }
+    const int perBlock = 4 * 2 * (64 / Q);
+    const long long most = second ? c->band16Blocks : c->narrowBlocks;
+    long long nb = (r.jobs + perBlock - 1) / perBlock;
+    if (nb > most) nb = most;
     void *nargs[] = {&np};
-    BBHIP(hipLaunchKernel(bbmsa::band_kernel(), dim3((unsigned)nb), dim3(256), nargs, (size_t)c->bandLds, stream));
+    BBHIP(hipLaunchKernel(bbmsa::band_kernel(Q), dim3((unsigned)nb), dim3(256), nargs, (size_t)(second ? c->band16Lds : c->bandLds), stream));
     return BBMAP_OK;
 }
 
@@ -349,7 +368,7 @@
     const size_t listBytes = (size_t)n_jobs * 4;
     BBHIP(c->slowList.grow(listBytes, 0, &stream));
     if (r.wide) BBHIP(c->slowList2.grow(listBytes, 0, &stream));
-    if (c->sw.bandPresent || r.sorted) BBHIP(c->fastList.grow(r.sorted ? 3 * listBytes : listBytes, 0, &stream));
+    if (c->sw.bandPresent || r.sorted) BBHIP(c->fastList.grow(((r.sorted ? 3 : 1) + (r.band16 ? 1 : 0)) * listBytes, 0, &stream));
     BBHIP(hipMemsetAsync(c->d_counters, 0, bbmsa::kCounterBytes, stream));
     c->last = r;
     BBHIP(hipEventRecord(c->ev[0], stream));
@@ -359,8 +378,9 @@
         BBHIP(hipEventRecord(c->ev[1], stream));
         return launch_generic<bbmsa::Scheme9PacBio>(c, B, stream, c->slowList.as<int>(), c->d_counters + CNT_SLOW_COUNT);
     }
-    if (r.sorted) BBTRY(bbmsa_width_sort(c, stream, jobs, n_jobs, r.band));
-    if (r.band) BBTRY(launch_band(c, B, r, stream));
+    if (r.sorted) BBTRY(bbmsa_width_sort(c, stream, jobs, n_jobs, r.band, r.band16));
+    if (r.band) BBTRY(launch_band(c, B, r, stream, 8));
+    if (r.band16) BBTRY(launch_band(c, B, r, stream, 16));
     BBHIP(hipEventRecord(c->ev[3], stream));
     bbmsa::FillParams fp = first_pass_params(c, B, r);
     const int jobsPerBlock = 4 * (64 / c->G);
@@ -379,6 +399,7 @@
 void bbmsa_use_narrow(bbmsa_ctx *c, bool on) { if (c) c->sw.bandOff = !on; }
 void bbmsa_sort_by_width(bbmsa_ctx *c, bool on) { if (c) c->sw.sortByWidth = on; }
 void bbmsa_sort_with_band(bbmsa_ctx *c, bool on) { if (c) c->sw.sortWithBand = on; }
+void bbmsa_use_band16(bbmsa_ctx *c, bool on) { if (c) c->sw.band16 = on; }
 void bbmsa_set_wide_unlimited(bbmsa_ctx *c, bool on) { if (c) c->sw.wideUnlimited = on; }
 int bbmsa_set_latency_jobs(bbmsa_ctx *c, int64_t n) {
     if (!c || c->sw.scheme != BBMSA_SCHEME_11TS || c->legacyOnly) return BBMAP_OK;
@@ -434,8 +455,36 @@
     if (getenv("BBMAP_DP_COUNTS")) {
         if (r.wide) fprintf(stderr, "   (first pass handed %u jobs to the wide pass)\n", h[CNT_SLOW_COUNT]);
         if (r.sorted) fprintf(stderr, "   (sorted: %u general, %u unlimited, %u band candidates)\n", h[CNT_SORTED_COUNT], h[CNT_UNL_LIST_COUNT], h[CNT_CAND_COUNT]);
+        if (r.band16) fprintf(stderr, "   (second band stage: %u by its rule + %u edge leavers of the first; finished %u, handed on %u)\n", h[CNT_WIDE_RULE_COUNT],
+                              h[CNT_WIDE_CAND_COUNT] - h[CNT_WIDE_RULE_COUNT], h[CNT_BAND16_DONE], h[CNT_BAND16_HANDED]);
         fprintf(stderr, "   (the wavefronts ran %u steps)\n", h[CNT_WAVE_STEPS]);
     }
+    return BBMAP_OK;
+}
+
+extern "C" int bbmsa_last_band_counts(bbmsa_ctx *c, int64_t *counts8) {
+    if (!c || !c->timed || !counts8) return bbfail(BBMAP_E_ARG, "bbmsa_last_band_counts: nothing launched yet");
+    unsigned h[bbmsa::kCounterWords];
+    BBTRY(read_counters(c, h));
+    const Route &r = c->last;
+    const int64_t leavers = r.band16 ? (int64_t)h[CNT_WIDE_CAND_COUNT] - h[CNT_WIDE_RULE_COUNT] : 0;
+    counts8[0] = h[CNT_BAND_DONE]; counts8[1] = h[CNT_BAND_HANDED];
+    counts8[2] = r.band16 ? h[CNT_BAND16_DONE] : 0; counts8[3] = r.band16 ? h[CNT_BAND16_HANDED] : 0;
+    counts8[4] = r.band16 ? h[CNT_WIDE_RULE_COUNT] : 0; counts8[5] = leavers;
+    counts8[6] = !r.band ? r.jobs : r.sorted ? (int64_t)h[CNT_SORTED_COUNT] + h[CNT_UNL_LIST_COUNT]
+                                             : (int64_t)h[CNT_LIST_COUNT] - (h[CNT_BAND_HANDED] - leavers) - counts8[3];
+    counts8[7] = r.band16 ? 1 : 0;
+    return BBMAP_OK;
+}
+
+extern "C" int bbmsa_debug_wide_list(bbmsa_ctx *c, int64_t n_jobs, int32_t *list, int64_t *lens2) {
+    if (!c || !c->timed || !list || !lens2) return bbfail(BBMAP_E_ARG, "bbmsa_debug_wide_list: nothing launched yet");
+    if (!c->last.band16 || n_jobs != c->last.jobs) return bbfail(BBMAP_E_ARG, "bbmsa_debug_wide_list: the last launch did not run the second band stage over n_jobs jobs");
+    unsigned h[bbmsa::kCounterWords];
+    BBTRY(read_counters(c, h));
+    if ((int64_t)h[CNT_WIDE_CAND_COUNT] > n_jobs) return bbfail(BBMAP_E_HIP, "bbmsa_debug_wide_list: the list is longer than the launch");
+    lens2[0] = h[CNT_WIDE_CAND_COUNT]; lens2[1] = h[CNT_WIDE_RULE_COUNT];
+    if (lens2[0]) BBHIP(hipMemcpy(list, wide_list(c, c->last), (size_t)lens2[0] * 4, hipMemcpyDeviceToHost));
     return BBMAP_OK;
 }
 
@@ -466,7 +515,8 @@
 
 int bbmsa_last_route_flags(const bbmsa_ctx *c) {
     if (!c || !c->timed) return 0;
-    return (c->last.band ? BBMSA_ROUTE_NARROW : 0) | (c->last.sorted ? BBMSA_ROUTE_SORTED : 0) | (c->last.latency ? BBMSA_ROUTE_LATENCY : 0);
+    return (c->last.band ? BBMSA_ROUTE_NARROW : 0) | (c->last.sorted ? BBMSA_ROUTE_SORTED : 0) | (c->last.latency ? BBMSA_ROUTE_LATENCY : 0) |
+           (c->last.band16 ? BBMSA_ROUTE_BAND16 : 0);
 }
 
 extern "C" int bbmsa_last_route(bbmsa_ctx *c, int64_t *route8) {
diff --git a/bbmap_amd/csrc/msa_route.h b/bbmap_amd/csrc/msa_route.h
--- a/bbmap_amd/csrc/msa_route.h
+++ b/bbmap_amd/csrc/msa_route.h
@@ -7,6 +7,8 @@
     bool bandPresent = false;
     bool bandOff = false;
     bool sortByWidth = false;
+    bool band16Present = false;
+    bool band16 = false;
     bool sortWithBand = false;
     bool unlimitedLoop = true;
     bool wideUnlimited = false;
@@ -17,6 +19,7 @@
 
 struct Route {
     bool band = false;
+    bool band16 = false;
     bool sorted = false;
     bool latency = false;
     bool indirect = false;
@@ -35,6 +38,7 @@
         return r;
     }
     r.band = s.bandPresent && !s.bandOff;
+    r.band16 = r.band && s.band16Present && s.band16;
     r.wide = s.widePresent;
     r.sorted = s.sortByWidth && !indirect && n_jobs >= 256 && n_jobs > s.latencyJobs && (!r.band || s.sortWithBand);
     r.latency = r.wide && !indirect && !r.band && n_jobs <= s.latencyJobs;
diff --git a/bbmap_amd/csrc/msa_sort.hip b/bbmap_amd/csrc/msa_sort.hip
--- a/bbmap_amd/csrc/msa_sort.hip
+++ b/bbmap_amd/csrc/msa_sort.hip
@@ -6,17 +6,18 @@
 
 namespace bbmsa {
 constexpr int WIDTH_PER_CLASS = 512;
-constexpr int WIDTH_CLASSES = 3;
+constexpr int WIDTH_CLASSES = 4;
 constexpr int WIDTH_BUCKETS = WIDTH_CLASSES * WIDTH_PER_CLASS;
-enum { CLASS_UNLIMITED = 0, CLASS_CANDIDATE = 1, CLASS_GENERAL = 2 };
+enum { CLASS_UNLIMITED = 0, CLASS_CANDIDATE = 1, CLASS_WIDE_CANDIDATE = 2, CLASS_GENERAL = 3 };
 constexpr int SORT_THREADS = 256, SORT_JOBS_PER_THREAD = 4;
-struct SortKey { int maxRows, maxColumns, bandwidth; float bandwidthRatio; int byKind, band, bandRows, maxSlack; };
+struct SortKey { int maxRows, maxColumns, bandwidth; float bandwidthRatio; int byKind, band, bandRows, maxSlack, wideSlack; };
 __device__ inline int job_width_bucket(const bbmsa_job &t, const SortKey k) {
     int a = t.refStartLoc, b = t.refEndLoc;
     if (t.flags & BBMSA_CLAMP_WINDOW) { a = max(0, a); b = min(t.ref_len - 1, b); if (b - a >= k.maxColumns) b = min(t.ref_len - 1, a + k.maxColumns - 1); }
     const int cols = max(0, b - a + 1);
     int cls = CLASS_GENERAL;
     if (k.band && band_is_candidate(t.flags, t.minScore, t.read_len, b - a + 1, k.maxRows, k.maxColumns, k.bandRows, k.maxSlack)) cls = CLASS_CANDIDATE;
+    else if (k.band && band_is_wide_candidate(t.flags, t.minScore, t.read_len, b - a + 1, k.maxRows, k.maxColumns, k.bandRows, k.maxSlack, k.wideSlack)) cls = CLASS_WIDE_CANDIDATE;
     else if (k.byKind && !fill_is_limited(t.flags, t.minScore, t.read_len, b - a + 1, fill_halfband(t.read_len, b - a + 1, k.bandwidth, k.bandwidthRatio))) cls = CLASS_UNLIMITED;
     constexpr int W = WIDTH_PER_CLASS;
     return cls * W + W - 1 - min(W - 1, cols >> 3);
@@ -34,7 +35,8 @@
     __syncthreads();
     for (int i = threadIdx.x; i < WIDTH_BUCKETS; i += SORT_THREADS) { const unsigned v = s[i]; if (v) atomicAdd(&hist[i], v); }
 }
-__global__ void width_scan_kernel(unsigned *hist, unsigned *listCount, unsigned *sortedCount, unsigned *unlCount, unsigned *candCount) {
+__global__ void width_scan_kernel(unsigned *hist, unsigned *listCount, unsigned *sortedCount, unsigned *unlCount, unsigned *candCount,
+                                  unsigned *wideCount, unsigned *wideRuleCount) {
     __shared__ unsigned s[WIDTH_PER_CLASS];
     const int t = threadIdx.x;
     for (int cls = 0; cls < WIDTH_CLASSES; cls++) {
@@ -46,12 +48,14 @@
         if (t == WIDTH_PER_CLASS - 1) {
             if (cls == CLASS_UNLIMITED) *unlCount = s[t];
             else if (cls == CLASS_CANDIDATE) *candCount = s[t];
+            else if (cls == CLASS_WIDE_CANDIDATE) { *wideCount = s[t]; *wideRuleCount = s[t]; }
             else { *listCount = s[t]; *sortedCount = s[t]; }
         }
         __syncthreads();
     }
 }
-__global__ __launch_bounds__(SORT_THREADS) void width_scatter_kernel(const bbmsa_job *jobs, long long n, SortKey key, unsigned *cursor, int *list, int *unlList, int *candList) {
+__global__ __launch_bounds__(SORT_THREADS) void width_scatter_kernel(const bbmsa_job *jobs, long long n, SortKey key, unsigned *cursor, int *list, int *unlList, int *candList,
+                                                                     int *wideList) {
     __shared__ unsigned s[WIDTH_BUCKETS];
     for (int i = threadIdx.x; i < WIDTH_BUCKETS; i += SORT_THREADS) s[i] = 0;
     __syncthreads();
@@ -73,26 +77,26 @@
         const unsigned pos = s[bucket[k]] + rank[k];
         if ((long long)pos >= n) continue;
         const int cls = bucket[k] / WIDTH_PER_CLASS;
-        (cls == CLASS_UNLIMITED ? unlList : (cls == CLASS_CANDIDATE ? candList : list))[pos] = (int)i;
+        (cls == CLASS_UNLIMITED ? unlList : (cls == CLASS_CANDIDATE ? candList : (cls == CLASS_WIDE_CANDIDATE ? wideList : list)))[pos] = (int)i;
     }
 }
 }
 
-int bbmsa_width_sort(bbmsa_ctx *c, hipStream_t stream, const bbmsa_job *jobs, int64_t n_jobs, bool band) {
+int bbmsa_width_sort(bbmsa_ctx *c, hipStream_t stream, const bbmsa_job *jobs, int64_t n_jobs, bool band, bool band16) {
     using namespace bbmsa;
     if (!c->d_widthHist) BBHIP(hipMalloc(&c->d_widthHist, WIDTH_BUCKETS * 4));
     BBHIP(hipMemsetAsync(c->d_widthHist, 0, WIDTH_BUCKETS * 4, stream));
     const int perBlock = SORT_THREADS * SORT_JOBS_PER_THREAD;
     const unsigned sb = (unsigned)((n_jobs + perBlock - 1) / perBlock);
     const SortKey key = {c->cfg.maxRows, c->cfg.maxColumns, c->cfg.bandwidth, c->cfg.bandwidthRatio, c->sw.unlimitedLoop ? 1 : 0,
-                         band ? 1 : 0, c->bandRows, c->narrowSlack};
+                         band ? 1 : 0, c->bandRows, c->narrowSlack, band16 ? c->wideSlack : 0};
     int *const list = c->fastList.as<int>();
     unsigned *const cnt = c->d_counters;
     hipLaunchKernelGGL(width_hist_kernel, dim3(sb), dim3(SORT_THREADS), 0, stream, jobs, (long long)n_jobs, key, c->d_widthHist);
     hipLaunchKernelGGL(width_scan_kernel, dim3(1), dim3(WIDTH_PER_CLASS), 0, stream, c->d_widthHist, cnt + CNT_LIST_COUNT, cnt + CNT_SORTED_COUNT,
-                       cnt + CNT_UNL_LIST_COUNT, cnt + CNT_CAND_COUNT);
+                       cnt + CNT_UNL_LIST_COUNT, cnt + CNT_CAND_COUNT, cnt + CNT_WIDE_CAND_COUNT, cnt + CNT_WIDE_RULE_COUNT);
     hipLaunchKernelGGL(width_scatter_kernel, dim3(sb), dim3(SORT_THREADS), 0, stream, jobs, (long long)n_jobs, key, c->d_widthHist,
-                       list, list + n_jobs, list + 2 * n_jobs);
+                       list, list + n_jobs, list + 2 * n_jobs, band16 ? list + 3 * n_jobs : list);
     BBHIP(hipGetLastError());
     return BBMAP_OK;
 }
diff --git a/bbmap_amd/mapper.py b/bbmap_amd/mapper.py
--- a/bbmap_amd/mapper.py
+++ b/bbmap_amd/mapper.py
@@ -52,7 +52,7 @@
                [("probe_stats", C.c_int64 * 5), ("reads_reprobed", C.c_int64), ("ms_overflow", C.c_float), ("log_growths", C.c_float),
                 ("ms_dp_wave_max", C.c_float), ("ms_final", C.c_float), ("final_fills", C.c_int64), ("final_rounds", C.c_int64),
                 ("final_local", C.c_int64), ("dp_narrow_launches", C.c_int64), ("dp_sorted_launches", C.c_int64),
-                ("sites_cross_scaffold", C.c_int64)]
+                ("sites_cross_scaffold", C.c_int64), ("dp_band16_launches", C.c_int64), ("dp_band16_finished", C.c_int64)]
 
 
 class bbmap_overflow_output(C.Structure):
diff --git a/bbmap_amd/msa.py b/bbmap_amd/msa.py
--- a/bbmap_amd/msa.py
+++ b/bbmap_amd/msa.py
@@ -161,6 +161,18 @@
         c = (C.c_int64 * 4)()
         _lib.check(self.L.bbmsa_last_counts(self.h, c), "bbmsa_last_counts")
         return {"narrow": c[0], "narrow_left": c[1], "wave": c[2], "generic": c[3]}
+
+    def last_band_counts(self):
+        c = (C.c_int64 * 8)()
+        _lib.check(self.L.bbmsa_last_band_counts(self.h, c), "bbmsa_last_band_counts")
+        return {"finished8": c[0], "handed8": c[1], "finished16": c[2], "handed16": c[3], "wide_rule": c[4], "leavers": c[5],
+                "untried": c[6], "band16": bool(c[7])}
+
+    def debug_wide_list(self, n_jobs):
+        lst = np.full(n_jobs, -1, np.int32)
+        lens = (C.c_int64 * 2)()
+        _lib.check(self.L.bbmsa_debug_wide_list(self.h, n_jobs, lst.ctypes.data, lens), "bbmsa_debug_wide_list")
+        return {"all": lst[:lens[0]].copy(), "n_rule": int(lens[1])}
 
     def debug_sorted_lists(self, n_jobs):
         lists = np.full((3, n_jobs), -1, np.int32)
diff --git a/include/bbmap_amd.h b/include/bbmap_amd.h
--- a/include/bbmap_amd.h
+++ b/include/bbmap_amd.h
@@ -124,6 +124,8 @@
 int bbmsa_last_kernel_ms(bbmsa_ctx *ctx, float *ms_fast, float *ms_slow);
 int bbmsa_last_kernel_ms3(bbmsa_ctx *ctx, float *ms3);
 int bbmsa_last_counts(bbmsa_ctx *ctx, int64_t *counts4);
+int bbmsa_last_band_counts(bbmsa_ctx *ctx, int64_t *counts8);
+int bbmsa_debug_wide_list(bbmsa_ctx *ctx, int64_t n_jobs, int32_t *list, int64_t *lens2);
 int bbmsa_debug_sorted_lists(bbmsa_ctx *ctx, int64_t n_jobs, int32_t *lists3, int64_t *lens3);
 int bbmsa_last_route(bbmsa_ctx *ctx, int64_t *route8);
 int bbmsa_last_unlimited(bbmsa_ctx *ctx, int64_t *counts4);
@@ -406,6 +408,8 @@
     int64_t dp_narrow_launches;
     int64_t dp_sorted_launches;
     int64_t sites_cross_scaffold;
+    int64_t dp_band16_launches;
+    int64_t dp_band16_finished;
 } bbmap_stats;
 
 typedef struct bbmap_ctx bbmap_ctx;
```

After: 10.26 million. No clear change (-0.2%).
